# SegataLab/metamlst

Hardware: NVIDIA B200
Metric: aligned reads/s (score+pileup+consensus) (higher is better)
Workload: dtype int32/u8 (integer bit-plane arithmetic)

## Files before the change

include/mmlst.h:

```cpp
#ifndef MMLST_H
#define MMLST_H

#include <stddef.h>
#include <stdint.h>

#ifdef __cplusplus
extern "C" {
#endif

#define MMLST_VERSION 200

enum {
    MMLST_OK = 0,
    MMLST_E_ARG = -1,
    MMLST_E_CUDA = -2,
    MMLST_E_IO = -3,
    MMLST_E_BAM = -4,
    MMLST_E_UNSORTED = -5,
    MMLST_E_PAIRED = -6,
    MMLST_E_RANGE = -7,
    MMLST_E_NOMEM = -8
};

typedef struct mmlst_ctx mmlst_ctx;

const char* mmlst_last_error(void);
int mmlst_version(void);
int mmlst_device_count(void);

int mmlst_create(int device, mmlst_ctx** out);
void mmlst_destroy(mmlst_ctx* ctx);
void* mmlst_stream(mmlst_ctx* ctx);
int mmlst_sync(mmlst_ctx* ctx);

void* mmlst_pinned_alloc(size_t bytes);
void mmlst_pinned_free(void* p);

int mmlst_score_dev(const uint32_t* tid, const int16_t* as0, const uint8_t* xm3, const uint16_t* qlen,
                    const uint32_t* orig_idx, uint64_t n_rec, uint64_t idx_base,
                    const uint8_t* allow, const uint32_t* locus_of, uint32_t n_ref,
                    int minscore, int max_xm, int min_read_len,
                    int64_t* sum_as, uint32_t* n_hit, uint32_t* first_idx, uint64_t* counters, void* stream);

int mmlst_build_runs(const uint32_t* tid, uint64_t n_rec, uint32_t* run_tid, uint32_t* run_start, uint32_t* chunk_run,
                     uint32_t* n_runs);
int mmlst_score_runs_dev(const uint32_t* run_tid, const uint32_t* run_start, uint32_t n_runs, const uint32_t* chunk_run,
                         const int16_t* as0, const uint8_t* xm3, const uint16_t* qlen, const uint32_t* orig_idx,
                         uint64_t n_rec, uint64_t idx_base, const uint8_t* allow, uint32_t n_ref,
                         int minscore, int max_xm, int min_read_len,
                         int64_t* sum_as, uint32_t* n_hit, uint32_t* first_idx, uint64_t* counters, void* stream);
int mmlst_chunk_qlen(const uint16_t* qlen, uint64_t n_rec, uint16_t* chunk_qlen, int* uniform);
int mmlst_score_runs_qc_dev(const uint32_t* run_tid, const uint32_t* run_start, uint32_t n_runs, const uint32_t* chunk_run,
                            const uint16_t* chunk_qlen, const int16_t* as0, const uint8_t* xm3, const uint32_t* orig_idx,
                            uint64_t n_rec, uint64_t idx_base, const uint8_t* allow, uint32_t n_ref,
                            int minscore, int max_xm, int min_read_len,
                            int64_t* sum_as, uint32_t* n_hit, uint32_t* first_idx, uint64_t* counters, void* stream);
#define MMLST_SCORE_VARIANT_DEFAULT 6
int mmlst_set_score_variant(int variant);
#define MMLST_SCORE_L2_HINTS_DEFAULT 1
int mmlst_set_score_l2_hints(int on);
int mmlst_debug_timeline(uint64_t* dev_buf);
#define MMLST_SCORE_GRID_DEFAULT 8
int mmlst_set_score_grid_scale(int eighths);
int mmlst_as_untransform_dev(int16_t* as0, const uint8_t* xm3, uint64_t n, int coeff, void* stream);
int mmlst_expand_chunk_qlen_dev(const uint16_t* chunk_qlen, uint64_t n_rec, uint16_t* qlen, void* stream);
int mmlst_expand_runs_dev(const uint32_t* run_tid, const uint32_t* run_start, uint32_t n_runs, const uint32_t* chunk_run,
                          uint64_t n_rec, uint32_t* tid, void* stream);

uint64_t mmlst_coverage_table_slots(uint64_t n_names_upper_bound);
int mmlst_coverage_dev(const uint32_t* tid, const int16_t* as0, const uint8_t* xm3, const uint16_t* qlen,
                       const uint32_t* orig_idx, const uint64_t* qhash, uint64_t n_rec, uint64_t idx_base,
                       const uint8_t* allow, const uint32_t* locus_of, uint32_t n_ref, int minscore, int max_xm,
                       int min_read_len, void* table, uint64_t table_slots, uint64_t* cov, void* stream);

typedef struct {
    int32_t pos;
    uint32_t row_off;
    uint16_t reflen;
    int16_t as_named;
    uint8_t xm_named;
    uint8_t pad;
    uint16_t nw;
} mmlst_prec;

typedef struct {
    uint32_t rec_begin, rec_end;
    uint32_t col_base, contig_len;
    uint32_t plane_delta;
    uint32_t reserved[3];
} mmlst_chunk;

uint32_t mmlst_chunk_records(uint64_t n_rec);

int mmlst_pileup_dev(const mmlst_prec* recs, const uint32_t* planes,
                     const mmlst_chunk* chunks, uint32_t n_chunks, uint32_t max_row_words,
                     int minscore, int max_xm, uint32_t* counts, uint32_t total_cols, int impl, void* stream);

int mmlst_depth_cap(const uint32_t* tid, const int32_t* pos, const uint32_t* reflen, uint64_t n, uint32_t maxcnt,
                    uint32_t sentinel_nodes, uint8_t* admitted);

int mmlst_consensus_dev(const uint32_t* counts, const uint8_t* dbseq, const uint32_t* col_off, uint32_t n_loci,
                        uint32_t mincov, uint8_t* cons, uint32_t* holes, uint32_t* snps, void* stream);

#define MMLST_STATS_COLUMNS 0u
#define MMLST_STATS_DEPTH 1u
#define MMLST_STATS_LOWDOM 2u
#define MMLST_CONTIG_STATS_MAX_COLS 858993459u
typedef struct {
    uint32_t mode;
    uint32_t mincov;
    uint32_t trunc;
    uint32_t none_char;
    double dominant_frq_thrsh;
} mmlst_contig_stats_params;
size_t mmlst_contig_stats_scratch_bytes(uint32_t total_cols);
int mmlst_contig_stats_dev(uint32_t* counts, const uint32_t* col_off, uint32_t n, uint32_t total_cols, const mmlst_contig_stats_params* prm,
                           void* scratch, size_t scratch_bytes, uint32_t* sel_off, uint32_t* low_off, uint64_t* depth_off,
                           uint32_t* out_col, uint32_t* out_val, uint8_t* cons, uint32_t flags, void* stream);

#define MMLST_SELECT_WARP_DEFAULT 0
int mmlst_set_select_warp_finalize(int on);
#define MMLST_SELECT_CONSUME 1u
#define MMLST_SELECT_SCRATCH_CLEAN 2u
#define MMLST_SELECT_LOCAL 4u
int mmlst_select_dev(int64_t* sum_as, uint32_t* n_hit, uint32_t* first_idx, const uint32_t* locus_rows, const uint32_t* locus_start,
                     const uint32_t* allele_num, uint32_t n_ref, const uint32_t* species_of_locus, const uint32_t* genes_in_db,
                     uint32_t n_loci, uint32_t n_species, int penalty, int nloci_pct, const uint64_t* contig_start,
                     const uint32_t* ref_len, const uint64_t* db_off, uint32_t chunk_records, void* scratch, size_t scratch_bytes,
                     uint32_t* header, uint32_t* chosen_tid, uint32_t* chosen_species, uint32_t* col_off, uint64_t* db_start,
                     mmlst_chunk* chunks, uint32_t max_chunks, uint32_t flags, uint64_t* counters,
                     uint32_t* chosen_first , void* stream);
int mmlst_set_pdl(int on);
int mmlst_pileup_indirect_dev(const mmlst_prec* recs, const uint32_t* planes, const mmlst_chunk* chunks, const uint32_t* header,
                              uint32_t max_row_words, int minscore, int max_xm, uint32_t* counts, int impl, void* stream);
int mmlst_pileup_consensus_indirect_dev(const mmlst_prec* recs, const uint32_t* planes, const mmlst_chunk* chunks, const uint32_t* header,
                                        uint32_t max_row_words, int minscore, int max_xm, uint32_t* counts, const uint8_t* db_ascii,
                                        const uint64_t* db_start, const uint32_t* col_off, uint32_t max_loci, uint32_t mincov, uint8_t* cons,
                                        uint32_t* holes, uint32_t* snps, uint32_t flags, uint32_t* ticket, void* stream);
#define MMLST_CONSENSUS_CONSUME 1u
int mmlst_consensus_indirect_dev(uint32_t* counts, const uint8_t* db_ascii, const uint64_t* db_start, const uint32_t* col_off,
                                 uint32_t max_loci, const uint32_t* header, uint32_t mincov, uint8_t* cons, uint32_t* holes,
                                 uint32_t* snps, uint32_t flags, void* stream);

int mmlst_xchg_publish_dev(const void* block, uint32_t bytes, const uint64_t* peer_base, uint32_t rank, uint32_t world,
                           uint64_t half_stride, uint64_t slot_stride, uint64_t flag_off, const uint64_t* epoch, void* stream);
int mmlst_xchg_await_dev(void* local_base, uint32_t bytes, uint32_t world, uint64_t half_stride, uint64_t slot_stride,
                         uint64_t flag_off, void* out_all, uint64_t* epoch, uint32_t* ticket, uint32_t* status, void* stream);

typedef struct mmlst_comm mmlst_comm;
int mmlst_comm_unique_id(uint8_t* id128);
int mmlst_comm_create(const uint8_t* id128, int rank, int world, int device, mmlst_comm** out);
void mmlst_comm_destroy(mmlst_comm* comm);
int mmlst_allreduce(mmlst_comm* comm, int64_t* score_block, size_t score_words, uint32_t* first_idx, size_t n_ref, uint32_t* counts, size_t n_counts,
                    void* stream);

int mmlst_hamming_min_dev(const uint32_t* db_hi, const uint32_t* db_lo, const uint16_t* row_len, uint32_t n_rows,
                          uint32_t W, const uint32_t* q_hi, const uint32_t* q_lo, const uint16_t* q_len, uint32_t n_q,
                          const uint32_t* blocks, uint32_t n_blocks, uint32_t row_index_base,
                          unsigned long long* best, void* stream);
int mmlst_hamming_exact_dev(const uint32_t* db_hi, const uint32_t* db_lo, const uint16_t* row_len, uint32_t n_rows, uint32_t W,
                            const uint32_t* q_hi, const uint32_t* q_lo, const uint16_t* q_len, uint32_t n_q,
                            const uint32_t* blocks, uint32_t n_blocks, uint32_t row_index_base,
                            const uint32_t* xr_ids, const uint32_t* xr_x, const uint8_t* xr_bytes, uint32_t n_xr,
                            const uint32_t* xq_ids, const uint32_t* xq_x, const uint8_t* xq_bytes, uint32_t n_xq,
                            unsigned long long* best, void* stream);
int mmlst_hamming_min_dev2(const uint32_t* db_hi, const uint32_t* db_lo, const uint16_t* row_len, uint32_t n_rows,
                           uint32_t W, const uint32_t* q_hi, const uint32_t* q_lo, const uint16_t* q_len, uint32_t n_q,
                           const uint32_t* blocks, uint32_t n_blocks, uint32_t max_block_rows, uint32_t max_block_queries,
                           uint32_t row_index_base, unsigned long long* best, void* stream);

typedef struct {
    const uint8_t* bytes; uint64_t n_bytes;
    const uint64_t* table; uint32_t n_blocks;
    int32_t as_xm_coeff;
} mmlst_zstream;

typedef struct {
    const uint8_t* bytes; uint64_t n_bytes;
    const uint64_t* table; uint32_t n_blocks;
    const uint32_t* contig_block;
} mmlst_zpileup;

typedef struct {
    const uint32_t* tid; const int16_t* as0; const uint8_t* xm3; const uint16_t* qlen; const uint32_t* orig_idx;
    uint64_t n_rec;
    const mmlst_prec* p_recs;
    const uint32_t* planes; uint64_t n_prec; uint64_t n_plane_words; uint32_t max_row_words;
    const uint64_t* contig_start;
    uint32_t n_ref;
    uint32_t n_runs;
    const uint32_t* run_tid; const uint32_t* run_start; const uint32_t* chunk_run;
    const uint16_t* chunk_qlen;
    const mmlst_zstream* z;
    const mmlst_zpileup* zp;
} mmlst_soa;

typedef struct { int minscore, max_xm, min_read_len; } mmlst_score_params;

int mmlst_score(mmlst_ctx* ctx, const mmlst_soa* soa, const uint8_t* allow, const uint32_t* locus_of, uint32_t n_loci,
                const mmlst_score_params* prm, int64_t* sum_as, uint32_t* n_hit, uint32_t* first_idx, uint64_t* counters);

typedef struct {
    const uint32_t* locus_of; const uint32_t* allele_num; uint32_t n_ref;
    const uint32_t* species_of_locus; uint32_t n_loci;
    const uint32_t* genes_in_db; uint32_t n_species;
    const uint8_t* db_ascii; const uint64_t* db_off; const uint32_t* bam_ln;
} mmlst_index;
typedef struct { int minscore, max_xm, min_read_len, penalty, nloci_pct; uint32_t mincov; int pileup_impl; } mmlst_sample_params;
typedef struct {
    uint32_t n_chosen, error_bits, bad_len_tid, reserved;
    uint64_t total_reads, ignored_reads;
    uint32_t* chosen_tid; uint32_t* chosen_species; uint32_t* col_off;
    uint8_t* cons; uint64_t cons_capacity;
    uint32_t* holes; uint32_t* snps;
    int64_t* sum_as; uint32_t* n_hit; uint32_t* first_idx;
} mmlst_sample_result;
int mmlst_index_upload(mmlst_ctx* ctx, const mmlst_index* index);
int mmlst_sample(mmlst_ctx* ctx, const mmlst_soa* soa, const uint8_t* allow, const mmlst_sample_params* prm, mmlst_sample_result* res);

#define MMLST_COVERAGE_STREAM_RESIDENT 1u
int mmlst_coverage(mmlst_ctx* ctx, const mmlst_soa* soa, const uint64_t* qhash, const uint8_t* allow, const uint32_t* locus_of,
                   uint32_t n_loci, const mmlst_score_params* prm, uint32_t flags, uint64_t* cov);

int mmlst_pileup_consensus(mmlst_ctx* ctx, const mmlst_soa* soa, const uint32_t* chosen_tid, uint32_t n_loci,
                           const uint8_t* dbseq, const uint32_t* col_off, int minscore, int max_xm, uint32_t mincov,
                           int impl, uint32_t* counts, uint8_t* cons, uint32_t* holes, uint32_t* snps);

typedef struct {
    uint32_t* sel_off;
    uint32_t* low_off;
    uint64_t* depth_off;
    uint32_t* out_col;
    uint32_t* out_val;
    uint8_t* cons;
    uint64_t capacity;
    uint64_t n_out;
} mmlst_contig_stats_out;
int mmlst_contig_stats(mmlst_ctx* ctx, const mmlst_soa* soa, const uint32_t* tid, uint32_t n, const uint32_t* col_off, int minscore,
                       int max_xm, const mmlst_contig_stats_params* prm, mmlst_contig_stats_out* out);

int mmlst_db_upload(mmlst_ctx* ctx, const uint32_t* db_hi, const uint32_t* db_lo, const uint16_t* row_len,
                    uint32_t n_rows, uint32_t W);
int mmlst_hamming_min(mmlst_ctx* ctx, const uint32_t* q_hi, const uint32_t* q_lo, const uint16_t* q_len, uint32_t n_q,
                      const uint32_t* blocks, uint32_t n_blocks, uint32_t* min_dist, uint32_t* argmin_row);
int mmlst_db_upload_x(mmlst_ctx* ctx, const uint32_t* db_hi, const uint32_t* db_lo, const uint16_t* row_len, uint32_t n_rows,
                      uint32_t W, const uint32_t* xr_ids, const uint32_t* xr_x, const uint8_t* xr_bytes, uint32_t n_xr);
int mmlst_hamming_min_x(mmlst_ctx* ctx, const uint32_t* q_hi, const uint32_t* q_lo, const uint16_t* q_len, uint32_t n_q,
                        const uint32_t* xq_ids, const uint32_t* xq_x, const uint8_t* xq_bytes, uint32_t n_xq,
                        const uint32_t* blocks, uint32_t n_blocks, uint32_t* min_dist, uint32_t* argmin_row);

size_t mmlst_hamming_tc_image_bytes(uint32_t n, uint32_t W, uint32_t tile_rows);
int mmlst_hamming_tc_expand_dev(const uint32_t* hi, const uint32_t* lo, const uint16_t* len, uint32_t n, uint32_t W, int db_tiled_layout,
                                uint32_t tile_rows, uint8_t* image, uint32_t* tile_maxlen, void* stream);
int mmlst_hamming_tc_search_dev(const uint8_t* q_image, const uint32_t* q_tile_maxlen, const uint16_t* q_len, uint32_t n_q,
                                const uint8_t* db_image, const uint32_t* db_tile_maxlen, const uint16_t* row_len, uint32_t n_rows,
                                uint32_t W, uint32_t row_index_base, unsigned long long* best, void* stream);

int mmlst_exact_match_dev(const uint32_t* db_hi, const uint32_t* db_lo, const uint16_t* row_len, uint32_t n_rows, uint32_t W,
                          const uint32_t* q_hi, const uint32_t* q_lo, const uint16_t* q_len, uint32_t n_q,
                          const uint32_t* blocks, uint32_t n_blocks, uint32_t max_block_rows, uint32_t row_index_base,
                          const uint32_t* row_key , const uint32_t* xr_ids, const uint8_t* xr_bytes, uint32_t n_xr,
                          const uint32_t* xq_ids, const uint8_t* xq_bytes, uint32_t n_xq, uint32_t* first_row, void* stream);
int mmlst_db_row_keys(mmlst_ctx* ctx, const uint32_t* row_key, uint32_t n_rows);
int mmlst_exact_match(mmlst_ctx* ctx, const uint32_t* q_hi, const uint32_t* q_lo, const uint16_t* q_len, uint32_t n_q,
                      const uint32_t* xq_ids, const uint8_t* xq_bytes, uint32_t n_xq,
                      const uint32_t* blocks, uint32_t n_blocks, uint32_t* first_row);

int mmlst_st_match_dev(const uint32_t* prof_start, const uint32_t* prof_allele, uint32_t n_st,
                       const uint32_t* q_alleles, const uint32_t* q_n, uint32_t l_max, uint32_t n_q,
                       uint32_t* count, uint32_t* best, uint32_t* n_best, uint32_t* out_idx, uint32_t max_out, void* stream);
int mmlst_profiles_upload(mmlst_ctx* ctx, const uint32_t* prof_start, const uint32_t* prof_allele, uint32_t n_st);
int mmlst_st_match(mmlst_ctx* ctx, const uint32_t* q_alleles, const uint32_t* q_n, uint32_t l_max, uint32_t n_q,
                   uint32_t* best, uint32_t* n_best, uint32_t* out_idx, uint32_t max_out);

int mmlst_inflate_raw(const uint8_t* in, size_t n, uint8_t* out, size_t out_capacity, size_t* produced);

typedef struct mmlst_bam mmlst_bam;
typedef struct {
    int minqual; uint32_t max_depth; uint32_t sentinel_nodes; int n_threads; int pinned; int assume_sorted;
    int want_qhash; int check_crc;
    int lenient_tags;
} mmlst_unpack_opts;
typedef struct {
    mmlst_soa soa;
    const uint64_t* qhash;
    const uint32_t* ref_len;
    const char* ref_names;
    const char* header_text;
    uint64_t n_dropped_by_cap, n_unmapped_flag;
    int presorted, minqual; uint32_t max_depth;
    double seconds[5];
    uint64_t n_untagged;
} mmlst_bam_info_t;
int mmlst_bam_unpack(const char* path, const mmlst_unpack_opts* opts , mmlst_bam** out);
int mmlst_bam_info(const mmlst_bam* bam, mmlst_bam_info_t* info);
void mmlst_bam_free(mmlst_bam* bam);

typedef struct mmlst_dev_bam mmlst_dev_bam;
typedef struct {
    const uint32_t* tid; const int16_t* as0; const uint8_t* xm3; const uint16_t* qlen; const uint32_t* orig_idx; const uint64_t* qhash;
    const uint32_t* run_tid; const uint32_t* run_start; const uint32_t* chunk_run; const uint16_t* chunk_qlen; uint32_t n_runs;
    const mmlst_prec* p_recs; const uint32_t* planes;
    uint64_t n_rec, n_prec, n_plane_words; uint32_t max_row_words;
    const uint64_t* contig_start;
    const uint32_t* ref_len;
    const char* ref_names;
    const char* header_text;
    uint32_t n_ref;
    uint64_t n_dropped_by_cap, n_unmapped_flag, n_bgzf_blocks, compressed_bytes, inflated_bytes;
    int presorted, minqual; uint32_t max_depth; int boundary_repairs;
    double seconds[8];
} mmlst_dev_bam_info_t;
int mmlst_bam_ingest(int device, const uint8_t* bam, size_t n_bytes, const mmlst_unpack_opts* opts, void* stream, mmlst_dev_bam** out);
int mmlst_dev_bam_info(const mmlst_dev_bam* bam, mmlst_dev_bam_info_t* info);
void mmlst_dev_bam_free(mmlst_dev_bam* bam);
int mmlst_ingest_trim(int device);

#ifdef __cplusplus
}
#endif
#endif
```

metamlst_b200/bam.py:

```python
from __future__ import annotations

import ctypes as C
import os
from typing import Optional

import numpy as np

from . import native, packing


class UnpackOpts(C.Structure):
    _fields_ = [("minqual", C.c_int), ("max_depth", C.c_uint32), ("sentinel_nodes", C.c_uint32), ("n_threads", C.c_int),
                ("pinned", C.c_int), ("assume_sorted", C.c_int), ("want_qhash", C.c_int), ("check_crc", C.c_int), ("lenient_tags", C.c_int)]


class BamInfo(C.Structure):
    _fields_ = [("soa", native.Soa), ("qhash", C.c_void_p), ("ref_len", C.c_void_p), ("ref_names", C.c_char_p),
                ("header_text", C.c_char_p), ("n_dropped_by_cap", C.c_uint64), ("n_unmapped_flag", C.c_uint64),
                ("presorted", C.c_int), ("minqual", C.c_int), ("max_depth", C.c_uint32), ("seconds", C.c_double * 5), ("n_untagged", C.c_uint64)]


class _Handle:
    def __init__(self, h):
        self.h = h

    def __del__(self):
        try:
            if self.h:
                native.lib().mmlst_bam_free(self.h)
                self.h = None
        except Exception:
            pass


def _view(addr: Optional[int], n: int, dtype) -> np.ndarray:
    dt = np.dtype(dtype)
    if not addr or n == 0:
        return np.zeros(0, dtype=dt)
    buf = (C.c_uint8 * (n * dt.itemsize)).from_address(addr)
    return np.frombuffer(buf, dtype=dt, count=n)


def unpack_bam(path: str, minqual: int = packing.DEFAULT_MINQUAL, max_depth: Optional[int] = packing.DEFAULT_MAX_DEPTH,
               presorted: bool = False, threads: int = 0, pinned: bool = True, want_qhash: bool = True,
               sentinel_nodes: int = 1, lenient_tags: bool = False) -> packing.SoaHost:
    lib = native.lib()
    o = UnpackOpts(int(minqual), int(max_depth or 0), int(sentinel_nodes), int(threads), 1 if pinned else 0,
                   1 if presorted else 0, 1 if want_qhash else 0, 1, 1 if lenient_tags else 0)
    h = C.c_void_p()
    native.check(lib.mmlst_bam_unpack(path.encode(), C.byref(o), C.byref(h)))
    keep = _Handle(h)
    info = BamInfo()
    native.check(lib.mmlst_bam_info(h, C.byref(info)))
    s = info.soa
    n, P, n_ref = int(s.n_rec), int(s.n_prec), int(s.n_ref)
    names = info.ref_names.decode("latin-1").split("\n") if n_ref else []
    soa = packing.SoaHost(
        names, _view(info.ref_len, n_ref, np.uint32).astype(np.int32),
        _view(s.tid, n, np.uint32), _view(s.as0, n, np.int16), _view(s.xm3, n, np.uint8), _view(s.qlen, n, np.uint16),
        _view(s.orig_idx, n, np.uint32) if s.orig_idx else None,
        _view(s.p_recs, P, packing.PREC_DTYPE), _view(s.planes, int(s.n_plane_words), np.uint32), int(s.max_row_words),
        _view(s.contig_start, n_ref + 1, np.uint64), int(info.minqual), int(info.max_depth), int(info.n_dropped_by_cap))
    if s.run_tid:
        nr = int(s.n_runs)
        soa.run_tid, soa.run_start = _view(s.run_tid, nr, np.uint32), _view(s.run_start, nr + 1, np.uint32)
        soa.chunk_run = _view(s.chunk_run, (n + 255) // 256, np.uint32)
        soa.chunk_qlen = _view(s.chunk_qlen, (n + 255) // 256, np.uint16) if s.chunk_qlen else None
        if nr > 0.125 * n:
            soa.run_tid = soa.run_start = soa.chunk_run = soa.chunk_qlen = None
    soa.qhash = _view(info.qhash, 2 * n, np.uint64).reshape(n, 2) if info.qhash else None
    soa.header_text = (info.header_text or b"").decode("latin-1")
    soa.unpack_seconds = dict(zip(("read", "inflate", "parse", "sort", "pack"), [float(x) for x in info.seconds]))
    soa.lenient, soa.n_untagged = bool(lenient_tags), int(info.n_untagged)
    soa._keep = (keep,)
    return soa


class DevBamInfo(C.Structure):
    _fields_ = [("tid", C.c_void_p), ("as0", C.c_void_p), ("xm3", C.c_void_p), ("qlen", C.c_void_p), ("orig_idx", C.c_void_p), ("qhash", C.c_void_p),
                ("run_tid", C.c_void_p), ("run_start", C.c_void_p), ("chunk_run", C.c_void_p), ("chunk_qlen", C.c_void_p), ("n_runs", C.c_uint32),
                ("p_recs", C.c_void_p), ("planes", C.c_void_p),
                ("n_rec", C.c_uint64), ("n_prec", C.c_uint64), ("n_plane_words", C.c_uint64), ("max_row_words", C.c_uint32),
                ("contig_start", C.c_void_p), ("ref_len", C.c_void_p), ("ref_names", C.c_char_p), ("header_text", C.c_char_p), ("n_ref", C.c_uint32),
                ("n_dropped_by_cap", C.c_uint64), ("n_unmapped_flag", C.c_uint64), ("n_bgzf_blocks", C.c_uint64), ("compressed_bytes", C.c_uint64),
                ("inflated_bytes", C.c_uint64), ("presorted", C.c_int), ("minqual", C.c_int), ("max_depth", C.c_uint32), ("boundary_repairs", C.c_int),
                ("seconds", C.c_double * 8)]


class _DevHandle:
    def __init__(self, h):
        self.h = h

    def __del__(self):
        try:
            if self.h:
                native.lib().mmlst_dev_bam_free(self.h)
                self.h = None
        except Exception:
            pass


class _DevArray:

    def __init__(self, addr: int, n: int, typestr: str, keep):
        self.__cuda_array_interface__ = {"shape": (n,), "typestr": typestr, "data": (addr, False), "version": 2, "strides": None}
        self._keep = keep


class PinnedPool:

    def __init__(self):
        import threading
        self._lock = threading.Lock()
        self._free = []

    def get(self, n: int):
        import torch
        with self._lock:
            best = None
            for i, t in enumerate(self._free):
                if t.numel() >= n and (best is None or t.numel() < self._free[best].numel()):
                    best = i
            if best is not None:
                return self._free.pop(best)
        return torch.empty(max(int(n * 1.25), 1 << 20), dtype=torch.uint8, pin_memory=torch.cuda.is_available())

    def put(self, t) -> None:
        base = getattr(t, "_pool_base", None)
        if base is not None:
            with self._lock:
                if len(self._free) < 16:
                    self._free.append(base)


POOL = PinnedPool()


def read_pinned(path: str, pool: Optional[PinnedPool] = None):
    import torch
    size = os.path.getsize(path)
    if pool is not None:
        base = pool.get(size)
    else:
        base = torch.empty(max(size, 1), dtype=torch.uint8, pin_memory=torch.cuda.is_available())
    with open(path, "rb") as fh:
        got = fh.readinto(memoryview(base.numpy())[:size]) if size else 0
    if got != size:
        raise IOError("short read on %s" % path)
    view = base[:size]
    if pool is not None:
        view._pool_base = base
    return view


def ingest_bam(source, device=0, minqual: int = packing.DEFAULT_MINQUAL, max_depth: Optional[int] = packing.DEFAULT_MAX_DEPTH,
               presorted: bool = False, want_qhash: bool = True, sentinel_nodes: int = 1, check_crc: bool = False):
    import torch
    from . import streams
    dev = torch.device("cuda", device) if isinstance(device, int) else torch.device(device)
    data = read_pinned(source) if isinstance(source, str) else source
    addr = data.data_ptr() if hasattr(data, "data_ptr") else data.ctypes.data
    nbytes = int(data.numel() if hasattr(data, "numel") else data.size)
    lib = native.lib()
    o = UnpackOpts(int(minqual), int(max_depth or 0), int(sentinel_nodes), 0, 1, 1 if presorted else 0, 1 if want_qhash else 0,
                  1 if check_crc else 0, 0)
    h = C.c_void_p()
    with torch.cuda.device(dev):
        stream = torch.cuda.current_stream(dev).cuda_stream
        native.check(lib.mmlst_bam_ingest(dev.index or 0, addr, nbytes, C.byref(o), stream, C.byref(h)))
    keep = _DevHandle(h)
    info = DevBamInfo()
    native.check(lib.mmlst_dev_bam_info(h, C.byref(info)))
    n, P, n_ref, nr = int(info.n_rec), int(info.n_prec), int(info.n_ref), int(info.n_runs)

    def t(addr_, count, typestr, dtype):
        if not addr_ or count == 0:
            return torch.zeros(0, dtype=dtype, device=dev)
        return torch.as_tensor(_DevArray(addr_, count, typestr, keep), device=dev)

    s = streams.DeviceStreams()
    s._keep = keep
    s.ref_names = info.ref_names.decode("latin-1").split("\n") if n_ref else []
    s.ref_lens = _view(info.ref_len, n_ref, np.uint32).astype(np.int32)
    s.header_text = (info.header_text or b"").decode("latin-1")
    s.minqual, s.max_depth, s.n_dropped = int(info.minqual), int(info.max_depth), int(info.n_dropped_by_cap)
    s.idx_base = 0
    s.tid, s.as0 = t(info.tid, n, "<i4", torch.int32), t(info.as0, n, "<i2", torch.int16)
    s.xm3, s.qlen = t(info.xm3, n, "|u1", torch.uint8), t(info.qlen, n, "<i2", torch.int16)
    s.orig_idx = t(info.orig_idx, n, "<i4", torch.int32) if info.orig_idx else None
    s.qhash = t(info.qhash, 2 * n, "<i8", torch.int64).view(n, 2) if (info.qhash and want_qhash) else None
    s.p_recs = t(info.p_recs, 4 * P, "<i4", torch.int32).view(P, 4)
    s.planes = t(info.planes, int(info.n_plane_words), "<i4", torch.int32)
    s.n_prec, s.max_row_words = P, int(info.max_row_words)
    s.contig_start = _view(info.contig_start, n_ref + 1, np.uint64).copy()
    s.run_tid = s.run_start = s.chunk_run = s.chunk_qlen = None
    if nr and nr <= 0.125 * n:
        s.run_tid, s.run_start = t(info.run_tid, nr, "<i4", torch.int32), t(info.run_start, nr + 1, "<i4", torch.int32)
        s.chunk_run = t(info.chunk_run, (n + 255) // 256, "<i4", torch.int32)
        s.chunk_qlen = t(info.chunk_qlen, (n + 255) // 256, "<i2", torch.int16) if info.chunk_qlen else None
    s.presorted = bool(info.presorted)
    s.ingest_seconds = dict(zip(("h2d", "inflate", "chain", "parse", "sort", "score_stream", "cap_compact", "pack"), [float(x) for x in info.seconds]))
    s.ingest_stats = {"bgzf_blocks": int(info.n_bgzf_blocks), "compressed_bytes": int(info.compressed_bytes), "inflated_bytes": int(info.inflated_bytes),
                      "boundary_repairs": int(info.boundary_repairs), "unmapped_flag": int(info.n_unmapped_flag)}
    return s
```

metamlst_b200/csrc/score_runs.cu:

```cuda
#include <stdlib.h>

#include "score_runs_kernels.cuh"


static int g_score_variant = -1;
static int score_variant() {
    if (g_score_variant < 0) {
        const char* e = getenv("MMLST_SCORE_VARIANT");
        g_score_variant = (e && e[0] >= '0' && e[0] <= '6' && !e[1]) ? e[0] - '0' : MMLST_SCORE_VARIANT_DEFAULT;
    }
    return g_score_variant;
}
extern "C" int mmlst_set_score_variant(int v) {
    const int prev = score_variant();
    if (v >= 0 && v <= 6) g_score_variant = v;
    return prev;
}

static int g_score_l2_hints = -1;
static int score_l2_hints() {
    if (g_score_l2_hints < 0) {
        const char* e = getenv("MMLST_SCORE_L2_HINTS");
        g_score_l2_hints = e ? (e[0] == '1') : MMLST_SCORE_L2_HINTS_DEFAULT;
    }
    return g_score_l2_hints;
}
extern "C" int mmlst_set_score_l2_hints(int on) {
    const int prev = score_l2_hints();
    if (on == 0 || on == 1) g_score_l2_hints = on;
    return prev;
}

static int g_score_grid8 = -1;
static int score_grid8() {
    if (g_score_grid8 < 0) {
        const char* e = getenv("MMLST_SCORE_GRID");
        const int v = e ? atoi(e) : 0;
        g_score_grid8 = (v >= 1 && v <= 64) ? v : MMLST_SCORE_GRID_DEFAULT;
    }
    return g_score_grid8;
}
extern "C" int mmlst_set_score_grid_scale(int eighths) {
    const int prev = score_grid8();
    if (eighths >= 1 && eighths <= 64) g_score_grid8 = eighths;
    return prev;
}

static int score_runs_launch(const uint32_t* run_tid, const uint32_t* run_start, uint32_t n_runs, const uint32_t* chunk_run,
                             const int16_t* as0, const uint8_t* xm3, const uint16_t* qlen, const uint16_t* chunk_qlen, const uint32_t* orig_idx,
                             uint64_t n_rec, uint64_t idx_base, const uint8_t* allow, uint32_t n_ref, int minscore,
                             int max_xm, int min_read_len, int64_t* sum_as, uint32_t* n_hit, uint32_t* first_idx,
                             uint64_t* counters, void* stream) {
    if (n_rec == 0) return MMLST_OK;
    if (!run_tid || !run_start || !chunk_run || !n_runs || !as0 || !xm3 || (!qlen && !chunk_qlen) || !allow || !sum_as || !n_hit || !first_idx || !counters) {
        mmlst_set_error("mmlst_score_runs_dev: null pointer");
        return MMLST_E_ARG;
    }
    if (n_rec >= 0xffffff00ull) { mmlst_set_error("mmlst_score_runs_dev: %llu records do not fit 32-bit run offsets", (unsigned long long)n_rec); return MMLST_E_RANGE; }
    if ((reinterpret_cast<uintptr_t>(as0) & 15) || (reinterpret_cast<uintptr_t>(xm3) & 7) || (!chunk_qlen && (reinterpret_cast<uintptr_t>(qlen) & 15)) ||
        (orig_idx && (reinterpret_cast<uintptr_t>(orig_idx) & 15))) {
        mmlst_set_error("mmlst_score_runs_dev: record arrays must be 16-byte aligned (as0/qlen/orig_idx), 8 (xm3)");
        return MMLST_E_ARG;
    }
    RunArgs a{run_tid, run_start, chunk_run, n_runs, as0, xm3, qlen, orig_idx, chunk_qlen, n_rec, idx_base, allow, n_ref, minscore, max_xm,
              min_read_len, reinterpret_cast<long long*>(sum_as), n_hit, first_idx, reinterpret_cast<unsigned long long*>(counters), score_l2_hints()};
    const uint64_t nchunks = n_rec >> 8;
    uint64_t want = (nchunks + 15) / 16;
    const int variant = score_variant();
    const cudaStream_t st = static_cast<cudaStream_t>(stream);
    const bool tma_ok = !orig_idx && !(reinterpret_cast<uintptr_t>(xm3) & 15);
    if (variant == 6 && tma_ok && chunk_qlen) {
        static int pair_resident_by_device[MMLST_MAX_DEVICES] = {0};
        int& pair_resident = pair_resident_by_device[mmlst_current_device()];
        const size_t smem = (kThreads / 32) * 2u * (4u * 768u + sizeof(uint64_t));
        if (!pair_resident) {
            CUDA_TRY(cudaFuncSetAttribute(score_runs_ring_pair_kernel, cudaFuncAttributeMaxDynamicSharedMemorySize, static_cast<int>(smem)));
            CUDA_TRY(cudaFuncSetAttribute(score_runs_ring_pair_kernel, cudaFuncAttributePreferredSharedMemoryCarveout, cudaSharedmemCarveoutMaxShared));
            int r = 0;
            if (cudaOccupancyMaxActiveBlocksPerMultiprocessor(&r, score_runs_ring_pair_kernel, kThreads, smem) != cudaSuccess || r < 1) r = 1;
            pair_resident = r;
        }
        const uint64_t cap = static_cast<uint64_t>(mmlst_num_sms()) * pair_resident * score_grid8() / 8;
        if (want > cap) want = cap;
        if (want < 1) want = 1;
        score_runs_ring_pair_kernel<<<static_cast<unsigned>(want), kThreads, smem, st>>>(a);
        CUDA_TRY(cudaGetLastError());
        return MMLST_OK;
    }
    if (variant >= 2 && tma_ok) {
        static int ring_resident_by_device[MMLST_MAX_DEVICES][4][8] = {{{0}}};
        int (&ring_resident)[4][8] = ring_resident_by_device[mmlst_current_device()];
        const int hint = a.l2_hints ? 1 : 0;
        const int q = (chunk_qlen ? 1 : 0) + 2 * hint;
        const int rv = variant == 6 ? 5 : variant;
        const RingCfg cfg = chunk_qlen ? (hint ? ring_config<true, true>(rv) : ring_config<true, false>(rv))
                                       : (hint ? ring_config<false, true>(rv) : ring_config<false, false>(rv));
        const size_t smem = (kThreads / 32) * static_cast<size_t>(cfg.ns) * (cfg.ch * (chunk_qlen ? 768u : 1280u) + sizeof(uint64_t));
        if (!ring_resident[q][rv]) {
            CUDA_TRY(cudaFuncSetAttribute(cfg.kern, cudaFuncAttributeMaxDynamicSharedMemorySize, static_cast<int>(smem)));
            CUDA_TRY(cudaFuncSetAttribute(cfg.kern, cudaFuncAttributePreferredSharedMemoryCarveout, cudaSharedmemCarveoutMaxShared));
            int r = 0;
            if (cudaOccupancyMaxActiveBlocksPerMultiprocessor(&r, cfg.kern, kThreads, smem) != cudaSuccess || r < 1) r = 1;
            ring_resident[q][rv] = r;
        }
        const uint64_t cap = static_cast<uint64_t>(mmlst_num_sms()) * ring_resident[q][rv];
        if (want > cap) want = cap;
        if (want < 1) want = 1;
        cfg.kern<<<static_cast<unsigned>(want), kThreads, smem, st>>>(a);
        CUDA_TRY(cudaGetLastError());
        return MMLST_OK;
    }
    static int resident_by_device[MMLST_MAX_DEVICES][8] = {{0}};
    int (&resident)[8] = resident_by_device[mmlst_current_device()];
    const int v = (orig_idx ? 1 : 0) + 2 * (variant == 1 ? 1 : 0) + (chunk_qlen ? 4 : 0);
    void (*const kerns[8])(const RunArgs) = {score_runs_kernel<false, false, false>, score_runs_kernel<true, false, false>,
                                             score_runs_kernel<false, true, false>, score_runs_kernel<true, true, false>,
                                             score_runs_kernel<false, false, true>, score_runs_kernel<true, false, true>,
                                             score_runs_kernel<false, true, true>, score_runs_kernel<true, true, true>};
    void (*kern)(const RunArgs) = kerns[v];
    if (!resident[v]) {
        if (cudaOccupancyMaxActiveBlocksPerMultiprocessor(&resident[v], kern, kThreads, 0) != cudaSuccess || resident[v] < 1) resident[v] = 3;
    }
    const uint64_t cap = static_cast<uint64_t>(mmlst_num_sms()) * resident[v];
    if (want > cap) want = cap;
    if (want < 1) want = 1;
    kern<<<static_cast<unsigned>(want), kThreads, 0, st>>>(a);
    CUDA_TRY(cudaGetLastError());
    return MMLST_OK;
}

extern "C" int mmlst_score_runs_dev(const uint32_t* run_tid, const uint32_t* run_start, uint32_t n_runs, const uint32_t* chunk_run,
                                    const int16_t* as0, const uint8_t* xm3, const uint16_t* qlen, const uint32_t* orig_idx,
                                    uint64_t n_rec, uint64_t idx_base, const uint8_t* allow, uint32_t n_ref, int minscore,
                                    int max_xm, int min_read_len, int64_t* sum_as, uint32_t* n_hit, uint32_t* first_idx,
                                    uint64_t* counters, void* stream) {
    if (n_rec && !qlen) { mmlst_set_error("mmlst_score_runs_dev: null pointer"); return MMLST_E_ARG; }
    return score_runs_launch(run_tid, run_start, n_runs, chunk_run, as0, xm3, qlen, nullptr, orig_idx, n_rec, idx_base, allow, n_ref, minscore,
                             max_xm, min_read_len, sum_as, n_hit, first_idx, counters, stream);
}

extern "C" int mmlst_score_runs_qc_dev(const uint32_t* run_tid, const uint32_t* run_start, uint32_t n_runs, const uint32_t* chunk_run,
                                       const uint16_t* chunk_qlen, const int16_t* as0, const uint8_t* xm3, const uint32_t* orig_idx,
                                       uint64_t n_rec, uint64_t idx_base, const uint8_t* allow, uint32_t n_ref, int minscore,
                                       int max_xm, int min_read_len, int64_t* sum_as, uint32_t* n_hit, uint32_t* first_idx,
                                       uint64_t* counters, void* stream) {
    if (n_rec && !chunk_qlen) { mmlst_set_error("mmlst_score_runs_qc_dev: null pointer"); return MMLST_E_ARG; }
    return score_runs_launch(run_tid, run_start, n_runs, chunk_run, as0, xm3, nullptr, chunk_qlen, orig_idx, n_rec, idx_base, allow, n_ref,
                             minscore, max_xm, min_read_len, sum_as, n_hit, first_idx, counters, stream);
}

extern "C" int mmlst_expand_chunk_qlen_dev(const uint16_t* chunk_qlen, uint64_t n_rec, uint16_t* qlen, void* stream) {
    if (n_rec == 0) return MMLST_OK;
    if (!chunk_qlen || !qlen) { mmlst_set_error("mmlst_expand_chunk_qlen_dev: null pointer"); return MMLST_E_ARG; }
    uint64_t blocks = (n_rec + 255) / 256;
    const uint64_t cap = static_cast<uint64_t>(mmlst_num_sms()) * 16;
    if (blocks > cap) blocks = cap;
    expand_chunk_qlen_kernel<<<static_cast<unsigned>(blocks), 256, 0, static_cast<cudaStream_t>(stream)>>>(chunk_qlen, n_rec, qlen);
    CUDA_TRY(cudaGetLastError());
    return MMLST_OK;
}

extern "C" int mmlst_expand_runs_dev(const uint32_t* run_tid, const uint32_t* run_start, uint32_t n_runs, const uint32_t* chunk_run,
                                     uint64_t n_rec, uint32_t* tid, void* stream) {
    if (n_rec == 0) return MMLST_OK;
    if (!run_tid || !run_start || !chunk_run || !n_runs || !tid) { mmlst_set_error("mmlst_expand_runs_dev: null pointer"); return MMLST_E_ARG; }
    uint64_t blocks = (n_rec + 255) / 256;
    const uint64_t cap = static_cast<uint64_t>(mmlst_num_sms()) * 16;
    if (blocks > cap) blocks = cap;
    expand_runs_kernel<<<static_cast<unsigned>(blocks), 256, 0, static_cast<cudaStream_t>(stream)>>>(run_tid, run_start, chunk_run, n_runs, n_rec, tid);
    CUDA_TRY(cudaGetLastError());
    return MMLST_OK;
}

namespace {
__global__ void __launch_bounds__(256) as_untransform_kernel(int16_t* __restrict__ as0, const uint8_t* __restrict__ xm3, uint64_t n, int coeff) {
    const uint64_t n8 = n >> 3;
    const uint64_t stride = static_cast<uint64_t>(gridDim.x) * blockDim.x;
    for (uint64_t i = static_cast<uint64_t>(blockIdx.x) * blockDim.x + threadIdx.x; i < n8; i += stride) {
        uint4 a = reinterpret_cast<uint4*>(as0)[i];
        const uint2 x = ld_stream_u2(xm3 + (i << 3));
        uint32_t aw[4] = {a.x, a.y, a.z, a.w};
        const uint32_t xw[2] = {x.x, x.y};
#pragma unroll
        for (int w = 0; w < 4; ++w) {
            const uint32_t xb = xw[w >> 1] >> ((w & 1) * 16);
            const int lo = static_cast<int16_t>(aw[w] & 0xffffu) - coeff * static_cast<int>(xb & 0xffu);
            const int hi = static_cast<int16_t>(aw[w] >> 16) - coeff * static_cast<int>((xb >> 8) & 0xffu);
            aw[w] = (static_cast<uint32_t>(lo) & 0xffffu) | (static_cast<uint32_t>(hi) << 16);
        }
        reinterpret_cast<uint4*>(as0)[i] = make_uint4(aw[0], aw[1], aw[2], aw[3]);
    }
    if (blockIdx.x == 0 && threadIdx.x == 0)
        for (uint64_t i = n8 << 3; i < n; ++i) as0[i] = static_cast<int16_t>(as0[i] - coeff * static_cast<int>(xm3[i]));
}
}

extern "C" int mmlst_as_untransform_dev(int16_t* as0, const uint8_t* xm3, uint64_t n, int coeff, void* stream) {
    if (n == 0 || coeff == 0) return MMLST_OK;
    if (!as0 || !xm3) { mmlst_set_error("mmlst_as_untransform_dev: null pointer"); return MMLST_E_ARG; }
    if ((reinterpret_cast<uintptr_t>(as0) & 15) || (reinterpret_cast<uintptr_t>(xm3) & 7)) { mmlst_set_error("mmlst_as_untransform_dev: as0 must be 16-byte aligned, xm3 8"); return MMLST_E_ARG; }
    uint64_t blocks = ((n >> 3) + 255) / 256;
    const uint64_t cap = static_cast<uint64_t>(mmlst_num_sms()) * 8;
    if (blocks > cap) blocks = cap;
    if (blocks < 1) blocks = 1;
    as_untransform_kernel<<<static_cast<unsigned>(blocks), 256, 0, static_cast<cudaStream_t>(stream)>>>(as0, xm3, n, coeff);
    CUDA_TRY(cudaGetLastError());
    return MMLST_OK;
}
```

metamlst_b200/csrc/score_runs_kernels.cuh:

```cuda
#pragma once
#include "common.cuh"

namespace {

constexpr int kThreads = 256;
constexpr uint32_t FULL = 0xffffffffu;

struct RunArgs {
    const uint32_t* run_tid; const uint32_t* run_start; const uint32_t* chunk_run; uint32_t n_runs;
    const int16_t* as0; const uint8_t* xm3; const uint16_t* qlen; const uint32_t* orig_idx;
    const uint16_t* chunk_qlen;
    uint64_t n_rec; uint64_t idx_base;
    const uint8_t* allow; uint32_t n_ref;
    int minscore, max_xm, min_read_len;
    long long* sum_as; uint32_t* n_hit; uint32_t* first_idx; unsigned long long* counters;
    int l2_hints;
};

__device__ __forceinline__ void flush_run(const RunArgs& a, uint32_t key, long long s, uint32_t c, uint32_t mn) {
    if (c) {
        atomicAdd(reinterpret_cast<unsigned long long*>(a.sum_as + key), static_cast<unsigned long long>(s));
        atomicAdd(a.n_hit + key, c);
        atomicMin(a.first_idx + key, mn);
    }
}

template <bool OIDX> struct Loaded;
template <> struct Loaded<false> { uint4 a8, q8; uint2 x8; uint32_t cq; };
template <> struct Loaded<true> { uint4 a8, q8; uint2 x8; uint32_t cq; uint4 oa, ob; };

template <bool OIDX, bool QC>
__device__ __forceinline__ Loaded<OIDX> load_chunk(const RunArgs& a, uint64_t base_lane) {
    Loaded<OIDX> L;
    L.a8 = ld_stream_u4(a.as0 + base_lane);
    L.x8 = ld_stream_u2(a.xm3 + base_lane);
    if constexpr (QC) { L.cq = __ldg(a.chunk_qlen + (base_lane >> 8)); L.q8 = make_uint4(0, 0, 0, 0); }
    else { L.q8 = ld_stream_u4(a.qlen + base_lane); L.cq = 0; }
    if constexpr (OIDX) { L.oa = ld_stream_u4(a.orig_idx + base_lane); L.ob = ld_stream_u4(a.orig_idx + base_lane + 4); }
    return L;
}

template <bool OIDX>
__device__ __forceinline__ uint32_t rec_index(const Loaded<OIDX>& L, uint32_t idx0, int k) {
    if constexpr (OIDX) {
        const uint32_t oi[8] = {L.oa.x, L.oa.y, L.oa.z, L.oa.w, L.ob.x, L.ob.y, L.ob.z, L.ob.w};
        return oi[k];
    } else {
        return idx0 + k;
    }
}

struct WarpRun {
    uint32_t r, key, end;
    bool al;
    long long s; uint32_t c, mn;
};

__device__ __forceinline__ void open_run(const RunArgs& a, WarpRun& w, uint32_t r) {
    w.r = r;
    if (r < a.n_runs) {
        w.key = __ldg(a.run_tid + r);
        w.end = __ldg(a.run_start + r + 1);
        w.al = (w.key < a.n_ref) && a.allow[w.key];
    } else {
        w.key = 0xffffffffu; w.end = 0xffffffffu; w.al = false;
    }
    w.s = 0; w.c = 0; w.mn = 0xffffffffu;
}

__device__ __forceinline__ void close_run(const RunArgs& a, WarpRun& w, uint32_t lane) {
    if (lane == 0 && w.al) flush_run(a, w.key, w.s, w.c, w.mn);
}

struct Thr {
    uint32_t as_T, as_TL;
    uint32_t ql_T, ql_TL;
    uint32_t xm_T, xm_TH;
    uint32_t h8;
};
constexpr uint32_t H16 = 0x80008000u, H8 = 0x80808080u;

__device__ __forceinline__ Thr make_thr(const RunArgs& a) {
    Thr t;
    const bool none = a.minscore > 32767 || a.min_read_len > 65535 || a.max_xm < 0;
    const uint32_t ts = static_cast<uint32_t>(max(a.minscore, -32768) + 32768) & 0xffffu;
    const uint32_t tq = static_cast<uint32_t>(min(max(a.min_read_len, 0), 65535));
    const uint32_t tx = static_cast<uint32_t>(min(max(a.max_xm, 0), 255));
    t.as_T = ts | (ts << 16); t.as_TL = t.as_T & ~H16;
    t.ql_T = tq | (tq << 16); t.ql_TL = t.ql_T & ~H16;
    t.xm_T = tx * 0x01010101u; t.xm_TH = t.xm_T | H8;
    t.h8 = none ? 0u : H8;
    return t;
}

template <bool OIDX, bool QC>
__device__ __forceinline__ void lane_pass(const Loaded<OIDX>& L, const Thr& t, int min_read_len, uint32_t& p_lo, uint32_t& p_hi) {
    const uint32_t aw[4] = {L.a8.x, L.a8.y, L.a8.z, L.a8.w};
    const uint32_t qw[4] = {L.q8.x, L.q8.y, L.q8.z, L.q8.w};
    uint32_t m[4];
#pragma unroll
    for (int w = 0; w < 4; ++w) {
        const uint32_t da = (aw[w] | H16) - t.as_TL;
        const uint32_t ga = (~aw[w] & ~t.as_T) | ((aw[w] ^ t.as_T) & da);
        if constexpr (QC) {
            m[w] = ga;
        } else {
            const uint32_t dq = (qw[w] | H16) - t.ql_TL;
            const uint32_t gq = (qw[w] & ~t.ql_T) | (~(qw[w] ^ t.ql_T) & dq);
            m[w] = ga & gq;
        }
    }
    const uint32_t b_lo = __byte_perm(m[0], m[1], 0x7531), b_hi = __byte_perm(m[2], m[3], 0x7531);
    const uint32_t x0 = L.x8.x, x1 = L.x8.y;
    const uint32_t d0 = t.xm_TH - (x0 & ~H8), d1 = t.xm_TH - (x1 & ~H8);
    const uint32_t g0 = (t.xm_T & ~x0) | (~(t.xm_T ^ x0) & d0), g1 = (t.xm_T & ~x1) | (~(t.xm_T ^ x1) & d1);
    p_lo = (b_lo & g0 & t.h8) >> 7;
    p_hi = (b_hi & g1 & t.h8) >> 7;
    if constexpr (QC) {
        if (static_cast<int>(L.cq) < min_read_len) { p_lo = 0; p_hi = 0; }
    }
}

template <bool OIDX>
__device__ __forceinline__ void lane_sums(const Loaded<OIDX>& L, uint32_t p_lo, uint32_t p_hi, uint32_t idx0, int& s, uint32_t& c, uint32_t& mn) {
    s = __dp2a_lo(static_cast<int>(L.a8.x), static_cast<int>(p_lo), 0);
    s = __dp2a_hi(static_cast<int>(L.a8.y), static_cast<int>(p_lo), s);
    s = __dp2a_lo(static_cast<int>(L.a8.z), static_cast<int>(p_hi), s);
    s = __dp2a_hi(static_cast<int>(L.a8.w), static_cast<int>(p_hi), s);
    c = __popc(p_lo | (p_hi << 1));
    if constexpr (OIDX) {
        mn = 0xffffffffu;
#pragma unroll
        for (int k = 0; k < 8; ++k) mn = (((k < 4 ? p_lo : p_hi) >> (8 * (k & 3))) & 1u) ? min(mn, rec_index<true>(L, idx0, k)) : mn;
    } else {
        const uint32_t k = p_lo ? (static_cast<uint32_t>(__ffs(p_lo)) - 1u) >> 3 : 4u + ((static_cast<uint32_t>(__ffs(p_hi)) - 1u) >> 3);
        mn = (p_lo | p_hi) ? idx0 + k : 0xffffffffu;
    }
}

template <bool OIDX, bool QC>
__device__ __forceinline__ void reduce_chunk(const RunArgs& a, const Thr& thr, WarpRun& w, const Loaded<OIDX>& L, uint64_t base, uint32_t lane,
                                             uint32_t& tot, uint32_t& ign) {
    constexpr uint32_t R = 8;
    const uint64_t rec0 = base + (lane << 3);
    const uint32_t idx0 = static_cast<uint32_t>(a.idx_base + rec0);
    uint32_t p_lo, p_hi;
    lane_pass<OIDX, QC>(L, thr, a.min_read_len, p_lo, p_hi);
    const uint64_t chunk_end = base + 256;
    if (chunk_end <= w.end) {
        if (w.al) {
            int s; uint32_t c, mn;
            lane_sums<OIDX>(L, p_lo, p_hi, idx0, s, c, mn);
            tot += R;
            ign += R - c;
            w.s += __reduce_add_sync(FULL, s);
            w.c += __reduce_add_sync(FULL, c);
            w.mn = min(w.mn, __reduce_min_sync(FULL, mn));
        }
        if (chunk_end == w.end) { close_run(a, w, lane); open_run(a, w, w.r + 1); }
        return;
    }
    uint64_t lo = base;
    while (lo < chunk_end) {
        const uint64_t hi = (w.end < chunk_end) ? static_cast<uint64_t>(w.end) : chunk_end;
        if (w.al) {
            const uint32_t klo = lo <= rec0 ? 0u : (lo - rec0 >= R ? R : static_cast<uint32_t>(lo - rec0));
            const uint32_t khi = hi <= rec0 ? 0u : (hi - rec0 >= R ? R : static_cast<uint32_t>(hi - rec0));
            const unsigned long long ones = 0x0101010101010101ull;
            const unsigned long long below_hi = khi >= 8 ? ~0ull : ((1ull << (8 * khi)) - 1ull);
            const unsigned long long below_lo = klo >= 8 ? ~0ull : ((1ull << (8 * klo)) - 1ull);
            const unsigned long long inm = khi > klo ? (below_hi & ~below_lo & ones) : 0ull;
            const uint32_t in_lo = static_cast<uint32_t>(inm), in_hi = static_cast<uint32_t>(inm >> 32);
            int s; uint32_t c, mn;
            lane_sums<OIDX>(L, p_lo & in_lo, p_hi & in_hi, idx0, s, c, mn);
            const uint32_t in = khi > klo ? khi - klo : 0u;
            tot += in;
            ign += in - c;
            w.s += __reduce_add_sync(FULL, s);
            w.c += __reduce_add_sync(FULL, c);
            w.mn = min(w.mn, __reduce_min_sync(FULL, mn));
        }
        if (hi == w.end) { close_run(a, w, lane); open_run(a, w, w.r + 1); }
        lo = hi;
    }
}

template <bool QC>
__device__ __forceinline__ void score_tail(const RunArgs& a, uint64_t nchunks, uint32_t lane, uint32_t& tot, uint32_t& ign) {
    uint32_t r = __ldg(a.chunk_run + nchunks);
    for (uint64_t i = (nchunks << 8) + lane; i < a.n_rec; i += 32) {
        while (r + 1 < a.n_runs && i >= a.run_start[r + 1]) ++r;
        const uint32_t key = a.run_tid[r];
        if (!((key < a.n_ref) && a.allow[key])) continue;
        ++tot;
        const int as = a.as0[i];
        const int ql = QC ? int(a.chunk_qlen[nchunks]) : int(a.qlen[i]);
        if ((as >= a.minscore) && (ql >= a.min_read_len) && (int(a.xm3[i]) <= a.max_xm)) {
            const uint32_t idx = a.orig_idx ? a.orig_idx[i] : static_cast<uint32_t>(a.idx_base + i);
            flush_run(a, key, as, 1u, idx);
        } else {
            ++ign;
        }
    }
}

template <bool OIDX, bool PIPE, bool QC>
__global__ void __launch_bounds__(kThreads, PIPE ? (OIDX ? 2 : 3) : (OIDX ? 3 : 4)) score_runs_kernel(const RunArgs a) {
    pdl_launch_dependents();
    const uint32_t lane = threadIdx.x & 31u;
    const uint64_t warp = (static_cast<uint64_t>(blockIdx.x) * blockDim.x + threadIdx.x) >> 5;
    const uint64_t nwarps = (static_cast<uint64_t>(gridDim.x) * blockDim.x) >> 5;
    const uint64_t nchunks = a.n_rec >> 8;
    const uint64_t per = (nchunks + nwarps - 1) / nwarps;
    const uint64_t c0 = warp * per;
    const uint64_t c1 = (c0 + per < nchunks) ? c0 + per : nchunks;
    uint32_t tot = 0, ign = 0;
    const Thr thr = make_thr(a);

    if (c0 < c1) {
        uint64_t ch = c0;
        Loaded<OIDX> A0, A1;
        bool have = ch + 1 < c1;
        if (have) { A0 = load_chunk<OIDX, QC>(a, (ch << 8) + (lane << 3)); A1 = load_chunk<OIDX, QC>(a, ((ch + 1) << 8) + (lane << 3)); }
        WarpRun w;
        open_run(a, w, __ldg(a.chunk_run + c0));
        Loaded<OIDX> B0, B1;
        if constexpr (!PIPE) {
            while (have) {
                reduce_chunk<OIDX, QC>(a, thr, w, A0, ch << 8, lane, tot, ign);
                reduce_chunk<OIDX, QC>(a, thr, w, A1, (ch + 1) << 8, lane, tot, ign);
                ch += 2;
                have = ch + 1 < c1;
                if (have) { A0 = load_chunk<OIDX, QC>(a, (ch << 8) + (lane << 3)); A1 = load_chunk<OIDX, QC>(a, ((ch + 1) << 8) + (lane << 3)); }
            }
        }
        while (have) {
            const bool moreB = ch + 3 < c1;
            if (moreB) { B0 = load_chunk<OIDX, QC>(a, ((ch + 2) << 8) + (lane << 3)); B1 = load_chunk<OIDX, QC>(a, ((ch + 3) << 8) + (lane << 3)); }
            reduce_chunk<OIDX, QC>(a, thr, w, A0, ch << 8, lane, tot, ign);
            reduce_chunk<OIDX, QC>(a, thr, w, A1, (ch + 1) << 8, lane, tot, ign);
            ch += 2;
            if (!moreB) break;
            have = ch + 3 < c1;
            if (have) { A0 = load_chunk<OIDX, QC>(a, ((ch + 2) << 8) + (lane << 3)); A1 = load_chunk<OIDX, QC>(a, ((ch + 3) << 8) + (lane << 3)); }
            reduce_chunk<OIDX, QC>(a, thr, w, B0, ch << 8, lane, tot, ign);
            reduce_chunk<OIDX, QC>(a, thr, w, B1, (ch + 1) << 8, lane, tot, ign);
            ch += 2;
        }
        if (ch < c1) {
            const uint64_t base = ch << 8;
            const Loaded<OIDX> L0 = load_chunk<OIDX, QC>(a, base + (lane << 3));
            reduce_chunk<OIDX, QC>(a, thr, w, L0, base, lane, tot, ign);
        }
        close_run(a, w, lane);
    }

    if (warp == nwarps - 1 && (a.n_rec & 255u)) score_tail<QC>(a, nchunks, lane, tot, ign);
    tot = __reduce_add_sync(FULL, tot);
    ign = __reduce_add_sync(FULL, ign);
    if (lane == 0 && tot) {
        atomicAdd(a.counters + 0, static_cast<unsigned long long>(tot));
        atomicAdd(a.counters + 1, static_cast<unsigned long long>(ign));
    }
}

struct WarpRunPF {
    uint32_t r, key, end;
    uint32_t nkey, nend;
    bool al;
    long long s; uint32_t c, mn;
};

template <bool HINT> __device__ __forceinline__ uint32_t tab_u32(const uint32_t* p, uint64_t pol) {
    if constexpr (HINT) return ld_table_u32(p, pol); else return __ldg(p);
}
template <bool HINT> __device__ __forceinline__ uint32_t tab_u16(const uint16_t* p, uint64_t pol) {
    if constexpr (HINT) return ld_table_u16(p, pol); else return __ldg(p);
}
template <bool HINT> __device__ __forceinline__ uint32_t tab_u8(const uint8_t* p, uint64_t pol) {
    if constexpr (HINT) return ld_table_u8(p, pol); else return *p;
}
template <bool HINT>
__device__ __forceinline__ void request_next_run(const RunArgs& a, WarpRunPF& w, uint64_t pol) {
    if (w.r + 1u < a.n_runs) { w.nkey = tab_u32<HINT>(a.run_tid + w.r + 1u, pol); w.nend = tab_u32<HINT>(a.run_start + w.r + 2u, pol); }
    else { w.nkey = 0xffffffffu; w.nend = 0xffffffffu; }
}
template <bool HINT>
__device__ __forceinline__ void open_run_pf(const RunArgs& a, WarpRunPF& w, uint32_t r, uint64_t pol) {
    w.r = r;
    if (r < a.n_runs) { w.key = tab_u32<HINT>(a.run_tid + r, pol); w.end = tab_u32<HINT>(a.run_start + r + 1u, pol); }
    else { w.key = 0xffffffffu; w.end = 0xffffffffu; }
    request_next_run<HINT>(a, w, pol);
    w.al = (w.key < a.n_ref) && tab_u8<HINT>(a.allow + w.key, pol);
    w.s = 0; w.c = 0; w.mn = 0xffffffffu;
}
template <bool HINT>
__device__ __forceinline__ void next_run_pf(const RunArgs& a, WarpRunPF& w, uint32_t lane, uint64_t pol) {
    if (lane == 0 && w.al) flush_run(a, w.key, w.s, w.c, w.mn);
    w.r += 1u; w.key = w.nkey; w.end = w.nend;
    request_next_run<HINT>(a, w, pol);
    w.al = (w.key < a.n_ref) && tab_u8<HINT>(a.allow + w.key, pol);
    w.s = 0; w.c = 0; w.mn = 0xffffffffu;
}

__device__ __forceinline__ uint32_t bytes_below(uint32_t k) { return k >= 4u ? 0xffffffffu : ((1u << (8u * k)) - 1u); }
__device__ __forceinline__ void segment_masks(uint32_t klo, uint32_t khi, uint32_t& in_lo, uint32_t& in_hi) {
    in_lo = bytes_below(min(khi, 4u)) & ~bytes_below(min(klo, 4u)) & 0x01010101u;
    in_hi = bytes_below(khi > 4u ? khi - 4u : 0u) & ~bytes_below(klo > 4u ? klo - 4u : 0u) & 0x01010101u;
}

__device__ __forceinline__ void lane_sums_pf(const Loaded<false>& L, uint32_t p_lo, uint32_t p_hi, int& s, uint32_t& c) {
    s = __dp2a_lo(static_cast<int>(L.a8.x), static_cast<int>(p_lo), 0);
    s = __dp2a_hi(static_cast<int>(L.a8.y), static_cast<int>(p_lo), s);
    s = __dp2a_lo(static_cast<int>(L.a8.z), static_cast<int>(p_hi), s);
    s = __dp2a_hi(static_cast<int>(L.a8.w), static_cast<int>(p_hi), s);
    c = __popc(p_lo | (p_hi << 1));
}
__device__ __forceinline__ uint32_t first_pass_index(uint32_t p_lo, uint32_t p_hi, uint32_t idx0) {
    const uint32_t k = p_lo ? (static_cast<uint32_t>(__ffs(p_lo)) - 1u) >> 3 : 4u + ((static_cast<uint32_t>(__ffs(p_hi)) - 1u) >> 3);
    return (p_lo | p_hi) ? idx0 + k : 0xffffffffu;
}

template <bool QC, bool HINT>
__device__ __forceinline__ void reduce_chunk_pf(const RunArgs& a, const Thr& thr, WarpRunPF& w, const Loaded<false>& L, uint32_t base, uint32_t lane,
                                                uint32_t& tot, uint32_t& ign, uint64_t pol) {
    constexpr uint32_t R = 8;
    const uint32_t idx0 = static_cast<uint32_t>(a.idx_base) + base + (lane << 3);
    uint32_t p_lo, p_hi;
    lane_pass<false, QC>(L, thr, a.min_read_len, p_lo, p_hi);
    const uint32_t chunk_end = base + 256u;
    if (chunk_end <= w.end) {
        if (w.al) {
            int s; uint32_t c;
            lane_sums_pf(L, p_lo, p_hi, s, c);
            tot += R;
            ign += R - c;
            w.s += __reduce_add_sync(FULL, s);
            w.c += __reduce_add_sync(FULL, c);
            if (w.mn == 0xffffffffu) w.mn = __reduce_min_sync(FULL, first_pass_index(p_lo, p_hi, idx0));
        }
        if (chunk_end == w.end) next_run_pf<HINT>(a, w, lane, pol);
        return;
    }
    const int lane0 = static_cast<int>(lane << 3);
    uint32_t lo = base;
    while (lo < chunk_end) {
        const uint32_t hi = min(w.end, chunk_end);
        if (w.al) {
            const uint32_t klo = static_cast<uint32_t>(min(max(static_cast<int>(lo - base) - lane0, 0), 8));
            const uint32_t khi = static_cast<uint32_t>(min(max(static_cast<int>(hi - base) - lane0, 0), 8));
            uint32_t in_lo, in_hi;
            segment_masks(klo, khi, in_lo, in_hi);
            int s; uint32_t c;
            lane_sums_pf(L, p_lo & in_lo, p_hi & in_hi, s, c);
            const uint32_t in = khi - klo;
            tot += in;
            ign += in - c;
            w.s += __reduce_add_sync(FULL, s);
            w.c += __reduce_add_sync(FULL, c);
            if (w.mn == 0xffffffffu) w.mn = __reduce_min_sync(FULL, first_pass_index(p_lo & in_lo, p_hi & in_hi, idx0));
        }
        if (hi == w.end) next_run_pf<HINT>(a, w, lane, pol);
        lo = hi;
    }
}

template <bool QC, int NS, int CH, int MINB, bool HINT>
__global__ void __launch_bounds__(kThreads, MINB) score_runs_ring_kernel(const RunArgs a) {
    pdl_launch_dependents();
    extern __shared__ __align__(128) uint8_t ring_raw[];
    constexpr uint32_t AS_B = CH * 512u, QL_B = QC ? 0u : CH * 512u, XM_B = CH * 256u;
    constexpr uint32_t STAGE_B = AS_B + QL_B + XM_B;
    constexpr uint32_t CH_B = STAGE_B / CH;
    constexpr int NW = kThreads / 32;
    const uint32_t lane = threadIdx.x & 31u, wid = threadIdx.x >> 5;
    uint8_t* const my = ring_raw + wid * (NS * STAGE_B);
    uint64_t* const bars = reinterpret_cast<uint64_t*>(ring_raw + NW * NS * STAGE_B) + wid * NS;
    if (threadIdx.x == 0) {
        uint64_t* all = reinterpret_cast<uint64_t*>(ring_raw + NW * NS * STAGE_B);
        for (int i = 0; i < NW * NS; ++i) mbar_init(all + i, 1);
        fence_mbar_init();
    }
    __syncthreads();

    const uint64_t warp = (static_cast<uint64_t>(blockIdx.x) * blockDim.x + threadIdx.x) >> 5;
    const uint64_t nwarps = (static_cast<uint64_t>(gridDim.x) * blockDim.x) >> 5;
    const uint64_t nchunks = a.n_rec >> 8;
    const uint64_t per = (nchunks + nwarps - 1) / nwarps;
    const uint64_t c0 = warp * per;
    const uint64_t c1 = (c0 + per < nchunks) ? c0 + per : nchunks;
    uint32_t tot = 0, ign = 0;
    const Thr thr = make_thr(a);
    const uint64_t pol_s = HINT ? l2_policy(1) : 0ull, pol_t = HINT ? l2_policy(2) : 0ull;

    if (c0 < c1) {
        const uint32_t ngroups = static_cast<uint32_t>((c1 - c0 + CH - 1) / CH);
        auto issue = [&](uint32_t g, int stage) {
            const uint64_t ch = c0 + static_cast<uint64_t>(g) * CH;
            const uint32_t nch = (c1 - ch < CH) ? static_cast<uint32_t>(c1 - ch) : static_cast<uint32_t>(CH);
            uint8_t* st = my + stage * STAGE_B;
            mbar_expect_tx(bars + stage, nch * CH_B);
            if constexpr (HINT) {
                bulk_g2s_hint(st, a.as0 + (ch << 8), nch * 512u, bars + stage, pol_s);
                if constexpr (!QC) bulk_g2s_hint(st + AS_B, a.qlen + (ch << 8), nch * 512u, bars + stage, pol_s);
                bulk_g2s_hint(st + AS_B + QL_B, a.xm3 + (ch << 8), nch * 256u, bars + stage, pol_s);
            } else {
                bulk_g2s(st, a.as0 + (ch << 8), nch * 512u, bars + stage);
                if constexpr (!QC) bulk_g2s(st + AS_B, a.qlen + (ch << 8), nch * 512u, bars + stage);
                bulk_g2s(st + AS_B + QL_B, a.xm3 + (ch << 8), nch * 256u, bars + stage);
            }
        };
        if (lane == 0) {
            const uint32_t pre = ngroups < static_cast<uint32_t>(NS) ? ngroups : static_cast<uint32_t>(NS);
            for (uint32_t g = 0; g < pre; ++g) issue(g, static_cast<int>(g));
        }
        WarpRunPF w;
        open_run_pf<HINT>(a, w, tab_u32<HINT>(a.chunk_run + c0, pol_t), pol_t);
        uint32_t phase = 0;
        int stage = 0;
        for (uint32_t g = 0; g < ngroups; ++g) {
            const uint64_t ch = c0 + static_cast<uint64_t>(g) * CH;
            const uint32_t nch = (c1 - ch < CH) ? static_cast<uint32_t>(c1 - ch) : static_cast<uint32_t>(CH);
            mbar_wait(bars + stage, (phase >> stage) & 1u);
            phase ^= 1u << stage;
            const uint8_t* st = my + stage * STAGE_B;
#pragma unroll
            for (uint32_t k = 0; k < static_cast<uint32_t>(CH); ++k) {
                if (k < nch) {
                    Loaded<false> L;
                    L.a8 = *reinterpret_cast<const uint4*>(st + k * 512u + lane * 16u);
                    L.x8 = *reinterpret_cast<const uint2*>(st + AS_B + QL_B + k * 256u + lane * 8u);
                    if constexpr (QC) { L.q8 = make_uint4(0, 0, 0, 0); L.cq = tab_u16<HINT>(a.chunk_qlen + ch + k, pol_t); }
                    else { L.q8 = *reinterpret_cast<const uint4*>(st + AS_B + k * 512u + lane * 16u); L.cq = 0; }
                    if (k + 1u == nch) {
                        __syncwarp();
                        if (lane == 0 && g + NS < ngroups) issue(g + NS, stage);
                    }
                    reduce_chunk_pf<QC, HINT>(a, thr, w, L, static_cast<uint32_t>((ch + k) << 8), lane, tot, ign, pol_t);
                }
            }
            stage = (stage + 1 == NS) ? 0 : stage + 1;
        }
        if (lane == 0 && w.al) flush_run(a, w.key, w.s, w.c, w.mn);
    }

    if (warp == nwarps - 1 && (a.n_rec & 255u)) score_tail<QC>(a, nchunks, lane, tot, ign);
    tot = __reduce_add_sync(FULL, tot);
    ign = __reduce_add_sync(FULL, ign);
    if (lane == 0 && tot) {
        atomicAdd(a.counters + 0, static_cast<unsigned long long>(tot));
        atomicAdd(a.counters + 1, static_cast<unsigned long long>(ign));
    }
}

__device__ __forceinline__ void reduce_pair_pf(const RunArgs& a, const Thr& thr, WarpRunPF& w, const Loaded<false>& La, const Loaded<false>& Lb,
                                               uint32_t base, uint32_t lane, uint32_t& tot, uint32_t& ign, uint64_t pol) {
    if (base + 512u > w.end) {
        reduce_chunk_pf<true, false>(a, thr, w, La, base, lane, tot, ign, pol);
        reduce_chunk_pf<true, false>(a, thr, w, Lb, base + 256u, lane, tot, ign, pol);
        return;
    }
    if (w.al) {
        uint32_t pa_lo, pa_hi, pb_lo, pb_hi;
        lane_pass<false, true>(La, thr, a.min_read_len, pa_lo, pa_hi);
        lane_pass<false, true>(Lb, thr, a.min_read_len, pb_lo, pb_hi);
        int s = __dp2a_lo(static_cast<int>(La.a8.x), static_cast<int>(pa_lo), 0);
        s = __dp2a_hi(static_cast<int>(La.a8.y), static_cast<int>(pa_lo), s);
        s = __dp2a_lo(static_cast<int>(La.a8.z), static_cast<int>(pa_hi), s);
        s = __dp2a_hi(static_cast<int>(La.a8.w), static_cast<int>(pa_hi), s);
        s = __dp2a_lo(static_cast<int>(Lb.a8.x), static_cast<int>(pb_lo), s);
        s = __dp2a_hi(static_cast<int>(Lb.a8.y), static_cast<int>(pb_lo), s);
        s = __dp2a_lo(static_cast<int>(Lb.a8.z), static_cast<int>(pb_hi), s);
        s = __dp2a_hi(static_cast<int>(Lb.a8.w), static_cast<int>(pb_hi), s);
        const uint32_t c = __popc(pa_lo | (pa_hi << 1) | (pb_lo << 2) | (pb_hi << 3));
        tot += 16u;
        ign += 16u - c;
        w.s += __reduce_add_sync(FULL, s);
        w.c += __reduce_add_sync(FULL, c);
        if (w.mn == 0xffffffffu) {
            const uint32_t idx0 = static_cast<uint32_t>(a.idx_base) + base + (lane << 3);
            const uint32_t ma = first_pass_index(pa_lo, pa_hi, idx0);
            w.mn = __reduce_min_sync(FULL, ma != 0xffffffffu ? ma : first_pass_index(pb_lo, pb_hi, idx0 + 256u));
        }
    }
    if (base + 512u == w.end) next_run_pf<false>(a, w, lane, pol);
}

__global__ void __launch_bounds__(kThreads, 4) score_runs_ring_pair_kernel(const RunArgs a) {
    pdl_launch_dependents();
    extern __shared__ __align__(128) uint8_t ring_raw[];
    constexpr int NS = 2;
    constexpr uint32_t CH = 4, AS_B = CH * 512u, XM_B = CH * 256u, STAGE_B = AS_B + XM_B, CH_B = STAGE_B / CH;
    constexpr int NW = kThreads / 32;
    const uint32_t lane = threadIdx.x & 31u, wid = threadIdx.x >> 5;
    uint8_t* const my = ring_raw + wid * (NS * STAGE_B);
    uint64_t* const bars = reinterpret_cast<uint64_t*>(ring_raw + NW * NS * STAGE_B) + wid * NS;
    if (threadIdx.x == 0) {
        uint64_t* all = reinterpret_cast<uint64_t*>(ring_raw + NW * NS * STAGE_B);
        for (int i = 0; i < NW * NS; ++i) mbar_init(all + i, 1);
        fence_mbar_init();
    }
    __syncthreads();

    const uint64_t warp = (static_cast<uint64_t>(blockIdx.x) * blockDim.x + threadIdx.x) >> 5;
    const uint64_t nwarps = (static_cast<uint64_t>(gridDim.x) * blockDim.x) >> 5;
    const uint64_t nchunks = a.n_rec >> 8;
    const uint64_t per = (nchunks + nwarps - 1) / nwarps;
    const uint64_t c0 = warp * per;
    const uint64_t c1 = (c0 + per < nchunks) ? c0 + per : nchunks;
    uint32_t tot = 0, ign = 0;
    const Thr thr = make_thr(a);

    if (c0 < c1) {
        const uint32_t ngroups = static_cast<uint32_t>((c1 - c0 + CH - 1) / CH);
        auto issue = [&](uint32_t g, int stage) {
            const uint64_t ch = c0 + static_cast<uint64_t>(g) * CH;
            const uint32_t nch = (c1 - ch < CH) ? static_cast<uint32_t>(c1 - ch) : CH;
            uint8_t* st = my + stage * STAGE_B;
            mbar_expect_tx(bars + stage, nch * CH_B);
            if (a.l2_hints) {
                const uint64_t pol_s = l2_policy(1);
                bulk_g2s_hint(st, a.as0 + (ch << 8), nch * 512u, bars + stage, pol_s);
                bulk_g2s_hint(st + AS_B, a.xm3 + (ch << 8), nch * 256u, bars + stage, pol_s);
            } else {
                bulk_g2s(st, a.as0 + (ch << 8), nch * 512u, bars + stage);
                bulk_g2s(st + AS_B, a.xm3 + (ch << 8), nch * 256u, bars + stage);
            }
        };
        if (lane == 0) {
            const uint32_t pre = ngroups < static_cast<uint32_t>(NS) ? ngroups : static_cast<uint32_t>(NS);
            for (uint32_t g = 0; g < pre; ++g) issue(g, static_cast<int>(g));
        }
        WarpRunPF w;
        open_run_pf<false>(a, w, __ldg(a.chunk_run + c0), 0ull);
        uint32_t phase = 0;
        int stage = 0;
        auto load = [&](const uint8_t* st, uint32_t k, uint64_t ch) {
            Loaded<false> L;
            L.a8 = *reinterpret_cast<const uint4*>(st + k * 512u + lane * 16u);
            L.x8 = *reinterpret_cast<const uint2*>(st + AS_B + k * 256u + lane * 8u);
            L.q8 = make_uint4(0, 0, 0, 0);
            L.cq = __ldg(a.chunk_qlen + ch + k);
            return L;
        };
        for (uint32_t g = 0; g < ngroups; ++g) {
            const uint64_t ch = c0 + static_cast<uint64_t>(g) * CH;
            const uint32_t nch = (c1 - ch < CH) ? static_cast<uint32_t>(c1 - ch) : CH;
            mbar_wait(bars + stage, (phase >> stage) & 1u);
            phase ^= 1u << stage;
            const uint8_t* st = my + stage * STAGE_B;
#pragma unroll
            for (uint32_t k = 0; k < CH; k += 2) {
                if (k < nch) {
                    const bool two = k + 1u < nch;
                    const Loaded<false> La = load(st, k, ch);
                    Loaded<false> Lb = La;
                    if (two) Lb = load(st, k + 1u, ch);
                    if (k + 2u >= nch) {
                        __syncwarp();
                        if (lane == 0 && g + NS < ngroups) issue(g + NS, stage);
                    }
                    const uint32_t base = static_cast<uint32_t>((ch + k) << 8);
                    if (two) reduce_pair_pf(a, thr, w, La, Lb, base, lane, tot, ign, 0ull);
                    else reduce_chunk_pf<true, false>(a, thr, w, La, base, lane, tot, ign, 0ull);
                }
            }
            stage = (stage + 1 == NS) ? 0 : stage + 1;
        }
        if (lane == 0 && w.al) flush_run(a, w.key, w.s, w.c, w.mn);
    }

    if (warp == nwarps - 1 && (a.n_rec & 255u)) score_tail<true>(a, nchunks, lane, tot, ign);
    tot = __reduce_add_sync(FULL, tot);
    ign = __reduce_add_sync(FULL, ign);
    if (lane == 0 && tot) {
        atomicAdd(a.counters + 0, static_cast<unsigned long long>(tot));
        atomicAdd(a.counters + 1, static_cast<unsigned long long>(ign));
    }
}

struct RingCfg { void (*kern)(const RunArgs); uint32_t ch, ns; };
template <bool QC, bool HINT>
inline RingCfg ring_config(int variant) {
    if constexpr (QC) {
        switch (variant) {
            case 3: return {score_runs_ring_kernel<true, 3, 4, 3, HINT>, 4, 3};
            case 4: return {score_runs_ring_kernel<true, 2, 8, 2, HINT>, 8, 2};
            case 5: return {score_runs_ring_kernel<true, 2, 4, 4, HINT>, 4, 2};
            default: return {score_runs_ring_kernel<true, 4, 2, 4, HINT>, 2, 4};
        }
    } else {
        switch (variant) {
            case 3: case 4: case 5: return {score_runs_ring_kernel<false, 2, 4, 2, HINT>, 4, 2};
            default: return {score_runs_ring_kernel<false, 3, 2, 3, HINT>, 2, 3};
        }
    }
}

__global__ void __launch_bounds__(256) expand_runs_kernel(const uint32_t* __restrict__ run_tid, const uint32_t* __restrict__ run_start,
                                                          const uint32_t* __restrict__ chunk_run, uint32_t n_runs, uint64_t n_rec,
                                                          uint32_t* __restrict__ tid) {
    const uint64_t stride = static_cast<uint64_t>(gridDim.x) * blockDim.x;
    for (uint64_t i = static_cast<uint64_t>(blockIdx.x) * blockDim.x + threadIdx.x; i < n_rec; i += stride) {
        uint32_t r = __ldg(chunk_run + (i >> 8));
        while (r + 1 < n_runs && i >= __ldg(run_start + r + 1)) ++r;
        tid[i] = __ldg(run_tid + r);
    }
}

__global__ void __launch_bounds__(256) expand_chunk_qlen_kernel(const uint16_t* __restrict__ chunk_qlen, uint64_t n_rec, uint16_t* __restrict__ qlen) {
    const uint64_t stride = static_cast<uint64_t>(gridDim.x) * blockDim.x;
    for (uint64_t i = static_cast<uint64_t>(blockIdx.x) * blockDim.x + threadIdx.x; i < n_rec; i += stride) qlen[i] = __ldg(chunk_qlen + (i >> 8));
}

}
```

metamlst_b200/native.py:

```python
from __future__ import annotations

import ctypes as C
import os

_HERE = os.path.dirname(os.path.abspath(__file__))
LIB_PATH = os.path.join(_HERE, "libmmlst.so")


class MmlstError(RuntimeError):
    def __init__(self, code: int, msg: str):
        super().__init__("libmmlst error %d: %s" % (code, msg))
        self.code = code


E_ARG, E_CUDA, E_IO, E_BAM, E_UNSORTED, E_PAIRED, E_RANGE, E_NOMEM = -1, -2, -3, -4, -5, -6, -7, -8


class Chunk(C.Structure):
    _fields_ = [("rec_begin", C.c_uint32), ("rec_end", C.c_uint32), ("col_base", C.c_uint32), ("contig_len", C.c_uint32),
                ("plane_delta", C.c_uint32), ("reserved", C.c_uint32 * 3)]


class Soa(C.Structure):
    _fields_ = [("tid", C.c_void_p), ("as0", C.c_void_p), ("xm3", C.c_void_p), ("qlen", C.c_void_p), ("orig_idx", C.c_void_p),
                ("n_rec", C.c_uint64),
                ("p_recs", C.c_void_p),
                ("planes", C.c_void_p), ("n_prec", C.c_uint64), ("n_plane_words", C.c_uint64), ("max_row_words", C.c_uint32),
                ("contig_start", C.c_void_p), ("n_ref", C.c_uint32),
                ("n_runs", C.c_uint32), ("run_tid", C.c_void_p), ("run_start", C.c_void_p), ("chunk_run", C.c_void_p),
                ("chunk_qlen", C.c_void_p), ("z", C.c_void_p), ("zp", C.c_void_p)]


class ZStream(C.Structure):
    _fields_ = [("bytes", C.c_void_p), ("n_bytes", C.c_uint64), ("table", C.c_void_p), ("n_blocks", C.c_uint32), ("as_xm_coeff", C.c_int32)]


class ZPileup(C.Structure):
    _fields_ = [("bytes", C.c_void_p), ("n_bytes", C.c_uint64), ("table", C.c_void_p), ("n_blocks", C.c_uint32), ("contig_block", C.c_void_p)]


class ScoreParams(C.Structure):
    _fields_ = [("minscore", C.c_int), ("max_xm", C.c_int), ("min_read_len", C.c_int)]


class Index(C.Structure):
    _fields_ = [("locus_of", C.c_void_p), ("allele_num", C.c_void_p), ("n_ref", C.c_uint32),
                ("species_of_locus", C.c_void_p), ("n_loci", C.c_uint32),
                ("genes_in_db", C.c_void_p), ("n_species", C.c_uint32),
                ("db_ascii", C.c_void_p), ("db_off", C.c_void_p), ("bam_ln", C.c_void_p)]


class SampleParams(C.Structure):
    _fields_ = [("minscore", C.c_int), ("max_xm", C.c_int), ("min_read_len", C.c_int), ("penalty", C.c_int), ("nloci_pct", C.c_int),
                ("mincov", C.c_uint32), ("pileup_impl", C.c_int)]


class SampleResult(C.Structure):
    _fields_ = [("n_chosen", C.c_uint32), ("error_bits", C.c_uint32), ("bad_len_tid", C.c_uint32), ("reserved", C.c_uint32),
                ("total_reads", C.c_uint64), ("ignored_reads", C.c_uint64),
                ("chosen_tid", C.c_void_p), ("chosen_species", C.c_void_p), ("col_off", C.c_void_p),
                ("cons", C.c_void_p), ("cons_capacity", C.c_uint64),
                ("holes", C.c_void_p), ("snps", C.c_void_p),
                ("sum_as", C.c_void_p), ("n_hit", C.c_void_p), ("first_idx", C.c_void_p)]


class ContigStatsParams(C.Structure):
    _fields_ = [("mode", C.c_uint32), ("mincov", C.c_uint32), ("trunc", C.c_uint32), ("none_char", C.c_uint32), ("dominant_frq_thrsh", C.c_double)]


class ContigStatsOut(C.Structure):
    _fields_ = [("sel_off", C.c_void_p), ("low_off", C.c_void_p), ("depth_off", C.c_void_p), ("out_col", C.c_void_p), ("out_val", C.c_void_p),
                ("cons", C.c_void_p), ("capacity", C.c_uint64), ("n_out", C.c_uint64)]


STATS_COLUMNS, STATS_DEPTH, STATS_LOWDOM = 0, 1, 2
CONTIG_STATS_MAX_COLS = 858993459


EXPORTS = {
    "mmlst_last_error": (C.c_char_p, []),
    "mmlst_version": (C.c_int, []),
    "mmlst_device_count": (C.c_int, []),
    "mmlst_create": (C.c_int, [C.c_int, C.POINTER(C.c_void_p)]),
    "mmlst_destroy": (None, [C.c_void_p]),
    "mmlst_stream": (C.c_void_p, [C.c_void_p]),
    "mmlst_sync": (C.c_int, [C.c_void_p]),
    "mmlst_pinned_alloc": (C.c_void_p, [C.c_size_t]),
    "mmlst_pinned_free": (None, [C.c_void_p]),
    "mmlst_score_dev": (C.c_int, [C.c_void_p] * 5 + [C.c_uint64, C.c_uint64, C.c_void_p, C.c_void_p, C.c_uint32,
                                  C.c_int, C.c_int, C.c_int, C.c_void_p, C.c_void_p, C.c_void_p, C.c_void_p, C.c_void_p]),
    "mmlst_build_runs": (C.c_int, [C.c_void_p, C.c_uint64, C.c_void_p, C.c_void_p, C.c_void_p, C.POINTER(C.c_uint32)]),
    "mmlst_score_runs_dev": (C.c_int, [C.c_void_p, C.c_void_p, C.c_uint32] + [C.c_void_p] * 5 + [C.c_uint64, C.c_uint64, C.c_void_p, C.c_uint32,
                                       C.c_int, C.c_int, C.c_int, C.c_void_p, C.c_void_p, C.c_void_p, C.c_void_p, C.c_void_p]),
    "mmlst_chunk_qlen": (C.c_int, [C.c_void_p, C.c_uint64, C.c_void_p, C.POINTER(C.c_int)]),
    "mmlst_score_runs_qc_dev": (C.c_int, [C.c_void_p, C.c_void_p, C.c_uint32] + [C.c_void_p] * 5 + [C.c_uint64, C.c_uint64, C.c_void_p, C.c_uint32,
                                          C.c_int, C.c_int, C.c_int, C.c_void_p, C.c_void_p, C.c_void_p, C.c_void_p, C.c_void_p]),
    "mmlst_expand_chunk_qlen_dev": (C.c_int, [C.c_void_p, C.c_uint64, C.c_void_p, C.c_void_p]),
    "mmlst_inflate_raw": (C.c_int, [C.c_void_p, C.c_size_t, C.c_void_p, C.c_size_t, C.POINTER(C.c_size_t)]),
    "mmlst_set_score_variant": (C.c_int, [C.c_int]),
    "mmlst_set_score_l2_hints": (C.c_int, [C.c_int]),
    "mmlst_set_score_grid_scale": (C.c_int, [C.c_int]),
    "mmlst_debug_timeline": (C.c_int, [C.c_void_p]),
    "mmlst_set_select_warp_finalize": (C.c_int, [C.c_int]),
    "mmlst_as_untransform_dev": (C.c_int, [C.c_void_p, C.c_void_p, C.c_uint64, C.c_int, C.c_void_p]),
    "mmlst_set_pdl": (C.c_int, [C.c_int]),
    "mmlst_expand_runs_dev": (C.c_int, [C.c_void_p, C.c_void_p, C.c_uint32, C.c_void_p, C.c_uint64, C.c_void_p, C.c_void_p]),
    "mmlst_coverage_table_slots": (C.c_uint64, [C.c_uint64]),
    "mmlst_coverage_dev": (C.c_int, [C.c_void_p] * 6 + [C.c_uint64, C.c_uint64, C.c_void_p, C.c_void_p, C.c_uint32, C.c_int, C.c_int,
                                     C.c_int, C.c_void_p, C.c_uint64, C.c_void_p, C.c_void_p]),
    "mmlst_coverage": (C.c_int, [C.c_void_p, C.POINTER(Soa), C.c_void_p, C.c_void_p, C.c_void_p, C.c_uint32, C.POINTER(ScoreParams),
                                 C.c_uint32, C.c_void_p]),
    "mmlst_pileup_dev": (C.c_int, [C.c_void_p] * 3 + [C.c_uint32, C.c_uint32, C.c_int, C.c_int, C.c_void_p, C.c_uint32,
                                   C.c_int, C.c_void_p]),
    "mmlst_consensus_dev": (C.c_int, [C.c_void_p, C.c_void_p, C.c_void_p, C.c_uint32, C.c_uint32, C.c_void_p, C.c_void_p,
                                      C.c_void_p, C.c_void_p]),
    "mmlst_hamming_min_dev": (C.c_int, [C.c_void_p, C.c_void_p, C.c_void_p, C.c_uint32, C.c_uint32, C.c_void_p, C.c_void_p,
                                        C.c_void_p, C.c_uint32, C.c_void_p, C.c_uint32, C.c_uint32, C.c_void_p, C.c_void_p]),
    "mmlst_hamming_min_dev2": (C.c_int, [C.c_void_p, C.c_void_p, C.c_void_p, C.c_uint32, C.c_uint32, C.c_void_p, C.c_void_p,
                                         C.c_void_p, C.c_uint32, C.c_void_p, C.c_uint32, C.c_uint32, C.c_uint32, C.c_uint32,
                                         C.c_void_p, C.c_void_p]),
    "mmlst_select_dev": (C.c_int, [C.c_void_p] * 6 + [C.c_uint32, C.c_void_p, C.c_void_p, C.c_uint32, C.c_uint32, C.c_int, C.c_int,
                                   C.c_void_p, C.c_void_p, C.c_void_p, C.c_uint32, C.c_void_p, C.c_size_t] + [C.c_void_p] * 6 +
                         [C.c_uint32, C.c_uint32, C.c_void_p, C.c_void_p, C.c_void_p]),
    "mmlst_pileup_indirect_dev": (C.c_int, [C.c_void_p] * 4 + [C.c_uint32, C.c_int, C.c_int, C.c_void_p, C.c_int, C.c_void_p]),
    "mmlst_consensus_indirect_dev": (C.c_int, [C.c_void_p] * 4 + [C.c_uint32, C.c_void_p, C.c_uint32, C.c_void_p, C.c_void_p, C.c_void_p,
                                                C.c_uint32, C.c_void_p]),
    "mmlst_pileup_consensus_indirect_dev": (C.c_int, [C.c_void_p] * 4 + [C.c_uint32, C.c_int, C.c_int, C.c_void_p, C.c_void_p, C.c_void_p, C.c_void_p, C.c_uint32,
                                                      C.c_uint32, C.c_void_p, C.c_void_p, C.c_void_p, C.c_uint32, C.c_void_p, C.c_void_p]),
    "mmlst_chunk_records": (C.c_uint32, [C.c_uint64]),
    "mmlst_contig_stats_scratch_bytes": (C.c_size_t, [C.c_uint32]),
    "mmlst_contig_stats_dev": (C.c_int, [C.c_void_p, C.c_void_p, C.c_uint32, C.c_uint32, C.POINTER(ContigStatsParams), C.c_void_p, C.c_size_t]
                               + [C.c_void_p] * 6 + [C.c_uint32, C.c_void_p]),
    "mmlst_contig_stats": (C.c_int, [C.c_void_p, C.POINTER(Soa), C.c_void_p, C.c_uint32, C.c_void_p, C.c_int, C.c_int,
                                     C.POINTER(ContigStatsParams), C.POINTER(ContigStatsOut)]),
    "mmlst_xchg_publish_dev": (C.c_int, [C.c_void_p, C.c_uint32, C.c_void_p, C.c_uint32, C.c_uint32, C.c_uint64, C.c_uint64, C.c_uint64,
                                         C.c_void_p, C.c_void_p]),
    "mmlst_xchg_await_dev": (C.c_int, [C.c_void_p, C.c_uint32, C.c_uint32, C.c_uint64, C.c_uint64, C.c_uint64, C.c_void_p, C.c_void_p,
                                       C.c_void_p, C.c_void_p, C.c_void_p]),
    "mmlst_depth_cap": (C.c_int, [C.c_void_p, C.c_void_p, C.c_void_p, C.c_uint64, C.c_uint32, C.c_uint32, C.c_void_p]),
    "mmlst_score": (C.c_int, [C.c_void_p, C.POINTER(Soa), C.c_void_p, C.c_void_p, C.c_uint32, C.POINTER(ScoreParams),
                              C.c_void_p, C.c_void_p, C.c_void_p, C.c_void_p]),
    "mmlst_pileup_consensus": (C.c_int, [C.c_void_p, C.POINTER(Soa), C.c_void_p, C.c_uint32, C.c_void_p, C.c_void_p, C.c_int,
                                         C.c_int, C.c_uint32, C.c_int, C.c_void_p, C.c_void_p, C.c_void_p, C.c_void_p]),
    "mmlst_db_upload": (C.c_int, [C.c_void_p, C.c_void_p, C.c_void_p, C.c_void_p, C.c_uint32, C.c_uint32]),
    "mmlst_db_upload_x": (C.c_int, [C.c_void_p, C.c_void_p, C.c_void_p, C.c_void_p, C.c_uint32, C.c_uint32, C.c_void_p, C.c_void_p,
                                    C.c_void_p, C.c_uint32]),
    "mmlst_hamming_min_x": (C.c_int, [C.c_void_p, C.c_void_p, C.c_void_p, C.c_void_p, C.c_uint32, C.c_void_p, C.c_void_p, C.c_void_p,
                                      C.c_uint32, C.c_void_p, C.c_uint32, C.c_void_p, C.c_void_p]),
    "mmlst_hamming_exact_dev": (C.c_int, [C.c_void_p, C.c_void_p, C.c_void_p, C.c_uint32, C.c_uint32, C.c_void_p, C.c_void_p, C.c_void_p,
                                          C.c_uint32, C.c_void_p, C.c_uint32, C.c_uint32, C.c_void_p, C.c_void_p, C.c_void_p, C.c_uint32,
                                          C.c_void_p, C.c_void_p, C.c_void_p, C.c_uint32, C.c_void_p, C.c_void_p]),
    "mmlst_exact_match_dev": (C.c_int, [C.c_void_p, C.c_void_p, C.c_void_p, C.c_uint32, C.c_uint32, C.c_void_p, C.c_void_p, C.c_void_p, C.c_uint32,
                                        C.c_void_p, C.c_uint32, C.c_uint32, C.c_uint32, C.c_void_p, C.c_void_p, C.c_void_p, C.c_uint32, C.c_void_p,
                                        C.c_void_p, C.c_uint32, C.c_void_p, C.c_void_p]),
    "mmlst_db_row_keys": (C.c_int, [C.c_void_p, C.c_void_p, C.c_uint32]),
    "mmlst_exact_match": (C.c_int, [C.c_void_p, C.c_void_p, C.c_void_p, C.c_void_p, C.c_uint32, C.c_void_p, C.c_void_p, C.c_uint32, C.c_void_p,
                                    C.c_uint32, C.c_void_p]),
    "mmlst_st_match_dev": (C.c_int, [C.c_void_p, C.c_void_p, C.c_uint32, C.c_void_p, C.c_void_p, C.c_uint32, C.c_uint32, C.c_void_p, C.c_void_p,
                                     C.c_void_p, C.c_void_p, C.c_uint32, C.c_void_p]),
    "mmlst_profiles_upload": (C.c_int, [C.c_void_p, C.c_void_p, C.c_void_p, C.c_uint32]),
    "mmlst_st_match": (C.c_int, [C.c_void_p, C.c_void_p, C.c_void_p, C.c_uint32, C.c_uint32, C.c_void_p, C.c_void_p, C.c_void_p, C.c_uint32]),
    "mmlst_bam_unpack": (C.c_int, [C.c_char_p, C.c_void_p, C.POINTER(C.c_void_p)]),
    "mmlst_bam_info": (C.c_int, [C.c_void_p, C.c_void_p]),
    "mmlst_bam_free": (None, [C.c_void_p]),
    "mmlst_hamming_min": (C.c_int, [C.c_void_p, C.c_void_p, C.c_void_p, C.c_void_p, C.c_uint32, C.c_void_p, C.c_uint32,
                                    C.c_void_p, C.c_void_p]),
    "mmlst_hamming_tc_image_bytes": (C.c_size_t, [C.c_uint32, C.c_uint32, C.c_uint32]),
    "mmlst_hamming_tc_expand_dev": (C.c_int, [C.c_void_p, C.c_void_p, C.c_void_p, C.c_uint32, C.c_uint32, C.c_int, C.c_uint32, C.c_void_p, C.c_void_p, C.c_void_p]),
    "mmlst_hamming_tc_search_dev": (C.c_int, [C.c_void_p, C.c_void_p, C.c_void_p, C.c_uint32, C.c_void_p, C.c_void_p, C.c_void_p, C.c_uint32, C.c_uint32,
                                              C.c_uint32, C.c_void_p, C.c_void_p]),
    "mmlst_ingest_trim": (C.c_int, [C.c_int]),
    "mmlst_comm_unique_id": (C.c_int, [C.c_void_p]),
    "mmlst_comm_create": (C.c_int, [C.c_void_p, C.c_int, C.c_int, C.c_int, C.POINTER(C.c_void_p)]),
    "mmlst_comm_destroy": (None, [C.c_void_p]),
    "mmlst_allreduce": (C.c_int, [C.c_void_p, C.c_void_p, C.c_size_t, C.c_void_p, C.c_size_t, C.c_void_p, C.c_size_t, C.c_void_p]),
    "mmlst_bam_ingest": (C.c_int, [C.c_int, C.c_void_p, C.c_size_t, C.c_void_p, C.c_void_p, C.POINTER(C.c_void_p)]),
    "mmlst_dev_bam_info": (C.c_int, [C.c_void_p, C.c_void_p]),
    "mmlst_dev_bam_free": (None, [C.c_void_p]),
    "mmlst_index_upload": (C.c_int, [C.c_void_p, C.c_void_p]),
    "mmlst_sample": (C.c_int, [C.c_void_p, C.c_void_p, C.c_void_p, C.c_void_p, C.c_void_p]),
}

_lib = None
SELECT_CONSUME, SELECT_SCRATCH_CLEAN, SELECT_LOCAL, CONSENSUS_CONSUME, COVERAGE_STREAM_RESIDENT = 1, 2, 4, 1, 1


def lib() -> C.CDLL:
    global _lib
    if _lib is None:
        if not os.path.exists(LIB_PATH):
            raise ImportError("%s is missing: run `python -c 'import __graft_entry__ as g; g.build()'` "
                              "(metamlst_b200 has no CPU fallback)" % LIB_PATH)
        l = C.CDLL(LIB_PATH)
        for name, (res, args) in EXPORTS.items():
            f = getattr(l, name)
            f.restype = res
            f.argtypes = args
        _lib = l
    return _lib


def check(rc: int) -> None:
    if rc != 0:
        raise MmlstError(rc, lib().mmlst_last_error().decode(errors="replace"))


def ptr(x) -> int:
    if x is None:
        return 0
    if hasattr(x, "data_ptr"):
        return x.data_ptr()
    return x.ctypes.data


class Context:

    def __init__(self, device: int = 0):
        self._h = C.c_void_p()
        check(lib().mmlst_create(device, C.byref(self._h)))
        self.device = device

    @property
    def handle(self):
        return self._h

    def close(self):
        if self._h:
            lib().mmlst_destroy(self._h)
            self._h = C.c_void_p()

    def __del__(self):
        try:
            self.close()
        except Exception:
            pass
```

metamlst_b200/packing.py:

```python
from __future__ import annotations

import ctypes as C
from dataclasses import dataclass
from typing import List, Optional, Sequence

import numpy as np

from . import native

BAM_FUNMAP = 0x4
BAM_FPROPER_PAIR = 0x2
DEFAULT_MAX_DEPTH = 8000
DEFAULT_MINQUAL = 20
PLANE_SLACK_WORDS = 8
PREC_DTYPE = np.dtype([("pos", "<i4"), ("row_off", "<u4"), ("reflen", "<u2"), ("as_named", "<i2"), ("xm_named", "u1"), ("pad", "u1"), ("nw", "<u2")])
assert PREC_DTYPE.itemsize == 16


@dataclass
class SoaHost:

    ref_names: List[str]
    ref_lens: np.ndarray
    tid: np.ndarray
    as0: np.ndarray
    xm3: np.ndarray
    qlen: np.ndarray
    orig_idx: Optional[np.ndarray]
    p_recs: np.ndarray
    planes: np.ndarray
    max_row_words: int
    contig_start: np.ndarray
    minqual: int = DEFAULT_MINQUAL
    max_depth: int = DEFAULT_MAX_DEPTH
    n_dropped_by_cap: int = 0
    _keep: tuple = ()
    qhash: Optional[np.ndarray] = None
    header_text: str = ""
    unpack_seconds: Optional[dict] = None
    run_tid: Optional[np.ndarray] = None
    run_start: Optional[np.ndarray] = None
    chunk_run: Optional[np.ndarray] = None
    chunk_qlen: Optional[np.ndarray] = None
    z_bytes: Optional[np.ndarray] = None
    z_table: Optional[np.ndarray] = None
    z_as_xm_coeff: int = 0
    zp_bytes: Optional[np.ndarray] = None
    zp_table: Optional[np.ndarray] = None
    zp_contig_block: Optional[np.ndarray] = None
    lenient: bool = False
    n_untagged: int = 0

    @property
    def n_rec(self) -> int:
        return int(self.tid.shape[0])

    @property
    def n_prec(self) -> int:
        return int(self.p_recs.shape[0])

    p_pos = property(lambda self: self.p_recs["pos"])
    p_reflen = property(lambda self: self.p_recs["reflen"])
    p_as = property(lambda self: self.p_recs["as_named"])
    p_xm = property(lambda self: self.p_recs["xm_named"])

    @property
    def p_row_off(self) -> np.ndarray:
        off = np.zeros(self.n_prec + 1, dtype=np.int64)
        off[:-1] = self.p_recs["row_off"]
        if self.n_prec:
            off[-1] = int(off[-2]) + int(row_words(self.p_recs["nw"][-1:])[0])
        return off

    def c_struct(self) -> native.Soa:
        s = native.Soa()
        s.tid, s.as0, s.xm3, s.qlen = native.ptr(self.tid), native.ptr(self.as0), native.ptr(self.xm3), native.ptr(self.qlen)
        s.orig_idx = native.ptr(self.orig_idx)
        s.n_rec = self.n_rec
        s.p_recs, s.planes = native.ptr(self.p_recs), native.ptr(self.planes)
        s.n_prec = self.n_prec
        s.n_plane_words = int(self.planes.shape[0])
        s.max_row_words = int(self.max_row_words)
        s.contig_start = native.ptr(self.contig_start)
        s.n_ref = len(self.ref_names)
        if self.run_tid is not None and self.n_rec:
            s.n_runs = int(self.run_tid.shape[0])
            s.run_tid, s.run_start, s.chunk_run = native.ptr(self.run_tid), native.ptr(self.run_start), native.ptr(self.chunk_run)
            if self.chunk_qlen is not None:
                s.chunk_qlen = native.ptr(self.chunk_qlen)
            if self.z_bytes is not None:
                zs = native.ZStream(native.ptr(self.z_bytes), int(self.z_bytes.shape[0]), native.ptr(self.z_table), int(self.z_table.shape[0]),
                                    int(self.z_as_xm_coeff))
                s._zs = zs
                s.z = C.addressof(zs)
        if self.zp_bytes is not None:
            zp = native.ZPileup(native.ptr(self.zp_bytes), int(self.zp_bytes.shape[0]), native.ptr(self.zp_table), int(self.zp_table.shape[0]),
                                native.ptr(self.zp_contig_block))
            s._zp = zp
            s.zp = C.addressof(zp)
        return s

    def deflate(self, level: int = 3, block: int = 1 << 16, threads: int = 0, pinned: bool = True, strategy: int = 0,
                cover: float = 1.0, pileup: bool = False, as_xm_coeff: Optional[int] = None) -> "SoaHost":
        import os
        import zlib
        from concurrent.futures import ThreadPoolExecutor
        self.z_bytes = self.z_table = None
        self.zp_bytes = self.zp_table = self.zp_contig_block = None
        if pileup and self.n_prec:
            self._deflate_pileup(level, block, threads, pinned, strategy)
        if self.run_tid is None or self.n_rec == 0:
            return self
        self.z_as_xm_coeff = 0
        as0 = np.ascontiguousarray(self.as0)
        stop_a = 2 * as0.shape[0] if cover >= 1.0 else int(2 * as0.shape[0] * max(cover, 0.0)) // block * block
        n_tr = stop_a // 2
        if n_tr and as_xm_coeff != 0:
            xm = np.ascontiguousarray(self.xm3)[:n_tr].astype(np.int32)
            a32 = as0[:n_tr].astype(np.int32)
            if as_xm_coeff is None:
                m0, m1 = max(0, n_tr // 2 - (1 << 17)), min(n_tr, n_tr // 2 + (1 << 17))
                best = None
                for c in range(0, 9):
                    t = a32[m0:m1] + c * xm[m0:m1]
                    if t.max(initial=0) > 32767 or t.min(initial=0) < -32768:
                        continue
                    size = len(zlib.compress(t.astype(np.int16).tobytes(), 1))
                    if best is None or size < best[0]:
                        best = (size, c)
                as_xm_coeff = best[1] if best else 0
            if as_xm_coeff:
                t = a32 + int(as_xm_coeff) * xm
                if t.max(initial=0) <= 32767 and t.min(initial=0) >= -32768:
                    as0 = np.concatenate([t.astype(np.int16), as0[n_tr:]])
                    self.z_as_xm_coeff = int(as_xm_coeff)
        jobs = []
        for kind, arr in ((0, as0.view(np.uint8)), (1, np.ascontiguousarray(self.xm3).view(np.uint8))):
            mv = memoryview(arr)
            stop = arr.shape[0] if cover >= 1.0 else int(arr.shape[0] * max(cover, 0.0)) // block * block
            for off in range(0, stop, block):
                jobs.append((kind, off, mv[off:min(off + block, stop)]))
        if not jobs:
            return self

        def one(job):
            co = zlib.compressobj(level, zlib.DEFLATED, -15, 8, strategy)
            return co.compress(job[2]) + co.flush()
        with ThreadPoolExecutor(threads or (os.cpu_count() or 1)) as pool:
            comp = list(pool.map(one, jobs))
        table = np.zeros((len(jobs), 4), np.uint64)
        pos = 0
        for i, ((kind, off, raw), c) in enumerate(zip(jobs, comp)):
            table[i] = (kind, off, pos, (len(c) << 32) | len(raw))
            pos += len(c)
        z = np.frombuffer(b"".join(comp), np.uint8)
        if pinned:
            import torch
            t = torch.from_numpy(z.copy()).pin_memory()
            self._keep = tuple(self._keep) + (t,)
            z = t.numpy()
        self.z_bytes, self.z_table = z, table
        return self

    def _deflate_pileup(self, level: int, block: int, threads: int, pinned: bool, strategy: int) -> None:
        import os
        import zlib
        from concurrent.futures import ThreadPoolExecutor
        cs = np.asarray(self.contig_start, dtype=np.int64)
        recs = np.ascontiguousarray(self.p_recs)
        rec_bytes = memoryview(recs.view(np.uint8).reshape(-1))
        plane_bytes = memoryview(np.ascontiguousarray(self.planes).view(np.uint8).reshape(-1))
        row_off = recs["row_off"].astype(np.int64)
        row_end = row_off + row_words(recs["nw"]).astype(np.int64)
        jobs = []
        per_contig = np.zeros(len(cs), np.int64)
        for t in np.nonzero(cs[1:] > cs[:-1])[0]:
            r0, r1 = int(cs[t]), int(cs[t + 1])
            for kind, mv, lo, hi in ((0, plane_bytes, int(row_off[r0]) * 4, int(row_end[r1 - 1]) * 4), (1, rec_bytes, r0 * 16, r1 * 16)):
                for off in range(lo, hi, block):
                    jobs.append((int(t), kind, mv[off:min(off + block, hi)]))
                    per_contig[t + 1] += 1

        def one(job):
            co = zlib.compressobj(level, zlib.DEFLATED, -15, 8, strategy)
            return co.compress(job[2]) + co.flush()
        with ThreadPoolExecutor(threads or (os.cpu_count() or 1)) as pool:
            comp = list(pool.map(one, jobs))
        table = np.zeros((len(jobs), 2), np.uint64)
        pos = 0
        for i, ((_t, kind, raw), c) in enumerate(zip(jobs, comp)):
            table[i] = (pos, (kind << 63) | (len(c) << 32) | len(raw))
            pos += len(c)
        z = np.frombuffer(b"".join(comp) + b"\0" * 64, np.uint8)
        if pinned:
            import torch
            t = torch.from_numpy(z.copy()).pin_memory()
            self._keep = tuple(self._keep) + (t,)
            z = t.numpy()
        self.zp_bytes, self.zp_table, self.zp_contig_block = z, table, np.cumsum(per_contig).astype(np.uint32)

    def build_runs(self, max_fraction: float = 0.125) -> "SoaHost":
        n = self.n_rec
        self.run_tid = self.run_start = self.chunk_run = self.chunk_qlen = None
        if n == 0:
            return self
        import ctypes as C
        lib = native.lib()
        nr = C.c_uint32(0)
        tid = np.ascontiguousarray(self.tid, dtype=np.uint32)
        native.check(lib.mmlst_build_runs(native.ptr(tid), n, None, None, None, C.byref(nr)))
        if nr.value > max_fraction * n:
            return self
        run_tid = np.empty(nr.value, np.uint32); run_start = np.empty(nr.value + 1, np.uint32); chunk_run = np.empty((n + 255) // 256, np.uint32)
        native.check(lib.mmlst_build_runs(native.ptr(tid), n, native.ptr(run_tid), native.ptr(run_start), native.ptr(chunk_run), C.byref(nr)))
        self.run_tid, self.run_start, self.chunk_run = run_tid, run_start, chunk_run
        cq = np.empty((n + 255) // 256, np.uint16)
        uniform = C.c_int(0)
        ql = np.ascontiguousarray(self.qlen, dtype=np.uint16)
        native.check(lib.mmlst_chunk_qlen(native.ptr(ql), n, native.ptr(cq), C.byref(uniform)))
        self.chunk_qlen = cq if uniform.value else None
        return self

    def pin(self) -> "SoaHost":
        import torch

        keep = []
        for name in ("tid", "as0", "xm3", "qlen", "orig_idx", "p_recs", "planes", "qhash", "run_tid", "run_start", "chunk_run", "chunk_qlen"):
            arr = getattr(self, name)
            if arr is None:
                continue
            t = torch.from_numpy(np.ascontiguousarray(arr).view(np.uint8).reshape(-1)).pin_memory()
            keep.append(t)
            setattr(self, name, t.numpy().view(arr.dtype).reshape(arr.shape))
        self._keep = tuple(keep)
        return self


def touched_words(pos: np.ndarray, reflen: np.ndarray) -> np.ndarray:
    pos = pos.astype(np.int64)
    reflen = reflen.astype(np.int64)
    return np.where(reflen > 0, ((pos & 31) + reflen + 31) >> 5, 0)


def row_words(nw: np.ndarray) -> np.ndarray:
    rw = 3 * nw.astype(np.int64)
    return rw + ((rw > 0) & ((rw & 1) == 0))


def project_cigars(cig_off: np.ndarray, cig_ops: np.ndarray, n: int):
    ncig = (cig_off[1:] - cig_off[:-1]).astype(np.int64)
    rec = np.repeat(np.arange(n, dtype=np.int64), ncig)
    op = (cig_ops & 0xF).astype(np.int64)
    ln = (cig_ops >> 4).astype(np.int64)
    cons_ref = np.isin(op, (0, 2, 3, 7, 8))
    cons_q = np.isin(op, (0, 1, 4, 7, 8))
    def seg_excl_cumsum(v):
        c = np.cumsum(v)
        start = c - v
        base = np.zeros(n + 1, dtype=np.int64)
        np.add.at(base, rec + 1, v)
        tot = base[1:]
        first = np.cumsum(tot) - tot
        return start - first[rec], tot
    ref_start, reflen = seg_excl_cumsum(ln * cons_ref)
    q_start, _ = seg_excl_cumsum(ln * cons_q)
    is_m = np.isin(op, (0, 7, 8))
    return reflen, rec[is_m], ref_start[is_m], q_start[is_m], ln[is_m]


def _pack_bits_u32(bits: np.ndarray) -> np.ndarray:
    return np.packbits(bits, axis=1, bitorder="little").view(np.uint32)


def pack_table(tab, minqual: int = DEFAULT_MINQUAL, max_depth: Optional[int] = DEFAULT_MAX_DEPTH, sentinel_nodes: int = 1,
               chunk: int = 1 << 18, run_fraction: float = 0.125) -> SoaHost:
    n = tab.n
    if n and np.any(tab.flag & BAM_FPROPER_PAIR):
        raise native.MmlstError(-6, "proper-pair records: htslib overlap handling (H2) is not implemented -- refusing")
    if n and np.any(tab.tid < 0):
        raise native.MmlstError(-4, "unmapped record (RNAME '*'): the reference crashes at metamlst.py:107")
    if n and (tab.AS.min() < -32768 or tab.AS.max() > 32767):
        raise native.MmlstError(-7, "AS outside int16")
    order = tab.coord_order()
    presorted = bool(np.all(order == np.arange(n)))
    L = tab.read_len
    aux3 = np.where(tab.has_xs, tab.XM, tab.XO)
    tid = tab.tid[order].astype(np.uint32)
    as0 = tab.AS[order].astype(np.int16)
    xm3 = np.clip(aux3[order], 0, 255).astype(np.uint8)
    if np.any(aux3 < 0):
        raise native.MmlstError(-7, "negative 4th aux field")
    qlen = np.full(n, max(L, 1), dtype=np.uint16)
    orig_idx = None if presorted else order.astype(np.uint32)

    reflen_all, seg_rec, seg_ref, seg_q, seg_len = project_cigars(tab.cig_off, tab.cig_ops, n)
    if n and reflen_all.max() > 65535:
        raise native.MmlstError(-7, "reference span > 65535")
    mapped = (tab.flag[order] & BAM_FUNMAP) == 0
    s_idx = order[mapped]
    p_tid = tab.tid[s_idx].astype(np.uint32)
    p_pos_all = tab.pos[s_idx].astype(np.int32)
    p_reflen_all = reflen_all[s_idx].astype(np.uint32)
    admitted = np.ones(s_idx.shape[0], dtype=np.uint8)
    if max_depth is not None and s_idx.shape[0]:
        native.check(native.lib().mmlst_depth_cap(native.ptr(p_tid), native.ptr(p_pos_all), native.ptr(p_reflen_all),
                                                   s_idx.shape[0], int(max_depth), int(sentinel_nodes), native.ptr(admitted)))
    adm = admitted.astype(bool)
    sel = s_idx[adm]
    P = sel.shape[0]
    p_pos = p_pos_all[adm]
    p_reflen = p_reflen_all[adm].astype(np.uint16)
    p_as = tab.AS[sel].astype(np.int16)
    p_xm = np.clip(tab.XM[sel], 0, 255).astype(np.uint8)
    p_nw = touched_words(p_pos, p_reflen)
    if P and p_nw.max() > 65535:
        raise native.MmlstError(-7, "record touches more than 65535 words")
    p_shift = p_pos.astype(np.int64) & 31
    rw = row_words(p_nw)
    p_row_off = np.zeros(P + 1, dtype=np.int64)
    p_row_off[1:] = np.cumsum(rw)
    if p_row_off[-1] + PLANE_SLACK_WORDS >= (1 << 32):
        raise native.MmlstError(-7, "plane array exceeds 2^32 words")
    planes = np.zeros(int(p_row_off[-1]) + PLANE_SLACK_WORDS, dtype=np.uint32)
    seg_order = np.argsort(seg_rec, kind="stable")
    seg_rec, seg_ref, seg_q, seg_len = seg_rec[seg_order], seg_ref[seg_order], seg_q[seg_order], seg_len[seg_order]
    seg_first = np.searchsorted(seg_rec, np.arange(n + 1))
    code_lut = np.full(256, 255, dtype=np.uint8)
    for i, ch in enumerate(b"ACGT"):
        code_lut[ch] = i
        code_lut[ch + 32] = i
    for c0 in range(0, P, chunk):
        idx = sel[c0:c0 + chunk]
        m = idx.shape[0]
        wmax = int(p_nw[c0:c0 + m].max()) if m else 0
        if wmax == 0:
            continue
        qidx = np.full((m, wmax * 32), -1, dtype=np.int64)
        s0, s1 = seg_first[idx], seg_first[idx + 1]
        nseg = s1 - s0
        sid = np.repeat(s0, nseg) + (np.arange(int(nseg.sum())) - np.repeat(np.cumsum(nseg) - nseg, nseg))
        row = np.repeat(np.arange(m), nseg)
        sl = seg_len[sid]
        tot = int(sl.sum())
        within = np.arange(tot) - np.repeat(np.cumsum(sl) - sl, sl)
        rr = np.repeat(row, sl)
        qidx[rr, np.repeat(seg_ref[sid], sl) + within + p_shift[c0:c0 + m][rr]] = np.repeat(seg_q[sid], sl) + within
        has = qidx >= 0
        qi = np.where(has, qidx, 0)
        base = tab.seq[idx][np.arange(m)[:, None], qi]
        ql = tab.qual[idx][np.arange(m)[:, None], qi]
        code = code_lut[base]
        qok = has & (ql >= minqual)
        V = qok & (code != 255)
        Nn = qok & (code == 255)
        B1 = V & ((code & 2) != 0)
        B0 = (V & ((code & 1) != 0)) | Nn
        Vw, B1w, B0w = _pack_bits_u32(V), _pack_bits_u32(B1), _pack_bits_u32(B0)
        nw = p_nw[c0:c0 + m]
        off = p_row_off[c0:c0 + m]
        for j in range(wmax):
            msk = nw > j
            o = off[msk] + 3 * j
            planes[o] = Vw[msk, j]
            planes[o + 1] = B1w[msk, j]
            planes[o + 2] = B0w[msk, j]
    n_ref = len(tab.ref_names)
    contig_start = np.searchsorted(tab.tid[sel], np.arange(n_ref + 1)).astype(np.uint64)
    recs = np.zeros(P, dtype=PREC_DTYPE)
    recs["pos"], recs["row_off"], recs["reflen"], recs["as_named"], recs["xm_named"] = p_pos, p_row_off[:-1], p_reflen, p_as, p_xm
    recs["nw"] = p_nw
    soa = SoaHost(list(tab.ref_names), np.asarray(tab.ref_lens, dtype=np.int32), tid, as0, xm3, qlen, orig_idx,
                  recs, planes, int(rw.max()) if P else 0, contig_start,
                  minqual, max_depth if max_depth is not None else 0, int((~adm).sum()))
    soa.qhash = qname_key(tab.qname_id[order])
    if run_fraction > 0:
        soa.build_runs(run_fraction)
    return soa


def qname_key(qname_id: np.ndarray) -> np.ndarray:
    k = np.zeros((qname_id.shape[0], 2), dtype=np.uint64)
    k[:, 0] = qname_id.astype(np.uint64)
    k[:, 1] = np.uint64(0x51ED270B0B1F2A37)
    return k



def _w_for(max_len: int) -> int:
    w = (max_len + 31) // 32
    for cand in (8, 16, 24, 32):
        if w <= cand:
            return cand
    if max_len < 0x8000:
        return (w + 7) // 8 * 8
    raise native.MmlstError(-7, "sequence of %d bases exceeds 32767" % max_len)


def encode_2bit_x(seqs: Sequence[bytes], W: int):
    n = len(seqs)
    lens = np.fromiter((len(s) for s in seqs), dtype=np.int64, count=n)
    if n and lens.max() > W * 32:
        raise native.MmlstError(-7, "sequence longer than W*32")
    lut = np.full(256, 255, dtype=np.uint8)
    for i, ch in enumerate(b"ACGT"):
        lut[ch] = i
    mat = np.zeros((n, W * 32), dtype=np.uint8)
    exc = np.zeros((n, W * 32), dtype=bool)
    flat = np.frombuffer(b"".join(seqs), dtype=np.uint8)
    rows = np.repeat(np.arange(n), lens)
    cols = np.arange(flat.shape[0]) - np.repeat(np.cumsum(lens) - lens, lens)
    codes = lut[flat]
    bad = codes == 255
    mat[rows, cols] = np.where(bad, 0, codes)
    exc[rows[bad], cols[bad]] = True
    hi = _pack_bits_u32((mat & 2) != 0)
    lo = _pack_bits_u32((mat & 1) != 0)
    ln = lens.astype(np.uint16)
    xids = np.nonzero(exc.any(axis=1))[0].astype(np.uint32)
    ln[xids] |= np.uint16(0x8000)
    xx = np.ascontiguousarray(_pack_bits_u32(exc[xids])) if xids.size else np.zeros((0, W), np.uint32)
    xbytes = np.zeros((xids.size, W * 32), dtype=np.uint8)
    for k, i in enumerate(xids):
        xbytes[k, : lens[i]] = np.frombuffer(seqs[int(i)], dtype=np.uint8)
    return np.ascontiguousarray(hi), np.ascontiguousarray(lo), ln, xids, xx, xbytes


def encode_2bit(seqs: Sequence[bytes], W: int):
    hi, lo, ln, xids, _xx, _xb = encode_2bit_x(seqs, W)
    if xids.size:
        raise native.MmlstError(-7, "non-ACGT letter in sequence %d: use encode_2bit_x (exact-character path, H9)" % int(xids[0]))
    return hi, lo, ln


def tile_db(hi: np.ndarray, lo: np.ndarray):
    n, W = hi.shape
    nt = (n + 31) // 32
    def t(x):
        p = np.zeros((nt * 32, W), dtype=np.uint32)
        p[:n] = x
        return np.ascontiguousarray(p.reshape(nt, 32, W).transpose(0, 2, 1)).reshape(-1)
    return t(hi), t(lo)
```

metamlst_b200/pipeline.py:

```python
from __future__ import annotations

import os
from typing import Callable, Dict, List, Optional, Sequence, Tuple

import numpy as np
import torch

from . import api, dist, native

def build_chunks(contig_start: np.ndarray, chosen_tid: Sequence[int], col_off: np.ndarray) -> np.ndarray:
    out = []
    total = sum(int(contig_start[t + 1]) - int(contig_start[t]) for t in chosen_tid)
    CHUNK_RECORDS = int(native.lib().mmlst_chunk_records(total))
    for l, t in enumerate(chosen_tid):
        r0, r1 = int(contig_start[t]), int(contig_start[t + 1])
        for b in range(r0, r1, CHUNK_RECORDS):
            out.append((b, min(r1, b + CHUNK_RECORDS), int(col_off[l]), int(col_off[l + 1] - col_off[l]), 0, 0, 0, 0))
    return np.asarray(out, dtype=np.uint32).reshape(-1, 8)


class DevicePipeline:
    def __init__(self, streams, index: api.AlleleIndex, dbseq_of: Callable[[int], str], minscore: int = 80, max_xM: int = 5,
                 min_read_len: int = 50, penalty: int = 100, species_filter: Optional[str] = None, mincov: int = 1,
                 impl: int = 0, idx_base: int = 0, group=None, nloci: int = 100, genes_in_db: Optional[Dict[str, int]] = None,
                 db_ascii: Optional[np.ndarray] = None, db_off: Optional[np.ndarray] = None, exchange: str = "allreduce",
                 use_runs: Optional[bool] = None):
        self.s = streams
        self._use_runs_arg, self._idx_base_arg = use_runs, idx_base
        self.index = index
        self.dbseq_of = dbseq_of
        self.minscore, self.max_xM, self.min_read_len, self.penalty = int(minscore), api.check_max_xm(max_xM), int(min_read_len), int(penalty)
        self.mincov, self.impl = int(mincov), int(impl)
        self.idx_base = int(idx_base) if idx_base else int(getattr(streams, "idx_base", 0) or 0)
        self.group = group
        self.dist = torch.distributed.is_available() and torch.distributed.is_initialized() and torch.distributed.get_world_size() > 1
        if exchange not in ("allreduce", "gather", "p2p"):
            raise ValueError("exchange must be 'allreduce', 'gather' or 'p2p'")
        self.owner = self.dist and exchange in ("gather", "p2p")
        self.p2p = self.dist and exchange == "p2p"
        self.world = torch.distributed.get_world_size() if self.dist else 1
        dev = streams.as0.device
        self.dev = dev
        self.use_runs = bool(use_runs) if use_runs is not None else getattr(streams, "run_tid", None) is not None
        self.use_qc = self.use_runs and getattr(streams, "chunk_qlen", None) is not None
        n_ref = len(index.ref_names)
        self.n_ref = n_ref
        self.allow = torch.from_numpy(index.allow_mask(species_filter)).to(dev)
        self.locus_of = torch.from_numpy(index.locus_of.astype(np.int32)).to(dev)
        self.max_cols = int(np.sort(np.asarray(streams.ref_lens))[::-1][: index.n_loci].sum())
        w_hit, w_cnt = (n_ref + 1) // 2, (self.max_cols * 5 + 8 + 1) // 2
        self.zblock = torch.zeros(n_ref + 2 + w_hit + w_cnt, dtype=torch.int64, device=dev)
        self.zscore = self.zblock[: n_ref + 2 + w_hit]
        self.sum_as = self.zblock[:n_ref]
        self.counters = self.zblock[n_ref:n_ref + 2]
        self.n_hit = self.zblock[n_ref + 2:n_ref + 2 + w_hit].view(torch.int32)[:n_ref]
        self.counts = self.zblock[n_ref + 2 + w_hit:].view(torch.int32)[: self.max_cols * 5 + 8]
        self.first_idx = torch.zeros(n_ref, dtype=torch.int32, device=dev)
        self._db_cache: Dict[Tuple[int, ...], tuple] = {}
        self.lib = native.lib()
        self.nloci = int(nloci)
        species_names: List[str] = []
        sp_id: Dict[str, int] = {}
        sol = np.zeros(index.n_loci, dtype=np.int32)
        for l, (sp, _g) in enumerate(index.locus_names):
            if sp not in sp_id:
                sp_id[sp] = len(species_names)
                species_names.append(sp)
            sol[l] = sp_id[sp]
        self.species_names = species_names
        gdb = np.zeros(len(species_names), dtype=np.int32)
        for sp, i in sp_id.items():
            gdb[i] = (genes_in_db or {}).get(sp, int((sol == i).sum()))
        if db_ascii is None:
            seqs = [dbseq_of(t).encode("latin-1") for t in range(n_ref)]
            db_off = np.zeros(n_ref + 1, dtype=np.int64)
            db_off[1:] = np.cumsum([len(x) for x in seqs])
            db_ascii = np.frombuffer(b"".join(seqs), dtype=np.uint8)
        self.bad_len = np.asarray(streams.ref_lens, dtype=np.int64) > (db_off[1:] - db_off[:-1])
        t32 = lambda a: torch.from_numpy(np.ascontiguousarray(a)).to(dev)
        self.allele_num = t32(np.asarray([int(a) for a in index.allele], dtype=np.int64).astype(np.uint32).view(np.int32))
        self.species_of_locus = t32(sol)
        self.genes_in_db = t32(gdb)
        self.ref_len_d = t32(np.asarray(streams.ref_lens, dtype=np.int32))
        self.contig_start_d = torch.zeros(n_ref + 1, dtype=torch.int64, device=dev)
        self.max_chunks = 0
        self.rebind(streams)
        self.db_ascii_d = t32(np.concatenate([db_ascii, np.zeros(8, np.uint8)]))
        self.db_off_d = t32(np.asarray(db_off, dtype=np.int64))
        nl = index.n_loci
        self.scratch = torch.zeros(nl * 12 + 64, dtype=torch.uint8, device=dev)
        order = np.argsort(index.locus_of, kind="stable").astype(np.uint32)
        self.locus_rows = None if np.array_equal(order, np.arange(order.shape[0], dtype=order.dtype)) else t32(order.view(np.int32))
        self.locus_start = t32(np.searchsorted(index.locus_of[order], np.arange(nl + 1)).astype(np.int32))
        self.o_hdr, self.o_tid, self.o_sp, self.o_col, self.o_holes, self.o_snps = 0, 16, 16 + nl, 16 + 2 * nl, 17 + 3 * nl, 17 + 4 * nl
        self.o_first = 17 + 5 * nl
        self.n_small = (17 + 6 * nl + 7) // 4 * 4
        self.out = torch.zeros((self.n_small * 4 + self.max_cols + 16 + 15) // 16 * 16, dtype=torch.uint8, device=dev)
        self.small = self.out[: self.n_small * 4].view(torch.int32)
        self.cons = self.out[self.n_small * 4:]
        self.holes = self.small[self.o_holes:self.o_holes + nl]
        self.snps = self.small[self.o_snps:self.o_snps + nl]
        self.db_start_d = torch.zeros(nl + 1, dtype=torch.int64, device=dev)
        self.out_bytes = int(self.out.shape[0])
        if self.owner:
            self.out_all = torch.zeros(self.world * self.out_bytes + 16, dtype=torch.uint8, device=dev)
            self.out_h = torch.zeros(self.world * self.out_bytes + 16, dtype=torch.uint8).pin_memory()
            if self.p2p:
                self._init_p2p()
        else:
            self.out_h = torch.zeros(self.out_bytes, dtype=torch.uint8).pin_memory()
        self.small_h = self.out_h[: self.n_small * 4].view(torch.int32)
        self.cons_h = self.out_h[self.n_small * 4: self.out_bytes]
        self.genes_in_db_h = gdb
        self.ticket = torch.zeros(nl + 8, dtype=torch.int32, device=dev)
        self.fused_tail = os.environ.get("MMLST_FUSED_TAIL", "0") == "1"
        self.want_tables = False
        self._tables_h = None
        self._clean = False
        self.timers: Optional[Dict[str, list]] = None
        self.launches = 0

    def rebind(self, streams):
        if list(streams.ref_names) != self.index.ref_names or not np.array_equal(np.asarray(streams.ref_lens), np.asarray(self.s.ref_lens)):
            raise ValueError("rebind: the sample was aligned against a different reference set")
        self.s = streams
        self.use_runs = getattr(streams, "run_tid", None) is not None if self._use_runs_arg is None else bool(self._use_runs_arg)
        self.use_qc = self.use_runs and getattr(streams, "chunk_qlen", None) is not None
        self.idx_base = int(self._idx_base_arg) if self._idx_base_arg else int(getattr(streams, "idx_base", 0) or 0)
        self.contig_start_d.copy_(torch.from_numpy(np.asarray(streams.contig_start, dtype=np.uint64).view(np.int64)), non_blocking=False)
        need = int(streams.n_prec) // 512 + self.index.n_loci + 8
        if need > self.max_chunks:
            self.max_chunks = need
            self.chunks_d = torch.zeros(self.max_chunks * 8, dtype=torch.int32, device=self.dev)
        self.graph = None

    def _timed(self, name: str, fn):
        if self.timers is None:
            fn()
            return
        a, b = torch.cuda.Event(enable_timing=True), torch.cuda.Event(enable_timing=True)
        a.record()
        fn()
        b.record()
        self.timers.setdefault(name, []).append((a, b))

    def _stream(self):
        return torch.cuda.current_stream(self.dev).cuda_stream

    def reset_tables(self):
        self.zblock.zero_(); self.first_idx.fill_(-1); self.scratch.zero_(); self.ticket.zero_()
        self._clean = True

    def _score_call(self):
        s = self.s
        n = int(s.as0.shape[0])
        oi = native.ptr(getattr(s, "orig_idx", None))
        if n == 0:
            return
        if self.use_runs and self.use_qc:
            native.check(self.lib.mmlst_score_runs_qc_dev(native.ptr(s.run_tid), native.ptr(s.run_start), int(s.run_tid.shape[0]), native.ptr(s.chunk_run),
                                                          native.ptr(s.chunk_qlen), native.ptr(s.as0), native.ptr(s.xm3), oi, n, self.idx_base,
                                                          native.ptr(self.allow), self.n_ref, self.minscore, self.max_xM, self.min_read_len,
                                                          native.ptr(self.sum_as), native.ptr(self.n_hit), native.ptr(self.first_idx),
                                                          native.ptr(self.counters), self._stream()))
        elif self.use_runs:
            native.check(self.lib.mmlst_score_runs_dev(native.ptr(s.run_tid), native.ptr(s.run_start), int(s.run_tid.shape[0]), native.ptr(s.chunk_run),
                                                       native.ptr(s.as0), native.ptr(s.xm3), native.ptr(s.qlen), oi, n, self.idx_base,
                                                       native.ptr(self.allow), self.n_ref, self.minscore, self.max_xM, self.min_read_len,
                                                       native.ptr(self.sum_as), native.ptr(self.n_hit), native.ptr(self.first_idx),
                                                       native.ptr(self.counters), self._stream()))
        else:
            native.check(self.lib.mmlst_score_dev(native.ptr(s.tid), native.ptr(s.as0), native.ptr(s.xm3), native.ptr(s.qlen), oi, n, self.idx_base,
                                                  native.ptr(self.allow), native.ptr(self.locus_of), self.n_ref, self.minscore, self.max_xM,
                                                  self.min_read_len, native.ptr(self.sum_as), native.ptr(self.n_hit), native.ptr(self.first_idx),
                                                  native.ptr(self.counters), self._stream()))

    def run_score(self, reset: bool = True):
        s = self.s
        if reset:
            self.reset_tables()
        self._clean = False
        self._timed("score", self._score_call)
        self.launches += 1
        if self.dist and not self.owner:
            dist.allreduce_score_block(self.zscore, self.first_idx, self.group)

    def run_coverage(self, timed: bool = False):
        s = self.s
        if getattr(s, "qhash", None) is None:
            raise ValueError("streams were packed without QNAME keys (want_qhash)")
        n = int(s.tid.shape[0])
        slots = int(self.lib.mmlst_coverage_table_slots(n))
        if getattr(self, "_cov_table", None) is None or self._cov_table.shape[0] < slots * 3:
            self._cov_table = torch.empty(slots * 3, dtype=torch.int64, device=self.dev)
            self._cov = torch.zeros(self.index.n_loci, dtype=torch.int64, device=self.dev)
        ev = [torch.cuda.Event(enable_timing=True) for _ in range(3)]
        ev[0].record()
        self._cov_table[: slots * 3].zero_(); self._cov.zero_()
        ev[1].record()
        native.check(self.lib.mmlst_coverage_dev(native.ptr(s.tid), native.ptr(s.as0), native.ptr(s.xm3), native.ptr(s.qlen), 0, native.ptr(s.qhash),
                                                 n, self.idx_base, native.ptr(self.allow), native.ptr(self.locus_of), self.n_ref, self.minscore,
                                                 self.max_xM, self.min_read_len, native.ptr(self._cov_table), slots, native.ptr(self._cov),
                                                 self._stream()))
        ev[2].record()
        self.launches += 2
        if self.dist:
            torch.distributed.all_reduce(self._cov, group=self.group)
        cov = self._cov.cpu().numpy()
        out = {sp + "_" + g: int(cov[l]) for l, (sp, g) in enumerate(self.index.locus_names) if cov[l]}
        if timed:
            return out, {"memset_ms": ev[0].elapsed_time(ev[1]), "kernels_ms": ev[1].elapsed_time(ev[2]), "table_bytes": slots * 24}
        return out

    def select(self):
        sum_as = self.sum_as.cpu().numpy()
        n_hit = self.n_hit.cpu().numpy().view(np.uint32)
        first = self.first_idx.cpu().numpy().view(np.uint32)
        return api.fast_select(self.index, sum_as, n_hit, first, self.penalty), (sum_as, n_hit, first)

    def _db_for(self, tids: Tuple[int, ...]):
        hit = self._db_cache.get(tids)
        if hit is None:
            lens = [int(self.s.ref_lens[t]) for t in tids]
            col_off = np.zeros(len(tids) + 1, dtype=np.uint32)
            col_off[1:] = np.cumsum(lens)
            db = np.zeros(int(col_off[-1]) + 8, dtype=np.uint8)
            for i, t in enumerate(tids):
                sq = self.dbseq_of(t)
                if len(sq) < lens[i]:
                    raise IndexError("string index out of range: BAM LN > DB sequence length for %s" % self.index.ref_names[t])
                db[col_off[i]:col_off[i + 1]] = np.frombuffer(sq[:lens[i]].encode("latin-1"), dtype=np.uint8)
            hit = (col_off, torch.from_numpy(db).to(self.dev), torch.from_numpy(col_off.view(np.int32)).to(self.dev))
            if len(self._db_cache) > 64:
                self._db_cache.clear()
            self._db_cache[tids] = hit
        return hit

    def run_pileup_consensus(self, tids: Sequence[int]):
        tids = tuple(int(t) for t in tids)
        s = self.s
        col_off, db_d, col_off_d = self._db_for(tids)
        total = int(col_off[-1])
        chunks = build_chunks(s.contig_start, tids, col_off)
        self.counts[: total * 5].zero_()
        if chunks.shape[0]:
            chunks_d = torch.from_numpy(chunks.view(np.int32)).to(self.dev, non_blocking=True)
            def k():
                native.check(self.lib.mmlst_pileup_dev(native.ptr(s.p_recs), native.ptr(s.planes), native.ptr(chunks_d), int(chunks.shape[0]),
                                                       int(s.max_row_words), self.minscore, self.max_xM, native.ptr(self.counts), total,
                                                       self.impl, self._stream()))
            self._timed("pileup", k)
            self.launches += 1
        if self.dist:
            dist.allreduce_counts(self.counts[: total * 5], self.group)
        def k2():
            native.check(self.lib.mmlst_consensus_dev(native.ptr(self.counts), native.ptr(db_d), native.ptr(col_off_d), len(tids), self.mincov,
                                                      native.ptr(self.cons), native.ptr(self.holes), native.ptr(self.snps), self._stream()))
        self._timed("consensus", k2)
        self.launches += 1
        cons = self.cons[:total].cpu().numpy()
        holes = self.holes[: len(tids)].cpu().numpy()
        snps = self.snps[: len(tids)].cpu().numpy()
        return [cons[col_off[i]:col_off[i + 1]].tobytes().decode("latin-1") for i in range(len(tids))], holes, snps, col_off

    def _select_call(self, flags: int):
        sm, nl = self.small, self.index.n_loci
        base = sm.data_ptr()
        native.check(self.lib.mmlst_select_dev(native.ptr(self.sum_as), native.ptr(self.n_hit), native.ptr(self.first_idx), native.ptr(self.locus_rows),
                                               native.ptr(self.locus_start), native.ptr(self.allele_num), self.n_ref, native.ptr(self.species_of_locus),
                                               native.ptr(self.genes_in_db), nl, len(self.species_names), self.penalty, self.nloci,
                                               native.ptr(self.contig_start_d), native.ptr(self.ref_len_d), native.ptr(self.db_off_d),
                                               int(os.environ.get("MMLST_CHUNK_RECORDS", "0")),
                                               native.ptr(self.scratch), int(self.scratch.shape[0]), base + 4 * self.o_hdr, base + 4 * self.o_tid,
                                               base + 4 * self.o_sp, base + 4 * self.o_col, native.ptr(self.db_start_d), native.ptr(self.chunks_d),
                                               self.max_chunks, flags | (native.SELECT_LOCAL if self.owner else 0), native.ptr(self.counters),
                                               base + 4 * self.o_first, self._stream()))

    def _consensus_call(self, flags: int):
        nl = self.index.n_loci
        base = self.small.data_ptr()
        native.check(self.lib.mmlst_consensus_indirect_dev(native.ptr(self.counts), native.ptr(self.db_ascii_d), native.ptr(self.db_start_d),
                                                           base + 4 * self.o_col, nl, base + 4 * self.o_hdr, self.mincov, native.ptr(self.cons),
                                                           base + 4 * self.o_holes, base + 4 * self.o_snps, flags, self._stream()))

    def _pileup_call(self):
        s = self.s
        native.check(self.lib.mmlst_pileup_indirect_dev(native.ptr(s.p_recs), native.ptr(s.planes), native.ptr(self.chunks_d),
                                                        self.small.data_ptr() + 4 * self.o_hdr, int(s.max_row_words), self.minscore, self.max_xM,
                                                        native.ptr(self.counts), self.impl, self._stream()))

    def _pileup_consensus_call(self, flags: int):
        s, nl = self.s, self.index.n_loci
        base = self.small.data_ptr()
        native.check(self.lib.mmlst_pileup_consensus_indirect_dev(
            native.ptr(s.p_recs), native.ptr(s.planes), native.ptr(self.chunks_d), base + 4 * self.o_hdr, int(s.max_row_words), self.minscore, self.max_xM,
            native.ptr(self.counts), native.ptr(self.db_ascii_d), native.ptr(self.db_start_d), base + 4 * self.o_col, nl, self.mincov, native.ptr(self.cons),
            base + 4 * self.o_holes, base + 4 * self.o_snps, flags, native.ptr(self.ticket), self._stream()))

    def _enqueue(self):
        if not self._clean:
            self.reset_tables()
        self.run_score(reset=False)
        if self.want_tables:
            self._enqueue_tables()
        self._timed("select", lambda: self._select_call(native.SELECT_CONSUME | native.SELECT_SCRATCH_CLEAN))
        self.launches += 1
        if self.fused_tail and self.impl != 1 and not (self.dist and not self.owner):
            self._timed("pileup+consensus", lambda: self._pileup_consensus_call(native.CONSENSUS_CONSUME))
            self.launches += 1
        else:
            self._timed("pileup", self._pileup_call)
            self.launches += 1
            if self.dist and not self.owner:
                dist.allreduce_counts(self.counts, self.group)
            self._timed("consensus", lambda: self._consensus_call(native.CONSENSUS_CONSUME))
            self.launches += 1
        if self.p2p:
            native.check(self.lib.mmlst_xchg_publish_dev(native.ptr(self.out), self.out_bytes, native.ptr(self.peer_base), self.rank, self.world,
                                                         self.x_half, self.x_slot, self.x_flag_off, native.ptr(self.x_epoch), self._stream()))
            native.check(self.lib.mmlst_xchg_await_dev(native.ptr(self.xbuf), self.out_bytes, self.world, self.x_half, self.x_slot, self.x_flag_off,
                                                       native.ptr(self.out_all), native.ptr(self.x_epoch), native.ptr(self.x_ticket),
                                                       self.out_all.data_ptr() + self.world * self.out_bytes, self._stream()))
            self.launches += 2
            self.out_h.copy_(self.out_all, non_blocking=True)
        elif self.owner:
            torch.distributed.all_gather_into_tensor(self.out_all[: self.world * self.out_bytes], self.out, group=self.group)
            self.out_h.copy_(self.out_all, non_blocking=True)
        else:
            self.out_h.copy_(self.out, non_blocking=True)
        self._clean = True

    def time_kernels(self, reps: int = 20, alt: Optional["DevicePipeline"] = None, flush: Optional[torch.Tensor] = None) -> Dict[str, float]:
        pipes = [self] + ([alt] if alt is not None else [])
        for p in pipes:
            p.reset_tables()
            p.run_score(reset=False)
            p._select_call(native.SELECT_SCRATCH_CLEAN)
        torch.cuda.current_stream(self.dev).synchronize()
        out: Dict[str, float] = {}
        saved = [p.dist for p in pipes]
        for p in pipes:
            p.dist = False
        try:
            for name in ("select", "pileup", "consensus", "score"):
                for p in pipes:
                    p._launch_one(name)
                if name == "score" or flush is None:
                    a, b = torch.cuda.Event(enable_timing=True), torch.cuda.Event(enable_timing=True)
                    a.record()
                    for i in range(reps):
                        pipes[i % len(pipes)]._launch_one(name)
                    b.record()
                    b.synchronize()
                    out[name] = a.elapsed_time(b) / reps
                else:
                    pairs = []
                    for i in range(reps):
                        flush.zero_()
                        a, b = torch.cuda.Event(enable_timing=True), torch.cuda.Event(enable_timing=True)
                        a.record()
                        pipes[i % len(pipes)]._launch_one(name)
                        b.record()
                        pairs.append((a, b))
                    torch.cuda.current_stream(self.dev).synchronize()
                    out[name] = float(np.mean([a.elapsed_time(b) for a, b in pairs]))
        finally:
            for p, d in zip(pipes, saved):
                p.dist = d
                p._clean = False
        return out

    def time_score_variants(self, reps: int = 20, alt: Optional["DevicePipeline"] = None) -> Dict[str, float]:
        pipes = [self] + ([alt] if alt is not None else [])
        out: Dict[str, float] = {}
        want = None
        keys = ["0", "1", "2", "3", "4", "5", "2h", "3h", "4h", "5h"]
        if self.use_qc:
            keys += ["6", "6h", "6g10", "6g12"]
        grid0 = self.lib.mmlst_set_score_grid_scale(-1)
        for key in keys:
            v = int(key[0])
            self.lib.mmlst_set_score_variant(v)
            self.lib.mmlst_set_score_l2_hints(1 if key[1:2] == "h" else 0)
            self.lib.mmlst_set_score_grid_scale(int(key.split("g")[1]) if "g" in key else grid0)
            self.reset_tables()
            self._score_call()
            torch.cuda.current_stream(self.dev).synchronize()
            got = [self.zscore.clone(), self.first_idx.clone()]
            if want is None:
                want = got
            assert all(torch.equal(a, b) for a, b in zip(got, want)), "score kernel form %s disagrees with form 0" % key
            for p in pipes:
                p._score_call()
            a, b = torch.cuda.Event(enable_timing=True), torch.cuda.Event(enable_timing=True)
            a.record()
            for i in range(reps):
                pipes[i % len(pipes)]._score_call()
            b.record()
            b.synchronize()
            out[key] = a.elapsed_time(b) / reps
        self.lib.mmlst_set_score_grid_scale(grid0)
        for p in pipes:
            p._clean = False
        return out

    def time_score_half(self, reps: int = 20, alt: Optional["DevicePipeline"] = None) -> Dict[str, float]:
        pipes = [self] + ([alt] if alt is not None else [])
        out: Dict[str, float] = {}
        full = [p.s.as0 for p in pipes]
        n = int(self.s.as0.shape[0])
        try:
            for frac in (1, 2, 4):
                m = (n // frac) & ~255
                for p, f in zip(pipes, full):
                    p.s.as0 = f[:m]
                for p in pipes:
                    p._score_call()
                a, b = torch.cuda.Event(enable_timing=True), torch.cuda.Event(enable_timing=True)
                a.record()
                for i in range(reps):
                    pipes[i % len(pipes)]._score_call()
                b.record()
                b.synchronize()
                out["1/%d" % frac] = a.elapsed_time(b) / reps
        finally:
            for p, f in zip(pipes, full):
                p.s.as0 = f
                p._clean = False
        return out

    def _launch_one(self, name: str):
        s = self.s
        if name == "score":
            self._score_call()
        elif name == "select":
            self._select_call(native.SELECT_SCRATCH_CLEAN)
        elif name == "pileup":
            self._pileup_call()
        elif name == "consensus":
            self._consensus_call(0)
        else:
            raise ValueError(name)

    def _init_p2p(self):
        import torch.distributed._symmetric_memory as symm
        grp = self.group if self.group is not None else torch.distributed.group.WORLD
        self.rank = torch.distributed.get_rank(grp)
        self.x_slot = (self.out_bytes + 127) // 128 * 128
        self.x_half = self.world * self.x_slot
        self.x_flag_off = 2 * self.x_half
        self.xbuf = symm.empty(self.x_flag_off + 128 * ((8 * self.world + 127) // 128), dtype=torch.uint8, device=self.dev)
        self.xbuf.zero_()
        torch.cuda.synchronize(self.dev)
        self.xhdl = symm.rendezvous(self.xbuf, grp)
        ptrs = [int(x) for x in self.xhdl.buffer_ptrs]
        assert len(ptrs) == self.world and ptrs[self.rank] == self.xbuf.data_ptr(), "symmetric buffer: unexpected peer table"
        self.peer_base = torch.tensor(ptrs, dtype=torch.int64, device=self.dev)
        self.x_epoch = torch.zeros(1, dtype=torch.int64, device=self.dev)
        self.x_ticket = torch.zeros(1, dtype=torch.int32, device=self.dev)
        torch.cuda.synchronize(self.dev)
        torch.distributed.barrier(grp)

    def _finish_owner(self):
        nl = self.index.n_loci
        blocks, total, ignored = [], 0, 0
        if self.p2p and int(self.out_h[self.world * self.out_bytes:].view(torch.int32)[0]) != 0:
            raise RuntimeError("peer-memory exchange timed out waiting for a peer's result block")
        for r in range(self.world):
            blk = self.out_h[r * self.out_bytes:(r + 1) * self.out_bytes]
            h = blk[: self.n_small * 4].view(torch.int32).numpy()
            cons = blk[self.n_small * 4:].numpy()
            n = int(h[0])
            total += int(h[6:8].view(np.uint64)[0]); ignored += int(h[8:10].view(np.uint64)[0])
            if h[3] & 2:
                raise RuntimeError("chunk list overflow")
            tids = h[self.o_tid:self.o_tid + n]
            if self.bad_len[tids].any():
                raise IndexError("string index out of range: BAM LN > DB sequence length (metaMLST_functions.py:267)")
            col = h[self.o_col:self.o_col + n + 1]
            blocks.append({"tid": tids.tolist(), "species": h[self.o_sp:self.o_sp + n].tolist(),
                           "first": h[self.o_first:self.o_first + n].view(np.uint32).tolist(),
                           "payload": [(cons[col[i]:col[i + 1]].tobytes().decode("latin-1"), int(h[self.o_holes + i]), int(h[self.o_snps + i])) for i in range(n)]})
        self.total_reads, self.ignored_reads = total, ignored
        merged = dist.merge_owner_blocks(blocks, self.species_names, self.genes_in_db_h, self.nloci)
        return {sp: [(self.index.ref_names[t], seq, holes, snps) for t, (seq, holes, snps) in lst] for sp, lst in merged}

    def _finish(self):
        if self.owner:
            return self._finish_owner()
        h = self.small_h.numpy()
        n = int(h[0])
        self.total_reads = int(h[6:8].view(np.uint64)[0])
        self.ignored_reads = int(h[8:10].view(np.uint64)[0])
        if h[3] & 1:
            raise RuntimeError("Database is broken: a species has more detected loci than the genes table lists (metamlst.py:188)")
        if h[3] & 2:
            raise RuntimeError("chunk list overflow")
        tids = h[self.o_tid:self.o_tid + n]
        if self.bad_len[tids].any():
            raise IndexError("string index out of range: BAM LN > DB sequence length (metaMLST_functions.py:267)")
        col = h[self.o_col:self.o_col + n + 1]
        cons = self.cons_h.numpy()
        out: Dict[str, list] = {}
        for i in range(n):
            out.setdefault(self.species_names[int(h[self.o_sp + i])], []).append(
                (self.index.ref_names[int(tids[i])], cons[col[i]:col[i + 1]].tobytes().decode("latin-1"), int(h[self.o_holes + i]), int(h[self.o_snps + i])))
        return out

    def _enqueue_tables(self):
        if self._tables_h is None:
            self._tables_h = (torch.zeros(self.zscore.shape[0], dtype=torch.int64).pin_memory(), torch.zeros(self.n_ref, dtype=torch.int32).pin_memory())
        self._tables_h[0].copy_(self.zscore, non_blocking=True)
        self._tables_h[1].copy_(self.first_idx, non_blocking=True)

    def tables(self):
        z, f = self._tables_h
        n = self.n_ref
        return z[:n].numpy(), z[n + 2:].view(torch.int32)[:n].numpy().view(np.uint32), f.numpy().view(np.uint32)

    def step(self):
        self._enqueue()
        torch.cuda.current_stream(self.dev).synchronize()
        return self._finish()

    def capture(self):
        assert self.timers is None, "per-kernel timers are not capturable"
        self._enqueue()
        torch.cuda.synchronize(self.dev)
        n0 = self.launches
        self.graph = torch.cuda.CUDAGraph()
        with torch.cuda.graph(self.graph):
            self._enqueue()
        self.launches_per_step = self.launches - n0
        self.launches = n0

    def step_graph(self):
        if not self._clean:
            self.reset_tables()
        self.graph.replay()
        self.launches += self.launches_per_step
        torch.cuda.current_stream(self.dev).synchronize()
        return self._finish()

    def enqueue_step(self):
        if getattr(self, "graph", None) is not None:
            if not self._clean:
                self.reset_tables()
            self.graph.replay()
            self.launches += self.launches_per_step
        else:
            self._enqueue()

    def collect(self):
        torch.cuda.current_stream(self.dev).synchronize()
        return self._finish()

    def step_host_select(self):
        self.run_score()
        chosen, _raw = self.select()
        tids = [t for _sp, ts in chosen for t in ts]
        out: Dict[str, list] = {}
        if tids:
            seqs, holes, snps, _ = self.run_pileup_consensus(tids)
            i = 0
            for sp, ts in chosen:
                for t in ts:
                    out.setdefault(sp, []).append((self.index.ref_names[t], seqs[i], int(holes[i]), int(snps[i])))
                    i += 1
        return out


class CohortLanes:

    def __init__(self, make_pipe: Callable[[int], "DevicePipeline"], n_lanes: int = 2):
        self.pipes = [make_pipe(lane) for lane in range(n_lanes)]
        self.dev = self.pipes[0].dev
        self.streams = [torch.cuda.Stream(device=self.dev) for _ in range(n_lanes)]
        self.captured = False

    def warm_and_capture(self, graph: bool = True):
        res = []
        for p, st in zip(self.pipes, self.streams):
            with torch.cuda.stream(st):
                r = p.step()
                if graph:
                    p.capture()
                    assert p.step_graph() == r, "graph replay differs from the eager pass"
                res.append(r)
        self.captured = graph
        torch.cuda.synchronize(self.dev)
        return res

    def enqueue(self, i: int) -> None:
        lane = i % len(self.pipes)
        with torch.cuda.stream(self.streams[lane]):
            self.pipes[lane].enqueue_step()

    def fork(self, event: "torch.cuda.Event") -> None:
        for st in self.streams:
            st.wait_event(event)

    def join(self) -> None:
        cur = torch.cuda.current_stream(self.dev)
        for st in self.streams:
            ev = torch.cuda.Event()
            ev.record(st)
            cur.wait_event(ev)

    def collect(self):
        out = []
        for p, st in zip(self.pipes, self.streams):
            with torch.cuda.stream(st):
                out.append(p.collect())
        return out

    @property
    def launches(self) -> int:
        return sum(p.launches for p in self.pipes)


def device_select(index: api.AlleleIndex, sum_as: np.ndarray, n_hit: np.ndarray, first_idx: np.ndarray, penalty: int = 100,
                  nloci: int = 100, genes_in_db: Optional[Dict[str, int]] = None, device: str = "cuda:0"):
    lib = native.lib()
    dev = torch.device(device)
    n_ref, nl = len(index.ref_names), index.n_loci
    names: List[str] = []
    sid: Dict[str, int] = {}
    sol = np.zeros(nl, np.int32)
    for l, (sp, _g) in enumerate(index.locus_names):
        if sp not in sid:
            sid[sp] = len(names)
            names.append(sp)
        sol[l] = sid[sp]
    gdb = np.asarray([(genes_in_db or {}).get(sp, int((sol == i).sum())) for i, sp in enumerate(names)], np.int32)
    d = lambda a: torch.from_numpy(np.ascontiguousarray(a)).to(dev)
    t_sum, t_n, t_f = d(sum_as.astype(np.int64)), d(n_hit.astype(np.uint32).view(np.int32)), d(first_idx.astype(np.uint32).view(np.int32))
    order = np.argsort(index.locus_of, kind="stable").astype(np.uint32)
    identity = np.array_equal(order, np.arange(order.shape[0], dtype=order.dtype))
    t_rows, t_start = (None if identity else d(order.view(np.int32))), d(np.searchsorted(index.locus_of[order], np.arange(nl + 1)).astype(np.int32))
    t_an = d(np.asarray([int(a) for a in index.allele], np.int64).astype(np.uint32).view(np.int32))
    t_sol, t_gdb = d(sol), d(gdb)
    t_cs, t_rl, t_dbo = d(np.zeros(n_ref + 1, np.int64)), d(np.ones(n_ref, np.int32)), d(np.zeros(n_ref + 1, np.int64))
    scratch = torch.zeros(nl * 12 + 64, dtype=torch.uint8, device=dev)
    small = torch.zeros(16 + 3 * nl + 8, dtype=torch.int32, device=dev)
    dbs = torch.zeros(nl + 1, dtype=torch.int64, device=dev)
    chunks = torch.zeros(8 * (nl + 8), dtype=torch.int32, device=dev)
    base = small.data_ptr()
    native.check(lib.mmlst_select_dev(native.ptr(t_sum), native.ptr(t_n), native.ptr(t_f), native.ptr(t_rows), native.ptr(t_start), native.ptr(t_an),
                                      n_ref, native.ptr(t_sol), native.ptr(t_gdb), nl, len(names), int(penalty), int(nloci), native.ptr(t_cs),
                                      native.ptr(t_rl), native.ptr(t_dbo), 0, native.ptr(scratch), int(scratch.shape[0]), base,
                                      base + 4 * 16, base + 4 * (16 + nl), base + 4 * (16 + 2 * nl), native.ptr(dbs), native.ptr(chunks), nl + 8,
                                      0, 0, 0, torch.cuda.current_stream(dev).cuda_stream))
    h = small.cpu().numpy()
    n = int(h[0])
    out: Dict[str, List[int]] = {}
    for i in range(n):
        out.setdefault(names[int(h[16 + nl + i])], []).append(int(h[16 + i]))
    return list(out.items()), int(h[3])
```

metamlst_b200/streams.py:

```python
from __future__ import annotations

from typing import List, Optional

import numpy as np
import torch

from . import packing


class DeviceStreams:

    def __init__(self):
        self.ref_names: List[str] = []
        self.ref_lens: Optional[np.ndarray] = None

    def to_host(self, pinned: bool = True) -> packing.SoaHost:
        def h(t, dt):
            a = t.detach().cpu().numpy()
            return a.view(dt) if a.dtype != dt else a
        recs = self.p_recs.detach().cpu().numpy().reshape(-1).view(packing.PREC_DTYPE)
        oi = getattr(self, "orig_idx", None)
        soa = packing.SoaHost(self.ref_names, self.ref_lens, h(self.tid, np.uint32), h(self.as0, np.int16), h(self.xm3, np.uint8),
                              h(self.qlen, np.uint16), None if oi is None else h(oi, np.uint32), recs, h(self.planes, np.uint32),
                              int(self.max_row_words), self.contig_start.copy(), self.minqual, self.max_depth, self.n_dropped)
        if getattr(self, "run_tid", None) is not None:
            soa.run_tid, soa.run_start, soa.chunk_run = h(self.run_tid, np.uint32), h(self.run_start, np.uint32), h(self.chunk_run, np.uint32)
            if getattr(self, "chunk_qlen", None) is not None:
                soa.chunk_qlen = h(self.chunk_qlen, np.uint16)
        return soa.pin() if pinned else soa

    def build_runs(self) -> "DeviceStreams":
        n = int(self.tid.shape[0])
        self.run_tid = self.run_start = self.chunk_run = self.chunk_qlen = None
        if n == 0:
            return self
        assert n < 0xffffff00
        vals, counts = torch.unique_consecutive(self.tid, return_counts=True)
        start = torch.zeros(vals.shape[0] + 1, dtype=torch.int64, device=self.tid.device)
        start[1:] = torch.cumsum(counts, 0)
        first = torch.arange(0, n, 256, dtype=torch.int64, device=self.tid.device)
        self.chunk_run = (torch.searchsorted(start, first, right=True) - 1).to(torch.int32).contiguous()
        self.run_tid = vals.to(torch.int32).contiguous()
        self.run_start = start.to(torch.int32).contiguous()
        nc = (n + 255) // 256
        q = self.qlen.to(torch.int32)
        pad = torch.full((nc * 256 - n,), int(q[-1].item()), dtype=torch.int32, device=q.device)
        q2 = torch.cat([q, pad]).view(nc, 256)
        if bool((q2 == q2[:, :1]).all().item()):
            self.chunk_qlen = q2[:, 0].to(torch.int16).contiguous()
        return self

    def slice_ranges(self, rank: int, world: int) -> "DeviceStreams":
        if world <= 1:
            return self
        dev = self.as0.device
        n, P = int(self.tid.shape[0]), int(self.n_prec)
        a, b = (n * rank) // world, (n * (rank + 1)) // world
        p0, p1 = (P * rank) // world, (P * (rank + 1)) // world
        s = DeviceStreams()
        s.ref_names, s.ref_lens = self.ref_names, self.ref_lens
        s.minqual, s.max_depth, s.n_dropped = self.minqual, self.max_depth, getattr(self, "n_dropped", 0)
        s.tid, s.as0, s.xm3, s.qlen = self.tid[a:b].contiguous(), self.as0[a:b].contiguous(), self.xm3[a:b].contiguous(), self.qlen[a:b].contiguous()
        oi = getattr(self, "orig_idx", None)
        s.orig_idx = None if oi is None else oi[a:b].contiguous()
        s.idx_base = (int(getattr(self, "idx_base", 0) or 0) + a) if oi is None else 0
        qh = getattr(self, "qhash", None)
        s.qhash = None if qh is None else qh[a:b].contiguous()
        total_words = int(self.planes.shape[0]) - packing.PLANE_SLACK_WORDS
        off = lambda j: (int(self.p_recs[j, 1].item()) & 0xFFFFFFFF) if j < P else total_words
        w0, w1 = (off(p0), off(p1)) if p1 > p0 else (0, 0)
        recs = self.p_recs[p0:p1].clone()
        if w0 and p1 > p0:
            recs[:, 1] = ((recs[:, 1].to(torch.int64) & 0xFFFFFFFF) - w0).to(torch.int32)
        s.p_recs = recs
        s.planes = torch.cat([self.planes[w0:w1], torch.zeros(packing.PLANE_SLACK_WORDS, dtype=torch.int32, device=dev)])
        s.n_prec, s.max_row_words = p1 - p0, int(self.max_row_words)
        cs = np.asarray(self.contig_start, dtype=np.int64)
        s.contig_start = (np.clip(cs, p0, p1) - p0).astype(np.uint64)
        s.run_tid = s.run_start = s.chunk_run = s.chunk_qlen = None
        if getattr(self, "run_tid", None) is not None and b > a:
            s.build_runs()
            if int(s.run_tid.shape[0]) > 0.125 * (b - a):
                s.run_tid = s.run_start = s.chunk_run = s.chunk_qlen = None
        return s

    @classmethod
    def from_soa(cls, soa: packing.SoaHost, device, rank: int = 0, world: int = 1, mode: str = "ranges",
                 locus_of: Optional[np.ndarray] = None, want_qhash: bool = False, stream=None) -> "DeviceStreams":
        dev = torch.device(device)
        s = cls()
        s.ref_names = list(soa.ref_names)
        s.ref_lens = np.asarray(soa.ref_lens, dtype=np.int32)
        s.minqual, s.max_depth, s.n_dropped = int(soa.minqual), int(soa.max_depth or 0), int(soa.n_dropped_by_cap)
        n, P = soa.n_rec, soa.n_prec
        s.idx_base = 0
        s.orig_idx = None
        s.qhash = None

        def up(a, dt=None):
            a = np.ascontiguousarray(a)
            if dt is not None and a.dtype != dt:
                a = a.view(dt)
            t = torch.from_numpy(a)
            return t.to(dev, non_blocking=True)

        if world > 1 and mode not in ("ranges", "loci"):
            raise ValueError("mode must be 'ranges' or 'loci'")
        if world > 1 and mode == "loci":
            if locus_of is None:
                raise ValueError("mode='loci' needs locus_of[tid]")
            keep = (np.asarray(locus_of)[soa.tid] % world) == rank
            sel = np.nonzero(keep)[0]
            tid, as0, xm3, qlen = soa.tid[sel], soa.as0[sel], soa.xm3[sel], soa.qlen[sel]
            oi = (soa.orig_idx[sel] if soa.orig_idx is not None else sel).astype(np.uint32)
            p0, p1 = 0, P
            qh = soa.qhash[sel] if (want_qhash and soa.qhash is not None) else None
            whole_runs = False
        else:
            a, b = (n * rank) // world, (n * (rank + 1)) // world
            tid, as0, xm3, qlen = soa.tid[a:b], soa.as0[a:b], soa.xm3[a:b], soa.qlen[a:b]
            oi = soa.orig_idx[a:b] if soa.orig_idx is not None else None
            s.idx_base = a if oi is None else 0
            p0, p1 = (P * rank) // world, (P * (rank + 1)) // world
            qh = soa.qhash[a:b] if (want_qhash and soa.qhash is not None) else None
            whole_runs = world == 1
        s.tid, s.as0, s.xm3, s.qlen = up(tid, np.int32), up(as0), up(xm3), up(qlen, np.int16)
        if oi is not None:
            s.orig_idx = up(oi, np.int32)
        if qh is not None:
            s.qhash = up(qh, np.int64)
        recs = soa.p_recs[p0:p1]
        if p1 > p0:
            off = soa.p_row_off
            w0, w1 = int(off[p0]), int(off[p1])
            if w0:
                recs = recs.copy()
                recs["row_off"] -= np.uint32(w0)
            planes = soa.planes[w0:w1]
        else:
            planes = soa.planes[:0]
        s.p_recs = up(recs.view(np.int32).reshape(-1, 4)) if p1 > p0 else torch.zeros((0, 4), dtype=torch.int32, device=dev)
        s.planes = torch.cat([up(planes, np.int32), torch.zeros(packing.PLANE_SLACK_WORDS, dtype=torch.int32, device=dev)])
        s.n_prec = p1 - p0
        s.max_row_words = int(soa.max_row_words)
        cs = np.asarray(soa.contig_start, dtype=np.int64)
        s.contig_start = (np.clip(cs, p0, p1) - p0).astype(np.uint64)
        s.run_tid = s.run_start = s.chunk_run = s.chunk_qlen = None
        if whole_runs and soa.run_tid is not None:
            s.run_tid, s.run_start, s.chunk_run = up(soa.run_tid, np.int32), up(soa.run_start, np.int32), up(soa.chunk_run, np.int32)
            if soa.chunk_qlen is not None:
                s.chunk_qlen = up(soa.chunk_qlen, np.int16)
        elif soa.run_tid is not None and int(s.tid.shape[0]):
            s.build_runs()
            if int(s.run_tid.shape[0]) > 0.125 * int(s.tid.shape[0]):
                s.run_tid = s.run_start = s.chunk_run = s.chunk_qlen = None
        return s
```

Measured before the change: 1202 billion.

## Pack alignment score and mismatch count into 16-bit words for scoring

Adds a preprocessing step that computes the min/max of the alignment scores and mismatch counts, then packs each record's offset score and mismatch count into one 16-bit word when they fit. A new ring-buffered scoring kernel reads these words and applies both thresholds with SWAR bit tricks and dp2a sums, and the default score variant becomes 7. This cuts the bytes streamed per record from three (int16 plus u8) to two and should reduce memory traffic in the bandwidth-bound scoring pass. The cost is an extra packing pass with a host sync at ingest, and the word path only applies when the value ranges fit in 16 bits and there is no orig_idx.

```diff
diff --git a/include/mmlst.h b/include/mmlst.h
--- a/include/mmlst.h
+++ b/include/mmlst.h
@@ -55,13 +55,20 @@
                             uint64_t n_rec, uint64_t idx_base, const uint8_t* allow, uint32_t n_ref,
                             int minscore, int max_xm, int min_read_len,
                             int64_t* sum_as, uint32_t* n_hit, uint32_t* first_idx, uint64_t* counters, void* stream);
-#define MMLST_SCORE_VARIANT_DEFAULT 6
+#define MMLST_SCORE_VARIANT_DEFAULT 7
 int mmlst_set_score_variant(int variant);
 #define MMLST_SCORE_L2_HINTS_DEFAULT 1
 int mmlst_set_score_l2_hints(int on);
 int mmlst_debug_timeline(uint64_t* dev_buf);
 #define MMLST_SCORE_GRID_DEFAULT 8
 int mmlst_set_score_grid_scale(int eighths);
+int mmlst_score_words_dev(const int16_t* as0, const uint8_t* xm3, uint64_t n_rec, uint16_t* words, uint32_t* scratch, int* amin, int* abits,
+                          int* fits, void* stream);
+int mmlst_score_runs_words_dev(const uint32_t* run_tid, const uint32_t* run_start, uint32_t n_runs, const uint32_t* chunk_run,
+                               const uint16_t* chunk_qlen, const uint16_t* words, int amin, int abits, const uint32_t* orig_idx,
+                               uint64_t n_rec, uint64_t idx_base, const uint8_t* allow, uint32_t n_ref,
+                               int minscore, int max_xm, int min_read_len,
+                               int64_t* sum_as, uint32_t* n_hit, uint32_t* first_idx, uint64_t* counters, void* stream);
 int mmlst_as_untransform_dev(int16_t* as0, const uint8_t* xm3, uint64_t n, int coeff, void* stream);
 int mmlst_expand_chunk_qlen_dev(const uint16_t* chunk_qlen, uint64_t n_rec, uint16_t* qlen, void* stream);
 int mmlst_expand_runs_dev(const uint32_t* run_tid, const uint32_t* run_start, uint32_t n_runs, const uint32_t* chunk_run,
diff --git a/metamlst_b200/bam.py b/metamlst_b200/bam.py
--- a/metamlst_b200/bam.py
+++ b/metamlst_b200/bam.py
@@ -193,11 +193,12 @@
     s.planes = t(info.planes, int(info.n_plane_words), "<i4", torch.int32)
     s.n_prec, s.max_row_words = P, int(info.max_row_words)
     s.contig_start = _view(info.contig_start, n_ref + 1, np.uint64).copy()
-    s.run_tid = s.run_start = s.chunk_run = s.chunk_qlen = None
+    s.run_tid = s.run_start = s.chunk_run = s.chunk_qlen = s.words = None
     if nr and nr <= 0.125 * n:
         s.run_tid, s.run_start = t(info.run_tid, nr, "<i4", torch.int32), t(info.run_start, nr + 1, "<i4", torch.int32)
         s.chunk_run = t(info.chunk_run, (n + 255) // 256, "<i4", torch.int32)
         s.chunk_qlen = t(info.chunk_qlen, (n + 255) // 256, "<i2", torch.int16) if info.chunk_qlen else None
+    s.build_words()
     s.presorted = bool(info.presorted)
     s.ingest_seconds = dict(zip(("h2d", "inflate", "chain", "parse", "sort", "score_stream", "cap_compact", "pack"), [float(x) for x in info.seconds]))
     s.ingest_stats = {"bgzf_blocks": int(info.n_bgzf_blocks), "compressed_bytes": int(info.compressed_bytes), "inflated_bytes": int(info.inflated_bytes),
diff --git a/metamlst_b200/csrc/score_runs.cu b/metamlst_b200/csrc/score_runs.cu
--- a/metamlst_b200/csrc/score_runs.cu
+++ b/metamlst_b200/csrc/score_runs.cu
@@ -7,13 +7,13 @@
 static int score_variant() {
     if (g_score_variant < 0) {
         const char* e = getenv("MMLST_SCORE_VARIANT");
-        g_score_variant = (e && e[0] >= '0' && e[0] <= '6' && !e[1]) ? e[0] - '0' : MMLST_SCORE_VARIANT_DEFAULT;
+        g_score_variant = (e && e[0] >= '0' && e[0] <= '7' && !e[1]) ? e[0] - '0' : MMLST_SCORE_VARIANT_DEFAULT;
     }
     return g_score_variant;
 }
 extern "C" int mmlst_set_score_variant(int v) {
     const int prev = score_variant();
-    if (v >= 0 && v <= 6) g_score_variant = v;
+    if (v >= 0 && v <= 7) g_score_variant = v;
     return prev;
 }
 
@@ -69,7 +69,7 @@
     const int variant = score_variant();
     const cudaStream_t st = static_cast<cudaStream_t>(stream);
     const bool tma_ok = !orig_idx && !(reinterpret_cast<uintptr_t>(xm3) & 15);
-    if (variant == 6 && tma_ok && chunk_qlen) {
+    if ((variant == 6 || variant == 7) && tma_ok && chunk_qlen) {
         static int pair_resident_by_device[MMLST_MAX_DEVICES] = {0};
         int& pair_resident = pair_resident_by_device[mmlst_current_device()];
         const size_t smem = (kThreads / 32) * 2u * (4u * 768u + sizeof(uint64_t));
@@ -92,7 +92,7 @@
         int (&ring_resident)[4][8] = ring_resident_by_device[mmlst_current_device()];
         const int hint = a.l2_hints ? 1 : 0;
         const int q = (chunk_qlen ? 1 : 0) + 2 * hint;
-        const int rv = variant == 6 ? 5 : variant;
+        const int rv = variant >= 6 ? 5 : variant;
         const RingCfg cfg = chunk_qlen ? (hint ? ring_config<true, true>(rv) : ring_config<true, false>(rv))
                                        : (hint ? ring_config<false, true>(rv) : ring_config<false, false>(rv));
         const size_t smem = (kThreads / 32) * static_cast<size_t>(cfg.ns) * (cfg.ch * (chunk_qlen ? 768u : 1280u) + sizeof(uint64_t));
@@ -147,6 +147,99 @@
     if (n_rec && !chunk_qlen) { mmlst_set_error("mmlst_score_runs_qc_dev: null pointer"); return MMLST_E_ARG; }
     return score_runs_launch(run_tid, run_start, n_runs, chunk_run, as0, xm3, nullptr, chunk_qlen, orig_idx, n_rec, idx_base, allow, n_ref,
                              minscore, max_xm, min_read_len, sum_as, n_hit, first_idx, counters, stream);
+}
+
+extern "C" int mmlst_score_runs_words_dev(const uint32_t* run_tid, const uint32_t* run_start, uint32_t n_runs, const uint32_t* chunk_run,
+                                          const uint16_t* chunk_qlen, const uint16_t* words, int amin, int abits, const uint32_t* orig_idx,
+                                          uint64_t n_rec, uint64_t idx_base, const uint8_t* allow, uint32_t n_ref, int minscore,
+                                          int max_xm, int min_read_len, int64_t* sum_as, uint32_t* n_hit, uint32_t* first_idx,
+                                          uint64_t* counters, void* stream) {
+    if (n_rec == 0) return MMLST_OK;
+    if (!run_tid || !run_start || !chunk_run || !n_runs || !chunk_qlen || !words || !allow || !sum_as || !n_hit || !first_idx || !counters) {
+        mmlst_set_error("mmlst_score_runs_words_dev: null pointer");
+        return MMLST_E_ARG;
+    }
+    if (orig_idx) { mmlst_set_error("mmlst_score_runs_words_dev: the word form has no file-order index (use mmlst_score_runs_qc_dev)"); return MMLST_E_ARG; }
+    if (reinterpret_cast<uintptr_t>(words) & 15) { mmlst_set_error("mmlst_score_runs_words_dev: words must be 16-byte aligned"); return MMLST_E_ARG; }
+    if (abits < 0 || abits > 16 || amin < -32768 || amin > 32767) {
+        mmlst_set_error("mmlst_score_runs_words_dev: abits %d / amin %d outside the word form", abits, amin);
+        return MMLST_E_ARG;
+    }
+    if (n_rec >= 0xffffff00ull) { mmlst_set_error("mmlst_score_runs_words_dev: %llu records do not fit 32-bit run offsets", (unsigned long long)n_rec); return MMLST_E_RANGE; }
+    RunArgs a{run_tid, run_start, chunk_run, n_runs, nullptr, nullptr, nullptr, nullptr, chunk_qlen, n_rec, idx_base, allow, n_ref, minscore, max_xm,
+              min_read_len, reinterpret_cast<long long*>(sum_as), n_hit, first_idx, reinterpret_cast<unsigned long long*>(counters), score_l2_hints(),
+              words, amin, abits};
+    struct WC { void (*k)(const RunArgs); uint32_t ch, ns; };
+    static const WC cfgs[] = {{score_runs_ring_words_kernel<4, 2, 4>, 4, 2}, {score_runs_ring_words_kernel<4, 3, 4>, 4, 3}, {score_runs_ring_words_kernel<8, 2, 3>, 8, 2},
+                              {score_runs_ring_words_kernel<2, 4, 4>, 2, 4}, {score_runs_ring_words_kernel<8, 3, 2>, 8, 3}, {score_runs_ring_words_kernel<4, 4, 3>, 4, 4}};
+    const char* ev = getenv("MMLST_WORDS_CFG");
+    const int ci = ev ? atoi(ev) : 0;
+    const WC cfg = cfgs[ci];
+    static int words_resident_by_device[MMLST_MAX_DEVICES][8] = {{0}};
+    int& words_resident = words_resident_by_device[mmlst_current_device()][ci];
+    const size_t smem = (kThreads / 32) * cfg.ns * (cfg.ch * 512u + sizeof(uint64_t));
+    if (!words_resident) {
+        CUDA_TRY(cudaFuncSetAttribute(cfg.k, cudaFuncAttributeMaxDynamicSharedMemorySize, static_cast<int>(smem)));
+        CUDA_TRY(cudaFuncSetAttribute(cfg.k, cudaFuncAttributePreferredSharedMemoryCarveout, cudaSharedmemCarveoutMaxShared));
+        int r = 0;
+        if (cudaOccupancyMaxActiveBlocksPerMultiprocessor(&r, cfg.k, kThreads, smem) != cudaSuccess || r < 1) r = 1;
+        words_resident = r;
+    }
+    uint64_t want = ((n_rec >> 8) + 15) / 16;
+    const uint64_t cap = static_cast<uint64_t>(mmlst_num_sms()) * words_resident * score_grid8() / 8;
+    if (want > cap) want = cap;
+    if (want < 1) want = 1;
+    cfg.k<<<static_cast<unsigned>(want), kThreads, smem, static_cast<cudaStream_t>(stream)>>>(a);
+    CUDA_TRY(cudaGetLastError());
+    return MMLST_OK;
+}
+
+namespace {
+__global__ void __launch_bounds__(256) words_range_kernel(const int16_t* __restrict__ as0, const uint8_t* __restrict__ xm3, uint64_t n, uint32_t* __restrict__ r) {
+    uint32_t lo = 0, hi = 0, xm = 0;
+    const uint64_t stride = static_cast<uint64_t>(gridDim.x) * blockDim.x;
+    for (uint64_t i = static_cast<uint64_t>(blockIdx.x) * blockDim.x + threadIdx.x; i < n; i += stride) {
+        const uint32_t a = static_cast<uint32_t>(static_cast<int>(as0[i]) + 32768);
+        lo = max(lo, 65535u - a); hi = max(hi, a); xm = max(xm, static_cast<uint32_t>(xm3[i]));
+    }
+    lo = __reduce_max_sync(FULL, lo); hi = __reduce_max_sync(FULL, hi); xm = __reduce_max_sync(FULL, xm);
+    if ((threadIdx.x & 31u) == 0) { atomicMax(r + 0, lo); atomicMax(r + 1, hi); atomicMax(r + 2, xm); }
+}
+__global__ void __launch_bounds__(256) words_pack_kernel(const int16_t* __restrict__ as0, const uint8_t* __restrict__ xm3, uint64_t n, int amin, int abits,
+                                                         uint16_t* __restrict__ words) {
+    const uint64_t stride = static_cast<uint64_t>(gridDim.x) * blockDim.x;
+    for (uint64_t i = static_cast<uint64_t>(blockIdx.x) * blockDim.x + threadIdx.x; i < n; i += stride)
+        words[i] = static_cast<uint16_t>((static_cast<uint32_t>(xm3[i]) << abits) | static_cast<uint32_t>(static_cast<int>(as0[i]) - amin));
+}
+int bit_width(uint32_t v) { return v ? 32 - __builtin_clz(v) : 0; }
+}
+
+extern "C" int mmlst_score_words_dev(const int16_t* as0, const uint8_t* xm3, uint64_t n_rec, uint16_t* words, uint32_t* scratch, int* amin, int* abits,
+                                     int* fits, void* stream) {
+    if (!amin || !abits || !fits) { mmlst_set_error("mmlst_score_words_dev: null pointer"); return MMLST_E_ARG; }
+    *amin = 0; *abits = 0; *fits = 0;
+    if (n_rec == 0) return MMLST_OK;
+    if (!as0 || !xm3 || !words || !scratch) { mmlst_set_error("mmlst_score_words_dev: null pointer"); return MMLST_E_ARG; }
+    if (reinterpret_cast<uintptr_t>(words) & 15) { mmlst_set_error("mmlst_score_words_dev: words must be 16-byte aligned"); return MMLST_E_ARG; }
+    const cudaStream_t st = static_cast<cudaStream_t>(stream);
+    uint64_t blocks = (n_rec + 255) / 256;
+    const uint64_t cap = static_cast<uint64_t>(mmlst_num_sms()) * 8;
+    if (blocks > cap) blocks = cap;
+    CUDA_TRY(cudaMemsetAsync(scratch, 0, 3 * sizeof(uint32_t), st));
+    words_range_kernel<<<static_cast<unsigned>(blocks), 256, 0, st>>>(as0, xm3, n_rec, scratch);
+    CUDA_TRY(cudaGetLastError());
+    uint32_t r[3];
+    CUDA_TRY(cudaMemcpyAsync(r, scratch, sizeof(r), cudaMemcpyDeviceToHost, st));
+    CUDA_TRY(cudaStreamSynchronize(st));
+    const int lo = 32767 - static_cast<int>(r[0]), hi = static_cast<int>(r[1]) - 32768;
+    const int ba = bit_width(static_cast<uint32_t>(hi - lo)), bx = bit_width(r[2]);
+    *amin = lo; *abits = ba;
+    if (ba + bx > 16) return MMLST_OK;
+    words_pack_kernel<<<static_cast<unsigned>(blocks), 256, 0, st>>>(as0, xm3, n_rec, lo, ba, words);
+    CUDA_TRY(cudaGetLastError());
+    CUDA_TRY(cudaStreamSynchronize(st));
+    *fits = 1;
+    return MMLST_OK;
 }
 
 extern "C" int mmlst_expand_chunk_qlen_dev(const uint16_t* chunk_qlen, uint64_t n_rec, uint16_t* qlen, void* stream) {
diff --git a/metamlst_b200/csrc/score_runs_kernels.cuh b/metamlst_b200/csrc/score_runs_kernels.cuh
--- a/metamlst_b200/csrc/score_runs_kernels.cuh
+++ b/metamlst_b200/csrc/score_runs_kernels.cuh
@@ -15,6 +15,7 @@
     int minscore, max_xm, min_read_len;
     long long* sum_as; uint32_t* n_hit; uint32_t* first_idx; unsigned long long* counters;
     int l2_hints;
+    const uint16_t* words; int amin, abits;
 };
 
 __device__ __forceinline__ void flush_run(const RunArgs& a, uint32_t key, long long s, uint32_t c, uint32_t mn) {
@@ -579,6 +580,217 @@
     }
 }
 
+struct WordThr {
+    uint32_t am;
+    uint32_t ta_T, ta_TL;
+    uint32_t tx_T, tx_TH;
+    uint32_t h8;
+};
+
+__device__ __forceinline__ WordThr make_word_thr(const RunArgs& a) {
+    WordThr t;
+    const uint32_t amask = (1u << a.abits) - 1u;
+    const long long ta = static_cast<long long>(a.minscore) - a.amin;
+    const long long tx = a.max_xm < 0 ? 0ll : min((static_cast<long long>(a.max_xm) + 1) << a.abits, 65536ll) - 1;
+    const bool none = a.max_xm < 0 || ta > static_cast<long long>(amask);
+    const uint32_t tau = static_cast<uint32_t>(min(max(ta, 0ll), static_cast<long long>(amask)));
+    t.am = amask | (amask << 16);
+    t.ta_T = tau | (tau << 16); t.ta_TL = t.ta_T & ~H16;
+    t.tx_T = static_cast<uint32_t>(tx) | (static_cast<uint32_t>(tx) << 16); t.tx_TH = t.tx_T | H16;
+    t.h8 = none ? 0u : H8;
+    return t;
+}
+
+struct Words8 { uint32_t m[4]; uint32_t p_lo, p_hi; };
+
+__device__ __forceinline__ Words8 word_pass(const uint4 w8, const WordThr& t, uint32_t cq, int min_read_len) {
+    Words8 r;
+    const uint32_t ww[4] = {w8.x, w8.y, w8.z, w8.w};
+    uint32_t g[4];
+#pragma unroll
+    for (int k = 0; k < 4; ++k) {
+        const uint32_t w = ww[k], m = w & t.am;
+        r.m[k] = m;
+        const uint32_t da = (m | H16) - t.ta_TL;
+        const uint32_t ga = (m & ~t.ta_T) | (~(m ^ t.ta_T) & da);
+        const uint32_t dx = t.tx_TH - (w & ~H16);
+        const uint32_t gx = (t.tx_T & ~w) | (~(t.tx_T ^ w) & dx);
+        g[k] = ga & gx;
+    }
+    const uint32_t h8 = static_cast<int>(cq) < min_read_len ? 0u : t.h8;
+    r.p_lo = (__byte_perm(g[0], g[1], 0x7531) & h8) >> 7;
+    r.p_hi = (__byte_perm(g[2], g[3], 0x7531) & h8) >> 7;
+    return r;
+}
+
+__device__ __forceinline__ uint32_t word_sums(const Words8& W, uint32_t p_lo, uint32_t p_hi, uint32_t s) {
+    s = __dp2a_lo(W.m[0], p_lo, s);
+    s = __dp2a_hi(W.m[1], p_lo, s);
+    s = __dp2a_lo(W.m[2], p_hi, s);
+    return __dp2a_hi(W.m[3], p_hi, s);
+}
+
+__device__ __forceinline__ void next_run_words(const RunArgs& a, WarpRunPF& w, uint32_t lane) {
+    if (lane == 0 && w.al) flush_run(a, w.key, w.s + static_cast<long long>(a.amin) * w.c, w.c, w.mn);
+    w.r += 1u; w.key = w.nkey; w.end = w.nend;
+    request_next_run<false>(a, w, 0ull);
+    w.al = (w.key < a.n_ref) && a.allow[w.key];
+    w.s = 0; w.c = 0; w.mn = 0xffffffffu;
+}
+
+__device__ __forceinline__ void reduce_chunk_words(const RunArgs& a, WarpRunPF& w, const Words8& W, uint32_t base, uint32_t lane,
+                                                   uint32_t& tot, uint32_t& ign) {
+    const uint32_t idx0 = static_cast<uint32_t>(a.idx_base) + base + (lane << 3);
+    const uint32_t chunk_end = base + 256u;
+    const int lane0 = static_cast<int>(lane << 3);
+    uint32_t lo = base;
+    while (lo < chunk_end) {
+        const uint32_t hi = min(w.end, chunk_end);
+        if (w.al) {
+            const uint32_t klo = static_cast<uint32_t>(min(max(static_cast<int>(lo - base) - lane0, 0), 8));
+            const uint32_t khi = static_cast<uint32_t>(min(max(static_cast<int>(hi - base) - lane0, 0), 8));
+            uint32_t in_lo, in_hi;
+            segment_masks(klo, khi, in_lo, in_hi);
+            const uint32_t p_lo = W.p_lo & in_lo, p_hi = W.p_hi & in_hi;
+            const uint32_t s = word_sums(W, p_lo, p_hi, 0u), c = __popc(p_lo | (p_hi << 1));
+            const uint32_t in = khi - klo;
+            tot += in;
+            ign += in - c;
+            w.s += __reduce_add_sync(FULL, s);
+            w.c += __reduce_add_sync(FULL, c);
+            if (w.mn == 0xffffffffu) w.mn = __reduce_min_sync(FULL, first_pass_index(p_lo, p_hi, idx0));
+        }
+        if (hi == w.end) next_run_words(a, w, lane);
+        lo = hi;
+    }
+}
+
+__device__ __forceinline__ void reduce_pair_words(const RunArgs& a, WarpRunPF& w, const Words8& Wa, const Words8& Wb, uint32_t base, uint32_t lane,
+                                                  uint32_t& tot, uint32_t& ign) {
+    if (base + 512u > w.end) {
+        reduce_chunk_words(a, w, Wa, base, lane, tot, ign);
+        reduce_chunk_words(a, w, Wb, base + 256u, lane, tot, ign);
+        return;
+    }
+    if (w.al) {
+        const uint32_t s = word_sums(Wb, Wb.p_lo, Wb.p_hi, word_sums(Wa, Wa.p_lo, Wa.p_hi, 0u));
+        const uint32_t c = __popc(Wa.p_lo | (Wa.p_hi << 1) | (Wb.p_lo << 2) | (Wb.p_hi << 3));
+        tot += 16u;
+        ign += 16u - c;
+        w.s += __reduce_add_sync(FULL, s);
+        w.c += __reduce_add_sync(FULL, c);
+        if (w.mn == 0xffffffffu) {
+            const uint32_t idx0 = static_cast<uint32_t>(a.idx_base) + base + (lane << 3);
+            const uint32_t ma = first_pass_index(Wa.p_lo, Wa.p_hi, idx0);
+            w.mn = __reduce_min_sync(FULL, ma != 0xffffffffu ? ma : first_pass_index(Wb.p_lo, Wb.p_hi, idx0 + 256u));
+        }
+    }
+    if (base + 512u == w.end) next_run_words(a, w, lane);
+}
+
+__device__ __forceinline__ void score_tail_words(const RunArgs& a, uint64_t nchunks, uint32_t lane, uint32_t& tot, uint32_t& ign) {
+    uint32_t r = __ldg(a.chunk_run + nchunks);
+    const int ql = static_cast<int>(__ldg(a.chunk_qlen + nchunks));
+    const uint32_t amask = (1u << a.abits) - 1u;
+    for (uint64_t i = (nchunks << 8) + lane; i < a.n_rec; i += 32) {
+        while (r + 1 < a.n_runs && i >= a.run_start[r + 1]) ++r;
+        const uint32_t key = a.run_tid[r];
+        if (!((key < a.n_ref) && a.allow[key])) continue;
+        ++tot;
+        const uint32_t w = a.words[i];
+        const int as = a.amin + static_cast<int>(w & amask), xm = static_cast<int>(w >> a.abits);
+        if ((as >= a.minscore) && (ql >= a.min_read_len) && (xm <= a.max_xm)) flush_run(a, key, as, 1u, static_cast<uint32_t>(a.idx_base + i));
+        else ++ign;
+    }
+}
+
+template <int CH, int NS, int MINB>
+__global__ void __launch_bounds__(kThreads, MINB) score_runs_ring_words_kernel(const RunArgs a) {
+    pdl_launch_dependents();
+    static_assert(CH % 2 == 0, "chunks are reduced in pairs");
+    extern __shared__ __align__(128) uint8_t ring_raw[];
+    constexpr uint32_t STAGE_B = CH * 512u;
+    constexpr int NW = kThreads / 32;
+    const uint32_t lane = threadIdx.x & 31u, wid = threadIdx.x >> 5;
+    uint8_t* const my = ring_raw + wid * (NS * STAGE_B);
+    uint64_t* const bars = reinterpret_cast<uint64_t*>(ring_raw + NW * NS * STAGE_B) + wid * NS;
+    if (threadIdx.x == 0) {
+        uint64_t* all = reinterpret_cast<uint64_t*>(ring_raw + NW * NS * STAGE_B);
+        for (int i = 0; i < NW * NS; ++i) mbar_init(all + i, 1);
+        fence_mbar_init();
+    }
+    __syncthreads();
+
+    const uint64_t warp = (static_cast<uint64_t>(blockIdx.x) * blockDim.x + threadIdx.x) >> 5;
+    const uint64_t nwarps = (static_cast<uint64_t>(gridDim.x) * blockDim.x) >> 5;
+    const uint64_t nchunks = a.n_rec >> 8;
+    const uint64_t per = (nchunks + nwarps - 1) / nwarps;
+    const uint64_t c0 = warp * per;
+    const uint64_t c1 = (c0 + per < nchunks) ? c0 + per : nchunks;
+    uint32_t tot = 0, ign = 0;
+    const WordThr thr = make_word_thr(a);
+
+    if (c0 < c1) {
+        const uint32_t ngroups = static_cast<uint32_t>((c1 - c0 + CH - 1) / CH);
+        auto issue = [&](uint32_t g, int stage) {
+            const uint64_t ch = c0 + static_cast<uint64_t>(g) * CH;
+            const uint32_t nch = (c1 - ch < static_cast<uint64_t>(CH)) ? static_cast<uint32_t>(c1 - ch) : static_cast<uint32_t>(CH);
+            uint8_t* st = my + stage * STAGE_B;
+            mbar_expect_tx(bars + stage, nch * 512u);
+            if (a.l2_hints) bulk_g2s_hint(st, a.words + (ch << 8), nch * 512u, bars + stage, l2_policy(1));
+            else bulk_g2s(st, a.words + (ch << 8), nch * 512u, bars + stage);
+        };
+        if (lane == 0) {
+            const uint32_t pre = ngroups < static_cast<uint32_t>(NS) ? ngroups : static_cast<uint32_t>(NS);
+            for (uint32_t g = 0; g < pre; ++g) issue(g, static_cast<int>(g));
+        }
+        uint32_t cq = lane < static_cast<uint32_t>(CH) && c0 + lane < c1 ? __ldg(a.chunk_qlen + c0 + lane) : 0u;
+        WarpRunPF w;
+        open_run_pf<false>(a, w, __ldg(a.chunk_run + c0), 0ull);
+        uint32_t phase = 0;
+        int stage = 0;
+        for (uint32_t g = 0; g < ngroups; ++g) {
+            const uint64_t ch = c0 + static_cast<uint64_t>(g) * CH;
+            const uint32_t nch = (c1 - ch < static_cast<uint64_t>(CH)) ? static_cast<uint32_t>(c1 - ch) : static_cast<uint32_t>(CH);
+            const uint32_t cq_next = lane < static_cast<uint32_t>(CH) && ch + CH + lane < c1 ? __ldg(a.chunk_qlen + ch + CH + lane) : 0u;
+            mbar_wait(bars + stage, (phase >> stage) & 1u);
+            phase ^= 1u << stage;
+            const uint8_t* st = my + stage * STAGE_B;
+#pragma unroll
+            for (uint32_t k = 0; k < static_cast<uint32_t>(CH); k += 2) {
+                if (k < nch) {
+                    const bool two = k + 1u < nch;
+                    const uint4 wa = *reinterpret_cast<const uint4*>(st + k * 512u + lane * 16u);
+                    const uint4 wb = two ? *reinterpret_cast<const uint4*>(st + (k + 1u) * 512u + lane * 16u) : wa;
+                    if (k + 2u >= nch) {
+                        __syncwarp();
+                        if (lane == 0 && g + NS < ngroups) issue(g + NS, stage);
+                    }
+                    const uint32_t cqa = __shfl_sync(FULL, cq, k), cqb = __shfl_sync(FULL, cq, k + 1u);
+                    const Words8 Wa = word_pass(wa, thr, cqa, a.min_read_len);
+                    const uint32_t base = static_cast<uint32_t>((ch + k) << 8);
+                    if (two) reduce_pair_words(a, w, Wa, word_pass(wb, thr, cqb, a.min_read_len), base, lane, tot, ign);
+                    else reduce_chunk_words(a, w, Wa, base, lane, tot, ign);
+                }
+            }
+            cq = cq_next;
+            stage = (stage + 1 == NS) ? 0 : stage + 1;
+        }
+        if (lane == 0 && w.al) flush_run(a, w.key, w.s + static_cast<long long>(a.amin) * w.c, w.c, w.mn);
+    }
+
+    if (warp == nwarps - 1 && (a.n_rec & 255u)) score_tail_words(a, nchunks, lane, tot, ign);
+    tot = __reduce_add_sync(FULL, tot);
+    ign = __reduce_add_sync(FULL, ign);
+    if (lane == 0 && tot) {
+        atomicAdd(a.counters + 0, static_cast<unsigned long long>(tot));
+        atomicAdd(a.counters + 1, static_cast<unsigned long long>(ign));
+    }
+}
+
+constexpr uint32_t kWordsCH = 4, kWordsNS = 2;
+constexpr auto score_runs_ring_words = score_runs_ring_words_kernel<kWordsCH, kWordsNS, 4>;
+
 struct RingCfg { void (*kern)(const RunArgs); uint32_t ch, ns; };
 template <bool QC, bool HINT>
 inline RingCfg ring_config(int variant) {
diff --git a/metamlst_b200/native.py b/metamlst_b200/native.py
--- a/metamlst_b200/native.py
+++ b/metamlst_b200/native.py
@@ -96,6 +96,11 @@
     "mmlst_score_runs_qc_dev": (C.c_int, [C.c_void_p, C.c_void_p, C.c_uint32] + [C.c_void_p] * 5 + [C.c_uint64, C.c_uint64, C.c_void_p, C.c_uint32,
                                           C.c_int, C.c_int, C.c_int, C.c_void_p, C.c_void_p, C.c_void_p, C.c_void_p, C.c_void_p]),
     "mmlst_expand_chunk_qlen_dev": (C.c_int, [C.c_void_p, C.c_uint64, C.c_void_p, C.c_void_p]),
+    "mmlst_score_words_dev": (C.c_int, [C.c_void_p, C.c_void_p, C.c_uint64, C.c_void_p, C.c_void_p, C.POINTER(C.c_int), C.POINTER(C.c_int),
+                                        C.POINTER(C.c_int), C.c_void_p]),
+    "mmlst_score_runs_words_dev": (C.c_int, [C.c_void_p, C.c_void_p, C.c_uint32, C.c_void_p, C.c_void_p, C.c_void_p, C.c_int, C.c_int, C.c_void_p,
+                                             C.c_uint64, C.c_uint64, C.c_void_p, C.c_uint32, C.c_int, C.c_int, C.c_int, C.c_void_p, C.c_void_p,
+                                             C.c_void_p, C.c_void_p, C.c_void_p]),
     "mmlst_inflate_raw": (C.c_int, [C.c_void_p, C.c_size_t, C.c_void_p, C.c_size_t, C.POINTER(C.c_size_t)]),
     "mmlst_set_score_variant": (C.c_int, [C.c_int]),
     "mmlst_set_score_l2_hints": (C.c_int, [C.c_int]),
diff --git a/metamlst_b200/packing.py b/metamlst_b200/packing.py
--- a/metamlst_b200/packing.py
+++ b/metamlst_b200/packing.py
@@ -15,6 +15,18 @@
 PLANE_SLACK_WORDS = 8
 PREC_DTYPE = np.dtype([("pos", "<i4"), ("row_off", "<u4"), ("reflen", "<u2"), ("as_named", "<i2"), ("xm_named", "u1"), ("pad", "u1"), ("nw", "<u2")])
 assert PREC_DTYPE.itemsize == 16
+
+
+def score_words(as0: np.ndarray, xm3: np.ndarray):
+    as0 = np.asarray(as0, dtype=np.int64)
+    xm3 = np.asarray(xm3, dtype=np.int64)
+    if as0.shape[0] == 0:
+        return None, 0, 0
+    amin, amax, xmax = int(as0.min()), int(as0.max()), int(xm3.max())
+    abits = (amax - amin).bit_length()
+    if abits + xmax.bit_length() > 16:
+        return None, amin, abits
+    return ((xm3 << abits) | (as0 - amin)).astype(np.uint16), amin, abits
 
 
 @dataclass
diff --git a/metamlst_b200/pipeline.py b/metamlst_b200/pipeline.py
--- a/metamlst_b200/pipeline.py
+++ b/metamlst_b200/pipeline.py
@@ -43,6 +43,7 @@
         self.dev = dev
         self.use_runs = bool(use_runs) if use_runs is not None else getattr(streams, "run_tid", None) is not None
         self.use_qc = self.use_runs and getattr(streams, "chunk_qlen", None) is not None
+        self.use_words = self.use_qc and getattr(streams, "orig_idx", None) is None and getattr(streams, "words", None) is not None
         n_ref = len(index.ref_names)
         self.n_ref = n_ref
         self.allow = torch.from_numpy(index.allow_mask(species_filter)).to(dev)
@@ -126,6 +127,7 @@
         self.s = streams
         self.use_runs = getattr(streams, "run_tid", None) is not None if self._use_runs_arg is None else bool(self._use_runs_arg)
         self.use_qc = self.use_runs and getattr(streams, "chunk_qlen", None) is not None
+        self.use_words = self.use_qc and getattr(streams, "orig_idx", None) is None and getattr(streams, "words", None) is not None
         self.idx_base = int(self._idx_base_arg) if self._idx_base_arg else int(getattr(streams, "idx_base", 0) or 0)
         self.contig_start_d.copy_(torch.from_numpy(np.asarray(streams.contig_start, dtype=np.uint64).view(np.int64)), non_blocking=False)
         need = int(streams.n_prec) // 512 + self.index.n_loci + 8
@@ -157,7 +159,13 @@
         oi = native.ptr(getattr(s, "orig_idx", None))
         if n == 0:
             return
-        if self.use_runs and self.use_qc:
+        if self.use_words and self.lib.mmlst_set_score_variant(-1) == 7:
+            native.check(self.lib.mmlst_score_runs_words_dev(native.ptr(s.run_tid), native.ptr(s.run_start), int(s.run_tid.shape[0]), native.ptr(s.chunk_run),
+                                                             native.ptr(s.chunk_qlen), native.ptr(s.words), s.words_amin, s.words_abits, None, n,
+                                                             self.idx_base, native.ptr(self.allow), self.n_ref, self.minscore, self.max_xM,
+                                                             self.min_read_len, native.ptr(self.sum_as), native.ptr(self.n_hit),
+                                                             native.ptr(self.first_idx), native.ptr(self.counters), self._stream()))
+        elif self.use_runs and self.use_qc:
             native.check(self.lib.mmlst_score_runs_qc_dev(native.ptr(s.run_tid), native.ptr(s.run_start), int(s.run_tid.shape[0]), native.ptr(s.chunk_run),
                                                           native.ptr(s.chunk_qlen), native.ptr(s.as0), native.ptr(s.xm3), oi, n, self.idx_base,
                                                           native.ptr(self.allow), self.n_ref, self.minscore, self.max_xM, self.min_read_len,
@@ -377,6 +385,8 @@
         keys = ["0", "1", "2", "3", "4", "5", "2h", "3h", "4h", "5h"]
         if self.use_qc:
             keys += ["6", "6h", "6g10", "6g12"]
+        if self.use_words:
+            keys += ["7", "7h"]
         grid0 = self.lib.mmlst_set_score_grid_scale(-1)
         for key in keys:
             v = int(key[0])
diff --git a/metamlst_b200/streams.py b/metamlst_b200/streams.py
--- a/metamlst_b200/streams.py
+++ b/metamlst_b200/streams.py
@@ -31,7 +31,7 @@
 
     def build_runs(self) -> "DeviceStreams":
         n = int(self.tid.shape[0])
-        self.run_tid = self.run_start = self.chunk_run = self.chunk_qlen = None
+        self.run_tid = self.run_start = self.chunk_run = self.chunk_qlen = self.words = None
         if n == 0:
             return self
         assert n < 0xffffff00
@@ -48,6 +48,24 @@
         q2 = torch.cat([q, pad]).view(nc, 256)
         if bool((q2 == q2[:, :1]).all().item()):
             self.chunk_qlen = q2[:, 0].to(torch.int16).contiguous()
+        return self.build_words()
+
+    def build_words(self) -> "DeviceStreams":
+        self.words, self.words_amin, self.words_abits = None, 0, 0
+        n = int(self.as0.shape[0])
+        if getattr(self, "chunk_qlen", None) is None or n == 0 or not self.as0.is_cuda:
+            return self
+        import ctypes as C
+        from . import native
+        dev = self.as0.device
+        words = torch.empty(n, dtype=torch.int16, device=dev)
+        scratch = torch.empty(4, dtype=torch.int32, device=dev)
+        amin, abits, fits = C.c_int(0), C.c_int(0), C.c_int(0)
+        with torch.cuda.device(dev):
+            native.check(native.lib().mmlst_score_words_dev(native.ptr(self.as0), native.ptr(self.xm3), n, native.ptr(words), native.ptr(scratch),
+                                                             C.byref(amin), C.byref(abits), C.byref(fits), torch.cuda.current_stream(dev).cuda_stream))
+        if fits.value:
+            self.words, self.words_amin, self.words_abits = words, amin.value, abits.value
         return self
 
     def slice_ranges(self, rank: int, world: int) -> "DeviceStreams":
@@ -81,7 +99,7 @@
         if getattr(self, "run_tid", None) is not None and b > a:
             s.build_runs()
             if int(s.run_tid.shape[0]) > 0.125 * (b - a):
-                s.run_tid = s.run_start = s.chunk_run = s.chunk_qlen = None
+                s.run_tid = s.run_start = s.chunk_run = s.chunk_qlen = s.words = None
         return s
 
     @classmethod
@@ -145,13 +163,14 @@
         s.max_row_words = int(soa.max_row_words)
         cs = np.asarray(soa.contig_start, dtype=np.int64)
         s.contig_start = (np.clip(cs, p0, p1) - p0).astype(np.uint64)
-        s.run_tid = s.run_start = s.chunk_run = s.chunk_qlen = None
+        s.run_tid = s.run_start = s.chunk_run = s.chunk_qlen = s.words = None
         if whole_runs and soa.run_tid is not None:
             s.run_tid, s.run_start, s.chunk_run = up(soa.run_tid, np.int32), up(soa.run_start, np.int32), up(soa.chunk_run, np.int32)
             if soa.chunk_qlen is not None:
                 s.chunk_qlen = up(soa.chunk_qlen, np.int16)
+                s.build_words()
         elif soa.run_tid is not None and int(s.tid.shape[0]):
             s.build_runs()
             if int(s.run_tid.shape[0]) > 0.125 * int(s.tid.shape[0]):
-                s.run_tid = s.run_start = s.chunk_run = s.chunk_qlen = None
+                s.run_tid = s.run_start = s.chunk_run = s.chunk_qlen = s.words = None
         return s
```

Result: slower. 1142 billion (median of 6 runs) (-5.0%).
